# pierluigiferrari/fcn8s_tensorflow

Measured on AMD Instinct MI355X. Metric: training images/sec at 1024x512 bs16, higher is better.
Workload: dtype f32; 1 GPU; FCN-8s (VGG-16, fc6 7x7, 20 classes) train step, 1024x512, 16 images/GPU, SGD+momentum, keep_prob 0.5; global_batch=16, parallelism=dp1

## Files before the change

fcn8s_tensorflow_amd/csrc/fcn8s_internal.h:

```cpp
#pragma once
#include <hip/hip_runtime.h>
#include <stdint.h>
#include "../../include/fcn8s_hip.h"

#if defined(__HIP_DEVICE_COMPILE__) && !defined(__gfx950__)
#error "libfcn8s_hip is written for gfx950 (MI355X) only: build with --offload-arch=gfx950"
#endif
#define FCN8S_LDS_BYTES_NEEDED (160u * 1024u)

#include <string>
namespace fcn8s {

extern thread_local const char* g_last_kernel;
void defer_error(int code, const char* fmt, ...) __attribute__((format(printf, 2, 3)));
int take_deferred_error(std::string* text);

struct IgemmArgs {
    const float* x; const float* w; const float* bias; const float* addend; const float* mask;
    float* y;
    int N, Ma, Mb; long long M;
    int Hi, Wi, Cin, ldx;
    int KW, in_scale, tap_step, tap_off, Ktot;
    int Ho, Wo, Cout, ldy;
    int out_scale, out_offy, out_offx;
    int phases_x; long long w_phase_stride;
    float alpha; int relu; float mask_scale;
    int dropout; float keep_prob; unsigned long long seed; unsigned int stream_id;
    int batched; long long x_batch_stride, y_batch_stride;
    int m_fastest;
    int bt, ldw;
    int fixed_tile;
    int split;
};
void launch_igemm(const IgemmArgs& a, int phases, hipStream_t s);

struct Bf16ConvArgs {
    const float* x; const unsigned short* xh;
    const unsigned short* wt; const float* bias; float* y;
    int N, H, W, Cin, Cout, K;
    int relu, dropout; float keep_prob; unsigned long long seed; unsigned int stream_id;
    long long M; int m_fastest;
};
void launch_w_to_bf16_tiles(const float* w, unsigned short* wt, int K, int Cout, hipStream_t s);
bool launch_conv_bf16(const Bf16ConvArgs& a, hipStream_t s);
void launch_f32_to_bf16(const float* x, unsigned short* y, long long n, hipStream_t s);
struct Bf16Conv256Args {
    const unsigned short* xp; const unsigned short* wt; const float* bias; float* y;
    int N, H, W, Cin, Cout, K;
    int relu, dropout; float keep_prob; unsigned long long seed; unsigned int stream_id;
    long long M; int m_fastest;
    const float* addend;
    const float* mask; float mask_scale;
    int any_shape;
    const unsigned short* mask16;
    float* colpart;
    int ksplit; float* part;
    int rows_bn;
    int guarded;
    unsigned short* yb; int yb_pad;
    long long xp_ps, yb_ps, mask16_ps;
};
bool conv_bf16_256_ok(long long M, int Cin, int Cout, int mode);
void launch_w_to_bf16_t(const float* w, unsigned short* wt, int K, int Cout, hipStream_t s);
void launch_f32_to_bf16_padded(const float* x, unsigned short* xp, int N, int H, int W, int C, int pad, hipStream_t s, long long ps = 0);
int conv_bf16_rows_bm(int Cout, int rows_bn);
bool launch_conv_bf16_256(const Bf16Conv256Args& a, hipStream_t s);
struct Fp8ConvArgs {
    const unsigned char* xp = nullptr; long long xp_ps = 0;
    const unsigned char* wq = nullptr; const int* ew = nullptr;
    const float* bias = nullptr; float* y = nullptr;
    unsigned char* yq = nullptr; long long yq_ps = 0; int yq_pad = 0, yq_exp = 0;
    int ex = 0, relu = 1;
    int N = 0, H = 0, W = 0, Cin = 0, Cout = 0, K = 1;
    long long M = 0;
};
bool launch_conv_fp8(const Fp8ConvArgs& a, hipStream_t s);
void launch_w_to_fp8(const float* w, unsigned char* wq, int* ew, unsigned* amax_scratch, int rows, int Cout, hipStream_t s);
void launch_f32_to_fp8_padded(const float* x, unsigned char* xq, int N, int H, int W, int C, int pad, long long ps, int ex, hipStream_t s);
void launch_zero_border_fp8(unsigned char* xq, int planes, long long ps, int N, int H, int W, int pad, hipStream_t s);
void launch_maxpool_fp8(const unsigned char* xq, long long xps, unsigned char* yq, long long yps, int N, int H, int W, int C, int ypad, hipStream_t s);
void launch_amax(const float* x, long long n, unsigned* amax, hipStream_t s);
bool launch_f32_to_bf16_padded_colsum(const float* x, unsigned short* xp, float* db, int N, int H, int W, int C, int pad, hipStream_t s, long long ps = 0);
void launch_w_to_bf16_flip_t(const float* w, unsigned short* wt, int K, int Cin, int Cout, hipStream_t s);
struct Bf16WgradArgs {
    const unsigned short* A; const unsigned short* B; float* C;
    long long R; int Ci, Cj, K, Wp;
    long long chunk, split_stride; int plain_store;
    long long a_ps, b_ps;
};
bool launch_wgrad_bf16(const Bf16WgradArgs& a, hipStream_t s);

struct WgradArgs {
    const float* A; const float* B; float* C;
    int N, Pa, Pb; long long P;
    int Ha, Wa, Adim, lda, Areal;
    int Bdim, ldb;
    int KW, a_scale, tap_off, ntaps;
    int ldc;
    float alpha;
    float* colsum;
    int batched; long long a_batch_stride, b_batch_stride;
    int c_uninitialized;
    int plain_store;
    int split;
    long long split_stride;
};
void launch_wgrad(const WgradArgs& a, hipStream_t s);

extern thread_local int t_deterministic;
float* det_scratch(hipStream_t s, size_t floats);
float* scratch2(hipStream_t s, size_t floats);
void scratch_release(hipStream_t s);
void launch_det_reduce(float* C, const float* ws, long long rows, int cols, int ldc, long long slab, int nsplit, bool accumulate, hipStream_t s);
bool launch_wgrad_taps(const float* X, const float* dZ, float* dW, float* db, int N, int H, int W, int Cin, int Cout,
// ... 42 lines not shown
                          float rate, float* loss_out, hipStream_t s, const unsigned long long* den = nullptr, float* terms = nullptr);
struct LovaszLayout {
    int nseg = 0, C = 0, tiles = 0; long long L = 0, nsc = 0;
    size_t o_keys[2] = {0, 0}, o_pays[2] = {0, 0}, o_hist = 0, o_tcnt = 0, o_part = 0, o_G = 0, o_V = 0, o_w = 0, o_ncls = 0, o_colpart = 0, o_lov = 0;
    size_t bytes = 0;
};
LovaszLayout lovasz_layout(long long npix, int nseg, int C);
double lovasz_bytes(long long npix, int C, int nmask);
void launch_lovasz_loss(const float* x, int is_logits, const uint8_t* labels, const PixMap* map, int N, long long npix, const LovaszLayout& y,
                        int classes_all, const uint8_t* mask_dev, char* ws, float* class_loss, float* terms, float lce, float llov, float* loss_out,
                        hipStream_t s);
void launch_lovasz_backward(const float* x, int is_logits, const uint8_t* labels, const PixMap* map, int N, long long npix, const LovaszLayout& y,
                            char* ws, float lambda, int accumulate, float* out, float* colsum, hipStream_t s);
void launch_lovasz_total(float* terms, float lce, float* loss_out, hipStream_t s);
void launch_softmax_argmax(const float* logits, float* softmax_out, long long* argmax_out,
                           long long npix, int C, hipStream_t s, const PixMap* map = nullptr, int N = 0);
void launch_tconv_im2col(const float* x, float* A, int N, int Hi, int Wi, int C, int KP, hipStream_t s);
void launch_tconv_col2im(const float* dA, float* dx, int N, int Hi, int Wi, int C, int KP, hipStream_t s);
void launch_tconv_pack_gemm(const float* w, const float* bias, float* b2, float* b2t, float* bias_tiled, int C, int S, int KP, hipStream_t s);
void launch_tconv_unpack_dw(const float* db2, float* dw, int C, int S, hipStream_t s);
void launch_unblock_logits(const float* blocked, float* nhwc, const PixMap& map, int N, int C, hipStream_t s);
void launch_onehot_to_ids(const void* oh, int elem_bytes, long long npix, int C, uint8_t* ids, int* bad, hipStream_t s);
void launch_confusion(const uint8_t* labels, const long long* pred, long long npix,
                      unsigned long long* conf, int C, hipStream_t s);
bool launch_head_fwd(const float* x, const float* w, const float* bias, float* y, long long M, int K, int C, float alpha, hipStream_t s,
                     float* scratch = nullptr, size_t scratch_floats = 0);
bool launch_head_dgrad(const float* dy, const float* wt, const float* mask, float mask_scale, float* dx, long long M, int K, int C, float alpha,
                       hipStream_t s);
bool launch_head_wgrad(const float* x, const float* dy, float* dw, long long M, int K, int C, float alpha, hipStream_t s);
bool launch_maxpool_bwd_bf16(const float* x, const float* dy, unsigned short* dzb, float* db, int N, int H, int W, int C, hipStream_t s, const unsigned char* route = nullptr, long long dzb_ps = 0);
void launch_colsum(const float* x, float* out, long long rows, int C, hipStream_t s);
void launch_sumsq(const float* x, float* out, long long n, hipStream_t s);
void launch_axpy(float* y, const float* x, float a, long long n, hipStream_t s);
void launch_tf_adam(float* theta, const float* g, float* m, float* v, long long n,
                    float lr_t, float b1, float b2, float eps, float gscale, hipStream_t s);
void launch_sgd_momentum(float* theta, const float* g, float* buf, long long n,
                         float lr, float mom, float gscale, hipStream_t s);
void launch_grad_accumulate(float* dst, const float* src, long long n, int mode, hipStream_t s);
constexpr int kGradNormBlocks = 2048;
struct UpdateStats { float norm, clip, scale; int ok; unsigned long long skipped; };
void launch_grad_norm(const float* g, long long n, float grad_scale, float max_norm, double* partials, void* out, bool as_floats, hipStream_t s);
void launch_tf_adam_dev(float* theta, const float* g, float* m, float* v, long long n,
                        float lr_t, float b1, float b2, float eps, const float* s_dev, const int* ok_dev, hipStream_t s);
void launch_sgd_momentum_dev(float* theta, const float* g, float* buf, long long n,
                             float lr, float mom, const float* s_dev, const int* ok_dev, hipStream_t s);
void launch_tf_adam_ema(float* theta, const float* g, float* m, float* v, float* sh, long long n, float lr_t, float b1, float b2, float eps,
                        float gscale, const float* s_dev, const int* ok_dev, float w, hipStream_t s);
void launch_sgd_momentum_ema(float* theta, const float* g, float* buf, float* sh, long long n, float lr, float mom,
                             float gscale, const float* s_dev, const int* ok_dev, float w, hipStream_t s);
void launch_ema_update(float* sh, const float* theta, long long n, float w, const int* ok_dev, hipStream_t s);
void launch_swap(float* a, float* b, long long n, hipStream_t s);
void launch_flip_transpose(const float* w, float* wt, int taps, int Cin, int Cout, hipStream_t s);
void launch_pad_cin(const float* w, float* w4, int taps, int Cin, int Cinp, int Cout, hipStream_t s);
void launch_tconv_phase_pack(const float* w, float* wp, int K, int S, int C, hipStream_t s);
void launch_dropout_mask(float* mask, long long n, float keep_prob, unsigned long long seed,
                         unsigned int stream_id, hipStream_t s);
int wino_r(int KS);
int wino_nsub(int KS);
int wino_alpha(int tile, int KS);
long long wino_slab(long long T, int C);
void launch_wino_filter(int tile, const float* w, float* u, int Cin, int Cout, int KS, hipStream_t s, int transpose_out = 0);
void launch_wino_input(int tile, const float* x, float* v, int N, int H, int W, int C, int KS, hipStream_t s, unsigned* rbits_out = nullptr);
void launch_wino_input_conv1(const float* x0, const float* w4, const float* bias, float* v, int N, int H, int W, hipStream_t s, unsigned* rbits_out = nullptr);
void launch_wino_input_xb(const float* x, float* v, unsigned short* xb, int N, int H, int W, int C, hipStream_t s, unsigned* rbits_out = nullptr);
bool launch_wino_input_dout(int tile, const float* dy, float* v, float* dm, int N, int H, int W, int C, hipStream_t s, const unsigned char* pidx = nullptr);
void launch_wino_output(int tile, const float* m, const float* bias, const float* addend, const float* mask, float mask_scale,
                        int relu, float* y, int N, int H, int W, int C, int dropout, float keep, unsigned long long seed,
                        unsigned int stream_id, hipStream_t s, float* pool = nullptr, unsigned char* pidx = nullptr, int KS = 3,
                        unsigned* rbits_out = nullptr, const unsigned* rbits_in = nullptr);
size_t wino_rbits_words(int tile, int N, int H, int W, int C);
void launch_wino_dout(int tile, const float* dy, float* dm, int N, int H, int W, int C, hipStream_t s, int KS = 3, const unsigned char* pidx = nullptr);
void launch_wino_dgrad_output_dout(const float* dv, const unsigned* rbits_in, float* dm, int N, int H, int W, int C, hipStream_t s);
void launch_wino_dgrad_output_sub44(const float* dv, float* dx, int N, int H, int W, int C, hipStream_t s);
void launch_wino_dgrad_output(const float* dv, const float* addend, const float* mask, float mask_scale, const unsigned* rbits_in, float* y,
                              int N, int H, int W, int C, hipStream_t s);
bool launch_wino_out_in(const float* m, const float* bias, float* v, unsigned* rbits_out, int N, int H, int W, int C, hipStream_t s, bool always = false);
void launch_wino_dfilter(int tile, const float* du, float* dw, int Cin, int Cout, int KS, hipStream_t s);
int fft_fc6_planes();
long long fft_fc6_tiles(int N, int H, int W);
void launch_fft_fc6_filter(const float* w, float* uf, int Cin, int Cout, hipStream_t s);
void launch_fft_fc6_dfilter(const float* duf, float* dw, int Cin, int Cout, hipStream_t s);
void launch_fft_fc6_input(const float* x, float* xf, int N, int H, int W, int C, hipStream_t s);
void launch_fft_fc6_output(const float* yf, const float* bias, float* y, int N, int H, int W, int C, int relu, int dropout, float keep,
                           unsigned long long seed, unsigned int stream_id, hipStream_t s);
void launch_fft_fc6_dout(const float* dz, float* dyf, int N, int H, int W, int C, hipStream_t s);
void launch_fft_fc6_din(const float* dxf, float* patches, float* dx, int N, int H, int W, int C, hipStream_t s);
void launch_augment_u8(const unsigned char* img, const unsigned char* lab, unsigned char* oimg, unsigned char* olab, const int* params,
                       const unsigned char* vlut, int N, int H, int W, int Ho, int Wo, int void_id, hipStream_t s);
void launch_resample_u8(const unsigned char* img, const unsigned char* lab, unsigned char* oimg, unsigned char* olab, const int* params,
                        int N, int H, int W, int Ho, int Wo, int void_id, hipStream_t s);
void launch_tta_input(const void* img, int dtype, int N, int H, int W, int Hs, int Ws, int Hp, int Wp, int flip, float* out4, hipStream_t s);
void launch_tta_accumulate(const float* logits, const PixMap& map, int N, int Hs, int Ws, int flip, int C, int H, int W, float* acc,
                           int first, int last, int npasses, float* softmax_out, long long* argmax_out, hipStream_t s);
bool crf_shape_supported(int C, int radius);
void launch_crf_meanfield(const float* qin, const float* prob, const unsigned char* img, int N, int H, int W, int C, int radius, int dilation,
                          float w_app, float w_smooth, float theta_alpha, float theta_beta, float theta_gamma, float* qout, long long* am, hipStream_t s);
void launch_crf_argmax(const float* p, long long npix, int C, long long* am, hipStream_t s);
size_t cityscapes_work_bytes(int N);
void launch_cityscapes_pair(const uint8_t* gt, const uint16_t* inst, const void* pred, int pred_kind, int N, long long P,
                            unsigned long long* conf, void* work, int* entries, int max_entries, unsigned long long* counts, hipStream_t s);
void launch_boundary_pair(const uint8_t* gt, const void* pred, int pred_kind, int N, int H, int W, int R, unsigned long long* rings,
                          unsigned long long* bprec, unsigned long long* brec, unsigned long long* bad, hipStream_t s);
void launch_fingerprint(const float* x, long long n, unsigned long long* out, hipStream_t s);
void launch_init_normal(float* w, long long n, float stddev, int truncated, unsigned long long seed,
                        unsigned int stream_id, hipStream_t s);

__host__ __device__ inline uint32_t mulhi32(uint32_t a, uint32_t b) { return (uint32_t)(((uint64_t)a * b) >> 32); }
__host__ __device__ inline uint32_t philox_u32(unsigned long long idx, unsigned long long seed, uint32_t stream)
{
    uint32_t c0 = (uint32_t)idx, c1 = (uint32_t)(idx >> 32), c2 = stream, c3 = 0x9E3779B9u;
    uint32_t k0 = (uint32_t)seed, k1 = (uint32_t)(seed >> 32);
#pragma unroll
    for (int r = 0; r < 10; ++r) {
        const uint32_t h0 = mulhi32(0xD2511F53u, c0), l0 = 0xD2511F53u * c0;
        const uint32_t h1 = mulhi32(0xCD9E8D57u, c2), l1 = 0xCD9E8D57u * c2;
        const uint32_t n0 = h1 ^ c1 ^ k0, n2 = h0 ^ c3 ^ k1;
        c0 = n0; c1 = l1; c2 = n2; c3 = l0;
        k0 += 0x9E3779B9u; k1 += 0xBB67AE85u;
    }
    return c0;
}
__host__ __device__ inline float philox_uniform(unsigned long long idx, unsigned long long seed, uint32_t stream)
{
    return (float)(philox_u32(idx, seed, stream) >> 8) * (1.0f / 16777216.0f);
}

}
```

fcn8s_tensorflow_amd/csrc/fft_fc6.hip:

```cpp
#include "fcn8s_internal.h"

namespace fcn8s {

namespace {

__device__ __forceinline__ float c14(int k)
{
    constexpr float t[14] = {1.000000000f, 0.900968868f, 0.623489802f, 0.222520934f, -0.222520934f, -0.623489802f, -0.900968868f,
                             -1.000000000f, -0.900968868f, -0.623489802f, -0.222520934f, 0.222520934f, 0.623489802f, 0.900968868f};
    return t[k % 14];
}
__device__ __forceinline__ float s14(int k)
{
    constexpr float t[14] = {0.000000000f, 0.433883739f, 0.781831482f, 0.974927912f, 0.974927912f, 0.781831482f, 0.433883739f,
                             0.000000000f, -0.433883739f, -0.781831482f, -0.974927912f, -0.974927912f, -0.781831482f, -0.433883739f};
    return t[k % 14];
}
constexpr int nu_of(int v) { return (v == 0 || v == 7) ? 8 : 14; }
constexpr bool is_real(int u, int v) { return (v == 0 || v == 7) && (u == 0 || u == 7); }
constexpr int cplx(int u, int v) { return v == 0 ? u - 1 : (v == 7 ? 90 + u - 1 : 6 + (v - 1) * 14 + u); }
constexpr int realp(int u, int v) { return 288 + (u == 7 ? 1 : 0) + (v == 7 ? 2 : 0); }

#define FFT_FENCE __builtin_amdgcn_sched_barrier(0)

// ... 141 lines not shown
            case 1: input_col<1>(x, xf, slab, tc, oy, ox, H, W, C, c, img); break;
            case 2: input_col<2>(x, xf, slab, tc, oy, ox, H, W, C, c, img); break;
            case 3: input_col<3>(x, xf, slab, tc, oy, ox, H, W, C, c, img); break;
            case 4: input_col<4>(x, xf, slab, tc, oy, ox, H, W, C, c, img); break;
            case 5: input_col<5>(x, xf, slab, tc, oy, ox, H, W, C, c, img); break;
            case 6: input_col<6>(x, xf, slab, tc, oy, ox, H, W, C, c, img); break;
            default: input_col<7>(x, xf, slab, tc, oy, ox, H, W, C, c, img); break;
        }
    }
}

template <int V>
__device__ __forceinline__ void output_col(const float* __restrict__ yf, long long slab, long long tc, float (&acc)[8][8])
{
    constexpr int NU = nu_of(V);
    float R[NU], I[NU];
#pragma unroll
    for (int u = 0; u < NU; ++u) {
        if (is_real(u, V)) { R[u] = yf[realp(u, V) * slab + tc]; I[u] = 0.f; }
        else {
            const float* p = yf + 3LL * cplx(u, V) * slab + tc;
            const float k1 = p[0], k2 = p[slab], k3 = p[2 * slab];
            R[u] = k1 - k3; I[u] = k1 + k2;
        }
    }
#pragma unroll
    for (int j = 0; j < 8; ++j) {
        const int n = 6 + j;
        float P = 0.f, Q = 0.f;
#pragma unroll
        for (int u = 0; u < NU; ++u) {
            const float beta = (is_real(u, V) ? 1.f : 2.f) / 196.f;
            if (is_real(u, V)) { P = fmaf(R[u], beta * c14(u * n), P); Q = fmaf(R[u], beta * s14(u * n), Q); }
            else {
                P = fmaf(R[u], beta * c14(u * n), fmaf(I[u], -beta * s14(u * n), P));
                Q = fmaf(R[u], beta * s14(u * n), fmaf(I[u], beta * c14(u * n), Q));
            }
        }
#pragma unroll
        for (int i = 0; i < 8; ++i) acc[j][i] = fmaf(P, c14(V * (6 + i)), fmaf(Q, -s14(V * (6 + i)), acc[j][i]));
    }
}
__device__ __forceinline__ void output_tile(const float* __restrict__ yf, const float* __restrict__ bias, float* __restrict__ y, int H, int W, int C, long long slab,
                                            long long tc, int n, int ty, int tx, int c, int relu, int dropout, float keep, unsigned long long seed, unsigned int stream_id)
{
    float acc[8][8];
#pragma unroll
    for (int j = 0; j < 8; ++j)
#pragma unroll
        for (int k = 0; k < 8; ++k) acc[j][k] = 0.f;
    output_col<0>(yf, slab, tc, acc); FFT_FENCE; output_col<1>(yf, slab, tc, acc); FFT_FENCE; output_col<2>(yf, slab, tc, acc); FFT_FENCE;
    output_col<3>(yf, slab, tc, acc); FFT_FENCE; output_col<4>(yf, slab, tc, acc); FFT_FENCE; output_col<5>(yf, slab, tc, acc); FFT_FENCE;
    output_col<6>(yf, slab, tc, acc); FFT_FENCE; output_col<7>(yf, slab, tc, acc); FFT_FENCE;
    const float bv = bias ? bias[c] : 0.f;
    const float ik = 1.f / keep;
#pragma unroll
    for (int j = 0; j < 8; ++j)
#pragma unroll
        for (int k = 0; k < 8; ++k) {
            const int py = 8 * ty + j, px = 8 * tx + k;
            if (py >= H || px >= W) continue;
            float v = bv + acc[j][k];
            if (relu) v = fmaxf(v, 0.f);
            const long long off = (((long long)n * H + py) * W + px) * C + c;
            if (dropout) v = philox_uniform((unsigned long long)off, seed, stream_id) < keep ? v * ik : 0.f;
            y[off] = v;
        }
}
__global__ __launch_bounds__(256) void fft_fc6_output_kernel(const float* __restrict__ yf, const float* __restrict__ bias, float* __restrict__ y,
                                                             int N, int H, int W, int C, long long slab, int relu, int dropout, float keep,
                                                             unsigned long long seed, unsigned int stream_id)
{
    const int th = (H + 7) / 8, tw = (W + 7) / 8;
    const long long total = (long long)N * th * tw * C;
    for (long long i = (long long)blockIdx.x * 256 + threadIdx.x; i < total; i += (long long)gridDim.x * 256) {
        const int c = (int)(i % C);
        const long long t = i / C;
        const int tx = (int)(t % tw), ty = (int)((t / tw) % th), n = (int)(t / ((long long)tw * th));
        output_tile(yf, bias, y, H, W, C, slab, i, n, ty, tx, c, relu, dropout, keep, seed, stream_id);
    }
}

template <int V>
__device__ __forceinline__ void dout_col(const float (&d)[8][8], float* __restrict__ dyf, long long slab, long long tc)
{
    float sr[8], si[8];
#pragma unroll
    for (int j = 0; j < 8; ++j) {
        float a = 0.f, b = 0.f;
#pragma unroll
        for (int k = 0; k < 8; ++k) { a = fmaf(d[j][k], c14(V * (6 + k)), a); b = fmaf(d[j][k], -s14(V * (6 + k)), b); }
        sr[j] = a; si[j] = b;
    }
#pragma unroll
    for (int u = 0; u < nu_of(V); ++u) {
        const float beta = (is_real(u, V) ? 1.f : 2.f) / 196.f;
        float gr = 0.f, gi = 0.f;
#pragma unroll
        for (int j = 0; j < 8; ++j) {
            const int n = 6 + j;
            gr = fmaf(sr[j], beta * c14(u * n), fmaf(si[j], beta * s14(u * n), gr));
            gi = fmaf(si[j], beta * c14(u * n), fmaf(sr[j], -beta * s14(u * n), gi));
        }
        if (is_real(u, V)) dyf[realp(u, V) * slab + tc] = gr;
        else {
            const long long p = 3LL * cplx(u, V) * slab + tc;
            dyf[p] = gr + gi; dyf[p + slab] = gi; dyf[p + 2 * slab] = -gr;
        }
    }
}
__global__ __launch_bounds__(256) void fft_fc6_dout_kernel(const float* __restrict__ dz, float* __restrict__ dyf, int N, int H, int W, int C, long long slab)
{
    const int th = (H + 7) / 8, tw = (W + 7) / 8;
    const long long total = (long long)N * th * tw * C;
    for (long long i = (long long)blockIdx.x * 256 + threadIdx.x; i < total; i += (long long)gridDim.x * 256) {
        const int c = (int)(i % C);
        const long long t = i / C;
        const int tx = (int)(t % tw), ty = (int)((t / tw) % th), n = (int)(t / ((long long)tw * th));
        float d[8][8];
#pragma unroll
        for (int j = 0; j < 8; ++j)
#pragma unroll
            for (int k = 0; k < 8; ++k) {
                const int py = 8 * ty + j, px = 8 * tx + k;
                d[j][k] = (py < H && px < W) ? dz[(((long long)n * H + py) * W + px) * C + c] : 0.f;
            }
        dout_col<0>(d, dyf, slab, i); dout_col<1>(d, dyf, slab, i); dout_col<2>(d, dyf, slab, i); dout_col<3>(d, dyf, slab, i);
        dout_col<4>(d, dyf, slab, i); dout_col<5>(d, dyf, slab, i); dout_col<6>(d, dyf, slab, i); dout_col<7>(d, dyf, slab, i);
    }
}

template <int V, int HALF>
__device__ __forceinline__ void din_col(const float* __restrict__ dxf, long long slab, long long tc, float (&acc)[7][14])
{
    constexpr int NU = nu_of(V);
    float A[NU], B[NU];
#pragma unroll
    for (int u = 0; u < NU; ++u) {
        if (is_real(u, V)) { A[u] = dxf[realp(u, V) * slab + tc]; B[u] = 0.f; }
        else {
            const float* p = dxf + 3LL * cplx(u, V) * slab + tc;
            const float ds = p[0], da = p[slab], db = p[2 * slab];
            A[u] = ds + da; B[u] = ds + db;
        }
    }
#pragma unroll
    for (int r = 0; r < 7; ++r) {
        const int n = 7 * HALF + r;
        float P = 0.f, Q = 0.f;
#pragma unroll
        for (int u = 0; u < NU; ++u) {
            if (is_real(u, V)) { P = fmaf(A[u], c14(u * n), P); Q = fmaf(A[u], s14(u * n), Q); }
            else {
                P = fmaf(A[u], c14(u * n), fmaf(B[u], -s14(u * n), P));
                Q = fmaf(A[u], s14(u * n), fmaf(B[u], c14(u * n), Q));
            }
        }
#pragma unroll
        for (int m = 0; m < 14; ++m) acc[r][m] = fmaf(P, c14(V * m), fmaf(Q, -s14(V * m), acc[r][m]));
    }
}
template <int HALF>
__device__ __forceinline__ void din_half(const float* __restrict__ dxf, float* __restrict__ pt, long long slab, long long t, int c, int C)
{
    float acc[7][14];
#pragma unroll
    for (int r = 0; r < 7; ++r)
#pragma unroll
        for (int m = 0; m < 14; ++m) acc[r][m] = 0.f;
    const long long tc = t * C + c;
    din_col<0, HALF>(dxf, slab, tc, acc); FFT_FENCE; din_col<1, HALF>(dxf, slab, tc, acc); FFT_FENCE; din_col<2, HALF>(dxf, slab, tc, acc); FFT_FENCE; din_col<3, HALF>(dxf, slab, tc, acc); FFT_FENCE;
    din_col<4, HALF>(dxf, slab, tc, acc); FFT_FENCE; din_col<5, HALF>(dxf, slab, tc, acc); FFT_FENCE; din_col<6, HALF>(dxf, slab, tc, acc); FFT_FENCE; din_col<7, HALF>(dxf, slab, tc, acc);
    float* o = pt + (t * 196 + 7 * HALF * 14) * C + c;
#pragma unroll
    for (int r = 0; r < 7; ++r)
#pragma unroll
        for (int m = 0; m < 14; ++m) o[(r * 14 + m) * C] = acc[r][m];
}
__global__ __launch_bounds__(256, 2) void fft_fc6_din_kernel(const float* __restrict__ dxf, float* __restrict__ pt, long long T, int C, long long slab)
{
    const long long total = T * 2 * C;
    for (long long i = (long long)blockIdx.x * 256 + threadIdx.x; i < total; i += (long long)gridDim.x * 256) {
        const int c = (int)(i % C);
        const long long r = i / C;
        const int half = (int)(r % 2);
        const long long t = r / 2;
        if (half == 0) din_half<0>(dxf, pt, slab, t, c, C);
        else           din_half<1>(dxf, pt, slab, t, c, C);
    }
}

__global__ __launch_bounds__(256) void fft_fc6_din_gather_kernel(const float* __restrict__ pt, float* __restrict__ dx, int N, int H, int W, int C)
{
    const int th = (H + 7) / 8, tw = (W + 7) / 8;
    const long long total = (long long)N * H * W * C;
    for (long long i = (long long)blockIdx.x * 256 + threadIdx.x; i < total; i += (long long)gridDim.x * 256) {
        const int c = (int)(i % C);
        const long long p = i / C;
        const int px = (int)(p % W), py = (int)((p / W) % H), n = (int)(p / ((long long)W * H));
        const int ty1 = (py + 3) / 8, tx1 = (px + 3) / 8;
        float s = 0.f;
#pragma unroll
        for (int dy = 1; dy >= 0; --dy) {
            const int ty = ty1 - dy, ry = py + 3 - 8 * ty;
            if (ty < 0 || ty >= th || ry > 13) continue;
#pragma unroll
            for (int dxo = 1; dxo >= 0; --dxo) {
                const int tx = tx1 - dxo, rx = px + 3 - 8 * tx;
                if (tx < 0 || tx >= tw || rx > 13) continue;
                s += pt[((((long long)n * th + ty) * tw + tx) * 196 + ry * 14 + rx) * C + c];
            }
        }
        dx[i] = s;
    }
}

}

int fft_fc6_planes() { return 292; }
long long fft_fc6_tiles(int N, int H, int W) { return (long long)N * ((H + 7) / 8) * ((W + 7) / 8); }

void launch_fft_fc6_filter(const float* w, float* uf, int Cin, int Cout, hipStream_t s)
{
    const long long CC = (long long)Cin * Cout;
    hipLaunchKernelGGL(fft_fc6_filter_kernel, dim3(grid_for(CC)), dim3(256), 0, s, w, uf, CC);
}
void launch_fft_fc6_dfilter(const float* duf, float* dw, int Cin, int Cout, hipStream_t s)
{
    const long long CC = (long long)Cin * Cout;
    hipLaunchKernelGGL(fft_fc6_dfilter_kernel, dim3(grid_for(CC)), dim3(256), 0, s, duf, dw, CC);
}
void launch_fft_fc6_input(const float* x, float* xf, int N, int H, int W, int C, hipStream_t s)
{
    const long long T = fft_fc6_tiles(N, H, W);
    hipLaunchKernelGGL(fft_fc6_input_kernel, dim3(grid_for(T * 8 * C)), dim3(256), 0, s, x, xf, N, H, W, C, wino_slab(T, C));
}
void launch_fft_fc6_output(const float* yf, const float* bias, float* y, int N, int H, int W, int C, int relu, int dropout, float keep,
                           unsigned long long seed, unsigned int stream_id, hipStream_t s)
{
    const long long T = fft_fc6_tiles(N, H, W);
    hipLaunchKernelGGL(fft_fc6_output_kernel, dim3(grid_for(T * C)), dim3(256), 0, s, yf, bias, y, N, H, W, C, wino_slab(T, C), relu, dropout, keep, seed, stream_id);
}
void launch_fft_fc6_dout(const float* dz, float* dyf, int N, int H, int W, int C, hipStream_t s)
{
    const long long T = fft_fc6_tiles(N, H, W);
    hipLaunchKernelGGL(fft_fc6_dout_kernel, dim3(grid_for(T * C)), dim3(256), 0, s, dz, dyf, N, H, W, C, wino_slab(T, C));
}
void launch_fft_fc6_din(const float* dxf, float* patches, float* dx, int N, int H, int W, int C, hipStream_t s)
{
    const long long T = fft_fc6_tiles(N, H, W);
    hipLaunchKernelGGL(fft_fc6_din_kernel, dim3(grid_for(T * 2 * C)), dim3(256), 0, s, dxf, patches, T, C, wino_slab(T, C));
    hipLaunchKernelGGL(fft_fc6_din_gather_kernel, dim3(grid_for((long long)N * H * W * C)), dim3(256), 0, s, patches, dx, N, H, W, C);
}

}
```

fcn8s_tensorflow_amd/csrc/igemm.hip:

```cpp
#include "fcn8s_internal.h"
#include <cmath>
#include <cstdlib>
#include <map>
#include <mutex>
#include <string>

namespace fcn8s {

thread_local const char* g_last_kernel = nullptr;
#define FCN8S_STR2(x) #x
#define FCN8S_STR(x) FCN8S_STR2(x)

typedef float f32x16 __attribute__((ext_vector_type(16)));
constexpr int BK_ = 16;

static __device__ __forceinline__ float4 ldg4(const float* p) { return *reinterpret_cast<const float4*>(p); }

static __device__ __forceinline__ unsigned xcd_swizzle(unsigned p, unsigned total)
{
    const unsigned q = total >> 3, r = total & 7u, xcd = p & 7u, i = p >> 3;
    return (xcd < r ? xcd * (q + 1) : r * (q + 1) + (xcd - r) * q) + i;
}

thread_local int t_deterministic = 0;
// ... 349 lines not shown
    }
}

static __device__ __forceinline__ void glds16(const float* sbase, unsigned voff, unsigned lds_byte_off)
{
    asm volatile("s_mov_b32 m0, %2\n\ts_nop 0\n\tglobal_load_lds_dwordx4 %0, %1" ::"v"(voff), "s"(sbase), "s"(lds_byte_off) : "memory", "m0");
}
template <int N> static __device__ __forceinline__ void wait_vmcnt() { asm volatile("s_waitcnt vmcnt(%0)" ::"n"(N) : "memory"); }

typedef __bf16 bf16x8 __attribute__((ext_vector_type(8)));
template <int NS> struct Bf16Pieces { bf16x8 p[NS]; };
template <int NS>
static __device__ __forceinline__ void split_bf16(const float (&x)[8], Bf16Pieces<NS>& o)
{
    typedef __bf16 bf16x2 __attribute__((ext_vector_type(2)));
    typedef float f32x2 __attribute__((ext_vector_type(2)));
    typedef unsigned u32x4 __attribute__((ext_vector_type(4)));
    u32x4 w[NS];
#pragma unroll
    for (int i = 0; i < 4; ++i) {
        f32x2 r = {x[2 * i], x[2 * i + 1]};
#pragma unroll
        for (int k = 0; k < NS; ++k) {
            const unsigned pk = __builtin_bit_cast(unsigned, __builtin_convertvector(r, bf16x2));
            w[k][i] = pk;
            if (k + 1 < NS) {
                const f32x2 back = {__builtin_bit_cast(float, pk << 16), __builtin_bit_cast(float, pk & 0xffff0000u)};
                r = r - back;
            }
        }
    }
#pragma unroll
    for (int k = 0; k < NS; ++k) o.p[k] = __builtin_bit_cast(bf16x8, w[k]);
}
template <int NS>
static __device__ __forceinline__ f32x16 mfma_split(const Bf16Pieces<NS>& a, const Bf16Pieces<NS>& b, f32x16 acc)
{
    if constexpr (NS == 3) {
        acc = __builtin_amdgcn_mfma_f32_32x32x16_bf16(a.p[2], b.p[0], acc, 0, 0, 0);
        acc = __builtin_amdgcn_mfma_f32_32x32x16_bf16(a.p[0], b.p[2], acc, 0, 0, 0);
        acc = __builtin_amdgcn_mfma_f32_32x32x16_bf16(a.p[1], b.p[1], acc, 0, 0, 0);
    }
    acc = __builtin_amdgcn_mfma_f32_32x32x16_bf16(a.p[1], b.p[0], acc, 0, 0, 0);
    acc = __builtin_amdgcn_mfma_f32_32x32x16_bf16(a.p[0], b.p[1], acc, 0, 0, 0);
    return __builtin_amdgcn_mfma_f32_32x32x16_bf16(a.p[0], b.p[0], acc, 0, 0, 0);
}

template <int BM, int BN, int WM, int WN, int S, bool EPI, int NSPLIT, bool BT = false>
static __device__ __forceinline__ void gemm_glds_body(const IgemmArgs& p);
template <int BM, int BN, int WM, int WN, int S, bool EPI>
__global__ __launch_bounds__(256, (S * (BM + BN) * 64 <= 40960) ? 4 : 3) void gemm_glds_kernel(const IgemmArgs p) { gemm_glds_body<BM, BN, WM, WN, S, EPI, 0>(p); }
template <int BM, int BN, int WM, int WN, int S, bool EPI>
__global__ __launch_bounds__(256, (S * (BM + BN) * 64 <= 40960) ? 4 : 3) void gemm_glds_x3_kernel(const IgemmArgs p) { gemm_glds_body<BM, BN, WM, WN, S, EPI, 3>(p); }
template <int BM, int BN, int WM, int WN, int S>
__global__ __launch_bounds__(256, (S * (BM + BN) * 64 <= 40960) ? 4 : 3) void gemm_glds_nt_kernel(const IgemmArgs p) { gemm_glds_body<BM, BN, WM, WN, S, false, 0, true>(p); }
template <int BM, int BN, int WM, int WN, int S>
__global__ __launch_bounds__(256, (S * (BM + BN) * 64 <= 40960) ? 4 : 3) void gemm_glds_nt_x3_kernel(const IgemmArgs p) { gemm_glds_body<BM, BN, WM, WN, S, false, 3, true>(p); }
template <int BM, int BN, int WM, int WN, int S, bool EPI>
__global__ __launch_bounds__(256, (S * (BM + BN) * 64 <= 40960) ? 4 : 3) void gemm_glds_x2_kernel(const IgemmArgs p) { gemm_glds_body<BM, BN, WM, WN, S, EPI, 2>(p); }
template <int BM, int BN, int WM, int WN, int S>
__global__ __launch_bounds__(256, (S * (BM + BN) * 64 <= 40960) ? 4 : 3) void gemm_glds_nt_x2_kernel(const IgemmArgs p) { gemm_glds_body<BM, BN, WM, WN, S, false, 2, true>(p); }
template <int BM, int BN, int WM, int WN, int S, bool EPI, int NSPLIT, bool BT>
static __device__ __forceinline__ void gemm_glds_body(const IgemmArgs& p)
{
    constexpr int BK = 16, CH = 4, RPI = 16;
    constexpr int TM = BM / WM / 32, TN = BN / WN / 32;
    constexpr int A_PW = BM / RPI / 4, B_PW = BT ? BN / RPI / 4 : BK * BN / 256 / 4;
    static_assert(WM * WN == 4 && A_PW >= 1 && B_PW >= 1, "tile / wave split");
    constexpr int L = A_PW + B_PW;
    constexpr int STAGE = BM * BK + BK * BN;
    __shared__ __attribute__((aligned(16))) float smem[S * STAGE];
    static_assert(S * STAGE >= 4 * 32 * 36, "epilogue patches");

    const int tid = threadIdx.x, lane = tid & 63, wave = __builtin_amdgcn_readfirstlane(tid >> 6);
    int cwave = wave;
    bool idle = false;
    if constexpr (BM == 64 && WM == 2 && WN == 2) {
        if (p.M <= 32) {
            const unsigned lin = blockIdx.x + gridDim.x * (blockIdx.y + gridDim.y * blockIdx.z);
            cwave = wave ^ (int)(((lin >> 8) & 1u) << 1); idle = cwave >= 2;
        }
    }
    const int wm = cwave / WN, wn = cwave % WN;
    const int pz = blockIdx.z;
    const float* __restrict__ Wp = p.w + (long long)pz * p.w_phase_stride;
    const float* __restrict__ X = p.batched ? p.x + (long long)pz * p.x_batch_stride : p.x;
    float* __restrict__ Y = p.batched ? p.y + (long long)pz * p.y_batch_stride : p.y;
    const unsigned ntn = (unsigned)(p.Cout / BN);
    const unsigned lid = xcd_swizzle(blockIdx.x, gridDim.x);
    const unsigned ntm = gridDim.x / ntn;
    const long long m0 = (long long)(p.m_fastest ? lid % ntm : lid / ntn) * BM;
    const int n0 = (int)(p.m_fastest ? lid / ntm : lid % ntn) * BN;

    unsigned a_voff[A_PW], b_voff[B_PW];
#pragma unroll
    for (int i = 0; i < A_PW; ++i) {
        const int row = (wave * A_PW + i) * RPI + lane / CH, pc = lane % CH;
        const int c = pc ^ ((row >> 2) & 3);
        long long m = m0 + row; if (m >= p.M) m = p.M - 1;
        a_voff[i] = (unsigned)((m - m0) * p.ldx + c * 4) * 4u;
    }
#pragma unroll
    for (int i = 0; i < B_PW; ++i) {
        if (BT) {
            const int row = (wave * B_PW + i) * RPI + lane / CH, pc = lane % CH;
            const int c = pc ^ ((row >> 2) & 3);
            b_voff[i] = (unsigned)(row * p.ldw + c * 4) * 4u;
        } else {
            const int f = (wave * B_PW + i) * 64 + lane;
            const int k = f / (BN / 4), j = (f % (BN / 4)) * 4;
            b_voff[i] = (unsigned)(k * p.Cout + j) * 4u;
        }
    }
    const int nkt_all = p.Ktot / BK;
    const int kt0 = (int)((long long)nkt_all * blockIdx.y / gridDim.y);
    const int nkt = (int)((long long)nkt_all * (blockIdx.y + 1) / gridDim.y) - kt0;
    const float* a_base = X + m0 * p.ldx + (long long)kt0 * BK;
    const float* b_base = BT ? Wp + (long long)n0 * p.ldw + (long long)kt0 * BK : Wp + n0 + (long long)kt0 * BK * p.Cout;
    const unsigned lds0 = (unsigned)(size_t)(__attribute__((address_space(3))) float*)smem;
    auto issue = [&](int kt, int stage) {
        const float* ga = a_base + (long long)kt * BK;
        const float* gb = BT ? b_base + (long long)kt * BK : b_base + (long long)kt * BK * p.Cout;
        const unsigned la = lds0 + (unsigned)(stage * STAGE + wave * A_PW * 256) * 4u;
        const unsigned lb = lds0 + (unsigned)(stage * STAGE + BM * BK + wave * B_PW * 256) * 4u;
#pragma unroll
        for (int i = 0; i < A_PW; ++i) glds16(ga, a_voff[i], la + i * 1024);
#pragma unroll
        for (int i = 0; i < B_PW; ++i) glds16(gb, b_voff[i], lb + i * 1024);
    };

    f32x16 acc[TM][TN];
#pragma unroll
    for (int i = 0; i < TM; ++i)
#pragma unroll
        for (int j = 0; j < TN; ++j)
#pragma unroll
            for (int r = 0; r < 16; ++r) acc[i][j][r] = 0.f;

    int a_off[TM], a_sw[TM];
#pragma unroll
    for (int tm = 0; tm < TM; ++tm) {
        const int row = wm * TM * 32 + tm * 32 + (lane & 31);
        a_off[tm] = row * BK;
        a_sw[tm] = (row >> 2) & 3;
    }
    const int b_off = ((lane >> 5) * 4) * BN + wn * TN * 32 + (lane & 31);
    int bt_off[TN], bt_sw[TN];
#pragma unroll
    for (int tn = 0; tn < TN; ++tn) {
        const int row = wn * TN * 32 + tn * 32 + (lane & 31);
        bt_off[tn] = row * BK;
        bt_sw[tn] = (row >> 2) & 3;
    }
    auto compute = [&](int stage) {
        if (idle) return;
        const float* sa = smem + stage * STAGE;
        const float* sb = sa + BM * BK;
        if constexpr (NSPLIT >= 2) {
            Bf16Pieces<NSPLIT> ap[TM], bp[TN];
#pragma unroll
            for (int tm = 0; tm < TM; ++tm) {
                const float4 u = *reinterpret_cast<const float4*>(sa + a_off[tm] + (((2 * (lane >> 5)) ^ a_sw[tm]) * 4));
                const float4 v = *reinterpret_cast<const float4*>(sa + a_off[tm] + (((2 * (lane >> 5) + 1) ^ a_sw[tm]) * 4));
                const float x[8] = {u.x, u.y, u.z, u.w, v.x, v.y, v.z, v.w};
                split_bf16<NSPLIT>(x, ap[tm]);
            }
#pragma unroll
            for (int tn = 0; tn < TN; ++tn) {
                float x[8];
                if (BT) {
                    const float4 u = *reinterpret_cast<const float4*>(sb + bt_off[tn] + (((2 * (lane >> 5)) ^ bt_sw[tn]) * 4));
                    const float4 v = *reinterpret_cast<const float4*>(sb + bt_off[tn] + (((2 * (lane >> 5) + 1) ^ bt_sw[tn]) * 4));
                    x[0] = u.x; x[1] = u.y; x[2] = u.z; x[3] = u.w; x[4] = v.x; x[5] = v.y; x[6] = v.z; x[7] = v.w;
// ... 282 lines not shown
            const long long pix = ((long long)n * p.H + y0 + 2 * g + (row >> 4)) * p.W + x0 + (row & 15);
            if (p.y) *reinterpret_cast<float4*>(p.y + pix * BN + wn * 32 + (lane & 7) * 4) = v;
        }
        if (p.yb16) {
            const float4 b0 = ldg4(p.bias + wn * 32 + (lane & 3) * 8), b1 = ldg4(p.bias + wn * 32 + (lane & 3) * 8 + 4);
#pragma unroll
            for (int j = 0; j < 2; ++j) {
                const int row = j * 16 + (lane >> 2);
                const float4 u = *reinterpret_cast<const float4*>(&patch[row * LDT + (lane & 3) * 8]);
                const float4 w_ = *reinterpret_cast<const float4*>(&patch[row * LDT + (lane & 3) * 8 + 4]);
                __attribute__((ext_vector_type(8))) __bf16 o;
                o[0] = (__bf16)fmaxf(u.x + b0.x, 0.f); o[1] = (__bf16)fmaxf(u.y + b0.y, 0.f); o[2] = (__bf16)fmaxf(u.z + b0.z, 0.f); o[3] = (__bf16)fmaxf(u.w + b0.w, 0.f);
                o[4] = (__bf16)fmaxf(w_.x + b1.x, 0.f); o[5] = (__bf16)fmaxf(w_.y + b1.y, 0.f); o[6] = (__bf16)fmaxf(w_.z + b1.z, 0.f); o[7] = (__bf16)fmaxf(w_.w + b1.w, 0.f);
                const long long q = ((long long)n * (p.H + 2) + y0 + 2 * g + (row >> 4) + 1) * (p.W + 2) + x0 + (row & 15) + 1;
                *reinterpret_cast<__attribute__((ext_vector_type(8))) __bf16*>(p.yb16 + (p.yb16_ps ? (long long)wn * p.yb16_ps + q * 32 + (lane & 3) * 8 : q * BN + wn * 32 + (lane & 3) * 8)) = o;
            }
        }
        __builtin_amdgcn_wave_barrier();
    }
  }
}

bool launch_conv1_fwd(const float* x4, const float* w48, const float* bias, float* y, const float* zero16, int N, int H, int W, int Cout, int tiled, hipStream_t s, unsigned short* yb16, long long yb16_ps)
{
    if (Cout != 64 || !bias || !zero16) return false;
    if ((yb16 || !y) && !(tiled && H % 8 == 0 && W % 16 == 0)) return false;
    Conv1Args a{x4, w48, bias, y, zero16, N, H, W, (long long)N * H * W, yb16, yb16_ps};
    if (tiled && H % 8 == 0 && W % 16 == 0) {
        g_last_kernel = "conv1_tile_kernel";
        const long long tiles = (long long)N * (H / 8) * (W / 16);
        if (W % 64 == 0 && tiles >= 4 * 4096) hipLaunchKernelGGL(conv1_tile_kernel<4>, dim3((unsigned)(tiles / 4)), dim3(256), 0, s, a);
        else                                  hipLaunchKernelGGL(conv1_tile_kernel<1>, dim3((unsigned)tiles), dim3(256), 0, s, a);
        return true;
    }
    g_last_kernel = "conv1_glds_kernel";
    hipLaunchKernelGGL(conv1_glds_kernel, dim3((unsigned)((a.M + 127) / 128)), dim3(256), 0, s, a);
    return true;
}

template <int BM, int BN, int WM, int WN, int BKF = 16>
static void launch_igemm_cfg(const IgemmArgs& a0, int phases, hipStream_t s)
{
    IgemmArgs a = a0;
    a.m_fastest = (double)a.Ktot * a.Cout > (double)a.M * a.Cin;
    dim3 grid((unsigned)(((a.M + BM - 1) / BM) * ((a.Cout + BN - 1) / BN)), 1, (unsigned)phases);
    const bool fast = (phases == 1 || a.batched) && a.Cin % BKF == 0 && a.Cout % BN == 0 && a.Ktot % a.Cin == 0;
    const bool tap_inner = fast && (double)a.Ktot * a.Cout * 4.0 <= 64e6 && a.Ktot / a.Cin <= 32;
    const bool plain = fast && a.batched && a.Ktot == a.Cin && !a.bias && !a.addend && !a.mask && !a.relu && !a.dropout && a.alpha == 1.f &&
                       a.out_scale == 1 && a.ldy >= a.Cout && a.ldy % 4 == 0 && a.in_scale == 1 && a.tap_off == 0;
    const int mode = !fast ? 0 : (plain ? 3 : (tap_inner ? 2 : 1));
    static const std::string base = "igemm_fwd_kernel<" + std::to_string(BM) + ", " + std::to_string(BN) + ", " + std::to_string(WM) + ", " + std::to_string(WN) + ", ";
    static const std::string tags[4] = {base + "0, 16>", base + "1, " + std::to_string(BKF) + ">", base + "2, " + std::to_string(BKF) + ">",
                                        base + "3, " + std::to_string(BKF) + ">"};
    g_last_kernel = tags[mode].c_str();
    const bool linear = (mode == 1 || mode == 3) && !a.relu && !a.mask && !a.dropout && !a.addend && a.out_scale == 1 && a.ldy == a.Cout;
    constexpr int splitk_min_kt = 64;
    const unsigned nblocks = grid.x * (unsigned)phases, nkt_all = (unsigned)(a.Ktot / BKF);
    if (linear && !t_deterministic && !a.fixed_tile && ((grid.x < 512 && nkt_all >= 512) || (nblocks < 2048 && nkt_all >= (unsigned)splitk_min_kt))) {
        unsigned ks = nkt_all >= 512 && grid.x < 512 ? 1024 / grid.x : 4096 / nblocks;
        if (ks > 8) ks = 8;
        if (ks > nkt_all / 16) ks = nkt_all / 16;
        if (ks >= 2) {
            grid.y = ks;
            const size_t nfl = a.batched ? (size_t)(phases - 1) * a.y_batch_stride + (size_t)a.M * a.Cout : (size_t)a.M * a.Cout;
            hipMemsetAsync(a.y, 0, nfl * sizeof(float), s);
        }
    }
    const bool rows1x1 = fast && a.Ktot == a.Cin && a.in_scale == 1 && a.tap_off == 0 && a.out_scale == 1 && a.out_offy == 0 && a.out_offx == 0 &&
                         (a.batched || (phases == 1 && a.Hi == a.Ma && a.Wi == a.Mb && a.Ho == a.Ma && a.Wo == a.Mb)) && a.ldy >= a.Cout;
    const bool bias_only = fast && a.bias && !a.addend && !a.mask && !a.relu && !a.dropout && a.alpha == 1.f && a.ldy % 4 == 0 && a.Cout % 4 == 0 && grid.y == 1;
    if constexpr (BN >= 64 && BKF == 16) {
        if (rows1x1 && (mode == 3 || grid.y == 1) && (long long)(BM - 1) * a.ldx < (1LL << 29) && (long long)16 * a.Cout < (1LL << 29)) {
            static const std::string gbase = "gemm_glds_kernel<" + std::to_string(BM) + ", " + std::to_string(BN) + ", " + std::to_string(WM) + ", " + std::to_string(WN) + ", 3, ";
            static const std::string xbase = "gemm_glds_x3_kernel<" + std::to_string(BM) + ", " + std::to_string(BN) + ", " + std::to_string(WM) + ", " + std::to_string(WN) + ", 3, ";
            static const std::string gt[4] = {gbase + "false>", gbase + "true>", xbase + "false>", xbase + "true>"};
            const bool mask_only = fast && a.mask && !a.bias && !a.addend && !a.relu && !a.dropout && a.alpha == 1.f && a.ldy % 4 == 0 && a.Cout % 4 == 0 && grid.y == 1;
            const bool epi = mode != 3 && !bias_only && !mask_only;
            if (a.bt) {
                static const std::string nb = "gemm_glds_nt_kernel<" + std::to_string(BM) + ", " + std::to_string(BN) + ", " + std::to_string(WM) + ", " + std::to_string(WN) + ", 3>";
                static const std::string nbx = "gemm_glds_nt_x3_kernel<" + std::to_string(BM) + ", " + std::to_string(BN) + ", " + std::to_string(WM) + ", " + std::to_string(WN) + ", 3>";
                if (mode != 3 || (long long)(BN - 1) * a.ldw >= (1LL << 29)) { defer_error(FCN8S_ERR_STATE, "transposed-B GEMM needs the plain batched form"); return; }
                static const std::string nbx2 = "gemm_glds_nt_x2_kernel<" + std::to_string(BM) + ", " + std::to_string(BN) + ", " + std::to_string(WM) + ", " + std::to_string(WN) + ", 3>";
                g_last_kernel = (a.split == 3 ? nbx : a.split == 2 ? nbx2 : nb).c_str();
                if (a.split == 3) hipLaunchKernelGGL((gemm_glds_nt_x3_kernel<BM, BN, WM, WN, 3>), grid, dim3(256), 0, s, a);
                else if (a.split == 2) hipLaunchKernelGGL((gemm_glds_nt_x2_kernel<BM, BN, WM, WN, 3>), grid, dim3(256), 0, s, a);
                else                   hipLaunchKernelGGL((gemm_glds_nt_kernel<BM, BN, WM, WN, 3>), grid, dim3(256), 0, s, a);
                return;
            }
            g_last_kernel = gt[(epi ? 1 : 0) + (a.split == 3 ? 2 : 0)].c_str();
            if (a.split == 3) {
                if (epi) hipLaunchKernelGGL((gemm_glds_x3_kernel<BM, BN, WM, WN, 3, true>), grid, dim3(256), 0, s, a);
                else     hipLaunchKernelGGL((gemm_glds_x3_kernel<BM, BN, WM, WN, 3, false>), grid, dim3(256), 0, s, a);
                return;
            }
            if (a.split == 2) {
                static const std::string x2base = "gemm_glds_x2_kernel<" + std::to_string(BM) + ", " + std::to_string(BN) + ", " + std::to_string(WM) + ", " + std::to_string(WN) + ", 3, ";
                static const std::string x2t[2] = {x2base + "false>", x2base + "true>"};
                g_last_kernel = x2t[epi ? 1 : 0].c_str();
                if (epi) hipLaunchKernelGGL((gemm_glds_x2_kernel<BM, BN, WM, WN, 3, true>), grid, dim3(256), 0, s, a);
                else     hipLaunchKernelGGL((gemm_glds_x2_kernel<BM, BN, WM, WN, 3, false>), grid, dim3(256), 0, s, a);
                return;
            }
            if (epi) hipLaunchKernelGGL((gemm_glds_kernel<BM, BN, WM, WN, 3, true>), grid, dim3(256), 0, s, a);
            else     hipLaunchKernelGGL((gemm_glds_kernel<BM, BN, WM, WN, 3, false>), grid, dim3(256), 0, s, a);
            return;
        }
    }
    if (a.bt) {
        defer_error(FCN8S_ERR_STATE, "transposed-B GEMM (M %lld, K %d, N %d, tile %dx%d) does not fit the LDS-DMA kernel", a.M, a.Ktot, a.Cout, BM, BN);
        return;
    }
    if (mode == 3)      hipLaunchKernelGGL((igemm_fwd_kernel<BM, BN, WM, WN, 3, BKF>), grid, dim3(256), 0, s, a);
    else if (mode == 2) hipLaunchKernelGGL((igemm_fwd_kernel<BM, BN, WM, WN, 2, BKF>), grid, dim3(256), 0, s, a);
    else if (mode == 1) hipLaunchKernelGGL((igemm_fwd_kernel<BM, BN, WM, WN, 1, BKF>), grid, dim3(256), 0, s, a);
    else                hipLaunchKernelGGL((igemm_fwd_kernel<BM, BN, WM, WN, 0, 16>), grid, dim3(256), 0, s, a);
}

void launch_igemm(const IgemmArgs& a, int phases, hipStream_t s)
{
    auto cost = [&](int bm, int bn, int bpc, double eff) {
        const long long blocks = ((a.M + bm - 1) / bm) * ((a.Cout + bn - 1) / bn) * phases;
        const long long n = (blocks + 255) / 256, rem = n % bpc;
        const double tail = rem == 0 ? 0.0 : (rem == 1 ? 2.0 : (rem == 2 ? 2.4 : 3.0));
        return ((double)(n / bpc) * bpc + tail) * bm * bn / eff;
    };
    if (a.fixed_tile && a.Cout % 128 == 0) { launch_igemm_cfg<128, 128, 2, 2>(a, phases, s); return; }
    if (a.fixed_tile && a.Cout % 64 == 0)  { launch_igemm_cfg<128, 64, 2, 2>(a, phases, s); return; }
    if (a.Cout <= 32)      launch_igemm_cfg<128, 32, 4, 1>(a, phases, s);
    else if (a.Cout <= 64) {
        if (cost(128, 64, 4, 1.0) <= cost(64, 64, 4, 0.9)) launch_igemm_cfg<128, 64, 2, 2>(a, phases, s);
        else                                               launch_igemm_cfg<64, 64, 2, 2>(a, phases, s);
    } else {
        const double c128 = cost(128, 128, 3, 1.0), c64x128 = cost(64, 128, 4, 0.9), c64 = cost(64, 64, 4, 0.85);
        if (a.M > 64 && c128 <= c64x128 && c128 <= c64) launch_igemm_cfg<128, 128, 2, 2>(a, phases, s);
        else if (c64x128 <= c64)                        launch_igemm_cfg<64, 128, 2, 2>(a, phases, s);
        else                                            launch_igemm_cfg<64, 64, 2, 2>(a, phases, s);
    }
}

template <int BM, int BN, int WM, int WN, int WK, bool FAST, bool COLSUM>
__global__ __launch_bounds__(256, FAST ? 4 : 1) void wgrad_kernel(const WgradArgs p, const int chunk)
{
    constexpr int BK = 16, LDA = BM, LDB = BN;
    constexpr int TM = BM / WM / 32, TN = BN / WN / 32;
    constexpr int A_F4 = BK * BM / 4, B_F4 = BK * BN / 4;
    constexpr int A_LD = (A_F4 + 255) / 256, B_LD = (B_F4 + 255) / 256;
    static_assert(WM * WN * WK == 4, "4 waves");
    __shared__ __attribute__((aligned(16))) float smem[2 * BK * LDA + 2 * BK * LDB];
    float* As = smem;
    float* Bs = smem + 2 * BK * LDA;

    const int tid = threadIdx.x, lane = tid & 63, wave = tid >> 6;
    const int wk = wave / (WM * WN), wmn = wave % (WM * WN);
    const int wm = wmn / WN, wn = wmn % WN;
    const int ntj = (p.Bdim + BN - 1) / BN;
    const int ti = blockIdx.x / ntj, tj = blockIdx.x - ti * ntj;
    const int i0 = ti * BM, j0 = tj * BN;
    const int tap = blockIdx.z;
    const int ty = tap / p.KW, tx = tap - ty * p.KW;
    const int dy = p.batched ? 0 : ty + p.tap_off, dx = p.batched ? 0 : tx + p.tap_off;
    const float* __restrict__ Ap = p.batched ? p.A + (long long)tap * p.a_batch_stride : p.A;
    const float* __restrict__ Bp = p.batched ? p.B + (long long)tap * p.b_batch_stride : p.B;
    const long long pbeg = (long long)blockIdx.y * chunk;
    const long long pend = (pbeg + chunk < p.P) ? pbeg + chunk : p.P;
    const int PaPb = p.Pa * p.Pb;
    const bool do_colsum = COLSUM && p.colsum != nullptr && tap == 0 && ti == 0 && wm == 0;
// ... 834 lines not shown
```

fcn8s_tensorflow_amd/csrc/model.hip:

```cpp
#include "../../include/fcn8s_hip.h"
#include "fcn8s_internal.h"
#include "device_buffer.h"
#include "pass_state.h"
#include <cstdarg>

#include <dlfcn.h>
#include <atomic>
#include <chrono>
#include <thread>
#include <cmath>
#include <cstdio>
#include <cstring>
#include <cstdlib>
#include <algorithm>
#include <mutex>
#include <map>
#include <set>
#include <string>
#include <vector>

using namespace fcn8s;

extern "C" {
typedef struct ncclComm* ncclComm_t;
typedef struct { char internal[128]; } ncclUniqueId;
typedef enum { ncclSuccess = 0, ncclUnhandledCudaError = 1, ncclSystemError = 2, ncclInternalError = 3, ncclInvalidArgument = 4, ncclInvalidUsage = 5,
               ncclRemoteError = 6, ncclInProgress = 7 } ncclResult_t;
typedef enum { ncclSum = 0 } ncclRedOp_t;
typedef enum { ncclFloat = 7, ncclDouble = 8 } ncclDataType_t;
}
static_assert(sizeof(ncclUniqueId) == FCN8S_COMM_ID_BYTES, "fcn8s_comm_unique_id hands out ncclUniqueId bytes");

namespace {

thread_local std::string g_last_error;
thread_local int t_deferred_code = 0;
thread_local std::string t_deferred_text;

struct ParamInfo {
    std::string name;
    int ndim;
    int64_t shape[4];
    size_t offset, numel;
};

struct ProfGroup {
    std::string name;
    std::vector<std::pair<hipEvent_t, hipEvent_t>> ev;
    std::vector<std::pair<hipEvent_t, hipEvent_t>> ev_shared;
    double flops = 0, bytes = 0;
    int64_t launches = 0;
};

struct Act { float* p = nullptr; size_t n = 0; int H = 0, W = 0, C = 0; };

const int kConvsPerBlock[5] = {2, 2, 3, 3, 3};

}

namespace fcn8s {
void defer_error(int code, const char* fmt, ...)
{
    if (t_deferred_code) return;
    char buf[1024];
    va_list ap; va_start(ap, fmt); vsnprintf(buf, sizeof buf, fmt, ap); va_end(ap);
    t_deferred_code = code; t_deferred_text = buf;
}
int take_deferred_error(std::string* text)
{
    const int c = t_deferred_code;
    if (c && text) *text = t_deferred_text;
    t_deferred_code = 0; t_deferred_text.clear();
    return c;
}
}

struct Q8Buf { DeviceBuf<unsigned char> p; int N = 0, H = 0, W = 0, C = 0, pad = -1, ex = 0; long long ps = 0; };
struct W8Bank { DeviceBuf<unsigned char> wq; int* ew = nullptr; unsigned* amax = nullptr; };

struct fcn8s_model {
    int C = 20, fc6k = 7, device = 0;
    int widths[7] = {64, 128, 256, 512, 512, 4096, 4096};
    uint64_t seed = 0;
    std::vector<ParamInfo> params;
    std::map<std::string, int> index;
    size_t total = 0;
    size_t bucket_off[FCN8S_MAX_BUCKETS] = {0}, bucket_n[FCN8S_MAX_BUCKETS] = {0};
    hipEvent_t bucket_ev[FCN8S_MAX_BUCKETS] = {nullptr};
    bool bucket_final[FCN8S_MAX_BUCKETS] = {false};
    ncclComm_t comm = nullptr; int comm_rank = 0, comm_world = 1;
    hipStream_t comm_stream = nullptr;
    static constexpr int kCommSlots = FCN8S_MAX_BUCKETS + 1, kCommMisc = FCN8S_MAX_BUCKETS;
    hipEvent_t comm_done[kCommSlots] = {nullptr}; bool comm_pending[FCN8S_MAX_BUCKETS] = {false};
    std::mutex comm_mu;
    std::thread comm_watch; std::atomic<bool> comm_watch_stop{false}, comm_failed{false};
    std::atomic<bool> comm_inflight[kCommSlots] = {}; int64_t comm_enq_ns[kCommSlots] = {0};
    std::string comm_error; int64_t comm_timeout_ms = 600000;
    float *d_params = nullptr, *d_grads = nullptr;
    DeviceBuf<float> own_params, own_grads;
    DeviceBuf<float> d_m, d_v, d_wt, d_w1pad, d_tph[3];
    DeviceBuf<float> d_wino_u; float *d_wino_v = nullptr, *d_wino_m = nullptr;
    size_t ufl = 0;
    int wino_min_cin = 64;
    int wino_tile = 6;
    int wino_fc6 = 1;
    int fc6_fft = 1;
    int fc6_fft_wgrad = 1;
    int wino_tile_hires = 0, wino_hires_pixels = 0;
    int wino_force_tile = 0;
    int precision = FCN8S_PREC_F32;
    bool frozen = false;
    unsigned long long frozen_fp = 0; DeviceBuf<unsigned long long> d_fp;
    PinnedBuf<unsigned long long> h_fp; hipEvent_t fp_event = nullptr;
    std::map<std::string, DeviceBuf<float>> u_cache;
    std::map<std::string, DeviceBuf<float>> u_train;
    bool fwd_train = false;
    PassState pass;
    int deterministic = 0;
    int fuse_dgrad_dout = 1;
    int fuse_out_in = 1;
    int conv1_tiled = 1, conv1_wgrad_mfma = 1;
    int conv1_in_transform = 1;
    DeviceBuf<unsigned short> d_wbf16;
    std::map<std::string, DeviceBuf<unsigned short>> wbf16_cache;
    std::set<std::string> bank_stale; bool banks_stale = false;
    int bf16_gemm256 = 1;
    DeviceBuf<unsigned short> d_abf16;
    std::map<std::string, DeviceBuf<unsigned short>> xbf16;
    using G16Map = std::map<std::string, DeviceBuf<unsigned short>>;
    G16Map xg16, dyg16;
    std::set<std::string> g16_stale;
    int bf16_fuse_pool = 1;
    int bf16_infer_copies = 1;
    int bf16_rows_bn = 0;
    int bf16_acts = 1;
    bool fp8_calibrated = false, fp8_calibrating = false; float fp8_amax[FCN8S_FP8_LAYERS] = {}; DeviceBuf<unsigned> d_fp8_amax;
    std::map<std::string, Q8Buf> q8;
    std::map<std::string, W8Bank> w8; std::set<std::string> w8_valid;
    int saved_wino_min_cin = -1, saved_wino_fc6 = -1;
    int bf16_copy_by_transform = 1;
    int64_t ws_allocs = 0;
    bool x0_ready = false;
    DeviceBuf<char> crf_buf;
    DeviceBuf<char> tta_buf;
    hipStream_t stream = nullptr;
    int64_t step = 0;
    int N = 0, H = 0, W = 0;
    int plan_N = 0;
    DeviceBuf<char> arena;
    std::map<std::string, Act> acts;
    struct KeptDy { DeviceBuf<float> p; size_t n = 0; };
    int keep_dy = 0; std::map<std::string, KeptDy> kept_dy;
    int tconv_gemm = 1; PixMap pm{0, 0, 0, 0, 0, 0}; int tg_kp = 0;
    float *logits_b = nullptr, *dlogits_b = nullptr, *tg_A = nullptr, *tg_dA = nullptr;
    DeviceBuf<float> tg_b2, tg_b2t, tg_bias, tg_db2;
    bool logits_nhwc_valid = false;
    float *dlogits = nullptr, *da3 = nullptr, *da4 = nullptr, *ds7 = nullptr, *gskip3 = nullptr, *gskip4 = nullptr;
    float *gbuf[2] = {nullptr, nullptr};
    int gcur = 0;
    void* d_images = nullptr; uint8_t* d_labels = nullptr;
    DeviceBuf<float> d_loss; float *d_regsum = nullptr, *d_softmax = nullptr;
    PinnedBuf<float> h_loss; hipEvent_t loss_ev = nullptr; bool loss_copied = false;
    float* d_lastbias = nullptr;
    double* d_partials = nullptr; long long* d_pred = nullptr;
    int loss_mode = 0, last_loss_mode = 0; float ohem_thresh = 0.f; int64_t ohem_min_kept = 0;
    DeviceBuf<float> d_cw; DeviceBuf<char> loss_ws;
    bool lov_on = false, have_terms = false; float lov_ce = 1.f, lov_w = 0.f; int lov_per_image = 0, lov_all = 0;
    DeviceBuf<uint8_t> d_lovmask; int lov_nmask = 0; DeviceBuf<char> lov_ws; float* d_terms = nullptr;
    DeviceBuf<float> d_acc; int acc_k[FCN8S_MAX_BUCKETS] = {0}; bool acc_taken[FCN8S_MAX_BUCKETS] = {false};
    float max_norm = 0.f; DeviceBuf<char> upd_ws; bool last_update_clipped = false;
    DeviceBuf<float> d_ema; double ema_decay = 0.0; int ema_warmup = 1; bool ema_swapped = false;
    DeviceBuf<unsigned long long> d_conf;
    double loss_sum = 0; int64_t loss_cnt = 0;
    float keep_prob = 1.f, l2_rate = 0.f;
    uint32_t drop_stream = 0;
    bool have_forward = false, have_loss = false, train_mode = false;
    int next_bucket = 0;
    const uint8_t* cur_labels = nullptr;
    bool profile = false, profile_detail = false;
    struct StageSlot { PinnedBuf<uint8_t> h_img, h_lab; DeviceBuf<uint8_t> d_img, d_lab;
                       hipEvent_t ready = nullptr, consumed = nullptr; bool used = false; };
    StageSlot slots[FCN8S_NUM_STAGE_SLOTS];
    hipStream_t copy_stream = nullptr;
    std::vector<ProfGroup> groups;
    std::string err;
    fcn8s_model() = default;
    fcn8s_model(const fcn8s_model&) = delete;
    ~fcn8s_model()
    {
// ... 67 lines not shown
    add("fc7_pool4_conv2d_trans/bias", {C});
    add("fc7_pool4_pool3_conv2d_trans/kernel", {16, 16, C, C});
    add("fc7_pool4_pool3_conv2d_trans/bias", {C});
    total = off;
    for (int i = 0; i < FCN8S_MAX_BUCKETS; ++i) { boff[i] = 0; bn[i] = 0; }
    boff[0] = fc7_start;   bn[0] = total - fc7_start;
    boff[1] = fc6_start;   bn[1] = fc7_start - fc6_start;
    boff[2] = conv4_start; bn[2] = fc6_start - conv4_start;
    boff[3] = 0;           bn[3] = conv4_start;
}

void resolve_cfg(const fcn8s_config* cfg, int& C, int widths[7], int& fc6k)
{
    static const int def[7] = {64, 128, 256, 512, 512, 4096, 4096};
    C = cfg->num_classes;
    fc6k = cfg->fc6_ksize > 0 ? cfg->fc6_ksize : 7;
    for (int i = 0; i < 7; ++i) widths[i] = cfg->widths[i] > 0 ? cfg->widths[i] : def[i];
}

const ParamInfo& P(const fcn8s_model* m, const std::string& n) { return m->params[m->index.at(n)]; }
float* Wp(fcn8s_model* m, const std::string& n) { return m->d_params + P(m, n).offset; }
float* Gp(fcn8s_model* m, const std::string& n) { return m->d_grads + P(m, n).offset; }
float* WTp(fcn8s_model* m, const std::string& n) { return m->d_wt + P(m, n).offset; }

int group_id(fcn8s_model* m, const char* name)
{
    for (size_t i = 0; i < m->groups.size(); ++i) if (m->groups[i].name == name) return (int)i;
    ProfGroup g; g.name = name; m->groups.push_back(g);
    return (int)m->groups.size() - 1;
}
struct ProfScope {
    fcn8s_model* m; int gid = -1; hipEvent_t a = nullptr, b = nullptr; double fl = 0, by = 0;
    ProfScope(fcn8s_model* m_, const char* group, double flops, double bytes, const char* layer = nullptr) : m(m_), fl(flops), by(bytes)
    {
        if (!m || !m->profile) return;
        fcn8s::g_last_kernel = nullptr;
        gid = (m->profile_detail && layer) ? group_id(m, (std::string(group) + ":" + layer).c_str()) : group_id(m, group);
        hipEventCreate(&a); hipEventCreate(&b);
        hipEventRecord(a, m->stream);
        m->groups[gid].flops += flops; m->groups[gid].bytes += bytes; m->groups[gid].launches += 1;
    }
    ~ProfScope()
    {
        if (gid < 0) return;
        hipEventRecord(b, m->stream);
        m->groups[gid].ev.emplace_back(a, b);
        if (fcn8s::g_last_kernel) {
            const int k = group_id(m, (std::string("kernel:") + fcn8s::g_last_kernel).c_str());
            m->groups[k].flops += fl; m->groups[k].bytes += by; m->groups[k].launches += 1;
            m->groups[k].ev_shared.emplace_back(a, b);
        }
    }
};

static void prof_derived(fcn8s_model* m, const char* what)
{
    if (m && m->profile && m->profile_detail) m->groups[group_id(m, (std::string("derived:") + what).c_str())].launches += 1;
}

struct ConvEpi { float alpha = 1.f; };
struct FwdEpi : ConvEpi {
    const float* bias = nullptr; int relu = 0;
    int dropout = 0; float keep = 1.f; uint32_t stream_id = 0;
    float* pool_out = nullptr; unsigned char* pool_idx = nullptr;
    int skip_y = 0;
    unsigned* relu_bits_out = nullptr;
    unsigned* in_relu_bits_out = nullptr; const char* in_layer = nullptr;
    float* next_v = nullptr; const char* next_layer = nullptr;
};
struct DgradEpi : ConvEpi {
    const float* addend = nullptr;
    const float* mask = nullptr; float mask_scale = 1.f;
    const unsigned* relu_bits_in = nullptr;
    const float* w_fwd = nullptr;
    int lazy_wt = 0;
    float* dm_out = nullptr; const char* dm_out_layer = nullptr;
    const char* yb_layer = nullptr; int yb_K = 3;
    bool yb_only = false;
};

static bool bt_gemm_ok(int K, int N) { return K % 16 == 0 && (N == 64 || N % 128 == 0); }
thread_local int t_op_split = 0;
thread_local int t_op_rows_bn = 0;
thread_local int t_op_planes = 1;
int split_of(const fcn8s_model* m)
{
    if (!m) return t_op_split;
    if (m->precision == FCN8S_PREC_F32X3 || m->precision == FCN8S_PREC_BF16_FWD) return 3;
    if (m->precision == FCN8S_PREC_F32X2 || m->precision == FCN8S_PREC_BF16_FWD_X2) return 2;
    return 0;
}
static inline bool bf16_fwd_mode(const fcn8s_model* m) { return m->precision == FCN8S_PREC_BF16_FWD || m->precision == FCN8S_PREC_BF16_FWD_X2; }
static inline bool bf16_train_mode(const fcn8s_model* m) { return m && m->precision == FCN8S_PREC_BF16_TRAIN; }
static inline long long bf16_guard_rows(int K, int Wp) { return (long long)((K - 1) / 2) * Wp + (K - 1) / 2 + 640; }
#ifndef A_PLANES
#define A_PLANES 1
#endif
static inline long long g16_ps(int N, int H, int W, int K) { const int pad = (K - 1) / 2, Wp_ = W + 2 * pad; return A_PLANES ? ((long long)N * (H + 2 * pad) * Wp_ + 2 * bf16_guard_rows(K, Wp_)) * 32 : 0; }
static inline long long g16_off(long long G, int C) { return A_PLANES ? G * 32 : G * C; }
unsigned short* g16_for(fcn8s_model* m, fcn8s_model::G16Map& bufs, const char* layer, int N, int H, int W, int C, int K, hipStream_t s);
unsigned short* dyb_for(fcn8s_model* m, const char* layer, const float* dy, int N, int H, int W, int C, int K, hipStream_t s, float* db = nullptr, bool* db_done = nullptr);

int wino_tile_for(const fcn8s_model* m, int H, int W, int K = 3)
{
    if (!m || H % 2 || W % 2) return 0;
    if (m->wino_force_tile && K == 3) return (m->wino_force_tile == 6 || (H % m->wino_force_tile == 0 && W % m->wino_force_tile == 0)) ? m->wino_force_tile : 0;
    int tmax = m->wino_tile;
    if (K == 3 && m->wino_tile_hires && m->wino_hires_pixels > 0 && (long long)H * W >= m->wino_hires_pixels && m->wino_tile_hires < tmax) tmax = m->wino_tile_hires;
    const bool t4 = tmax >= 4 && H % 4 == 0 && W % 4 == 0;
    if (K == 7) return (m->wino_tile >= 4 && H % 4 == 0 && W % 4 == 0) ? 4 : 0;
    if (tmax == 6) {
        auto rows = [&](long long tiles) { return m->plan_N == 1 ? (tiles + 63) / 64 * 64 : tiles; };
        const long long c6 = 64LL * rows((long long)((H + 5) / 6) * ((W + 5) / 6)), c4 = t4 ? 36LL * rows((long long)(H / 4) * (W / 4)) : 16LL * rows((long long)(H / 2) * (W / 2));
        if (c6 < c4) return 6;
    }
    return t4 ? 4 : 2;
}
long long wino_tiles(int tile, int N, int H, int W) { return (long long)N * ((H + tile - 1) / tile) * ((W + tile - 1) / tile); }
struct WinoEpi { const float* bias = nullptr; const float* addend = nullptr; const float* mask = nullptr; float mask_scale = 1.f;
                 int relu = 0; int dropout = 0; float keep = 1.f; unsigned long long seed = 0; unsigned int stream_id = 0; float* pool = nullptr; unsigned char* pidx = nullptr;
                 unsigned* rbits_out = nullptr; const unsigned* rbits_in = nullptr; int skip_y = 0;
                 unsigned* in_rbits_out = nullptr;
                 float* next_v = nullptr; bool* fused_out = nullptr; };
static bool fft6_cheaper(const fcn8s_model* m, int H, int W)
{
    const long long fft = 292LL * ((H + 7) / 8) * ((W + 7) / 8);
    const long long other = wino_tile_for(m, H, W, 7) == 4 ? 196LL * (H / 4) * (W / 4) : 49LL * H * W;
    return fft < other;
}
static bool fft6_shape_ok(const fcn8s_model* m, int ci, int co) { return m->wino_fc6 && m->fc6_fft && m->fc6k == 7 && ci % 16 == 0 && co % 128 == 0; }
static bool fft6_on(const fcn8s_model* m, int N, int H, int W, int ci, int co)
{
    if (!m || !fft6_shape_ok(m, ci, co) || !fft6_cheaper(m, H, W) || m->precision != FCN8S_PREC_F32 || m->frozen || !m->d_wino_v || !m->d_wino_m) return false;
    const long long T = fft_fc6_tiles(N, H, W);
    auto v = m->acts.find("wino_v"), mm = m->acts.find("wino_m");
    return v != m->acts.end() && mm != m->acts.end() && v->second.n >= (size_t)fft_fc6_planes() * (size_t)wino_slab(T, ci) &&
           mm->second.n >= std::max((size_t)fft_fc6_planes() * (size_t)wino_slab(T, co), (size_t)T * 196 * ci);
}
constexpr long long kFft6WgradMinTiles = 32;
static bool fft6_wgrad_wanted(const fcn8s_model* m, long long T) { return m->fc6_fft_wgrad == 2 || (m->fc6_fft_wgrad == 1 && T >= kFft6WgradMinTiles); }
struct Fc6Scratch { size_t v_wino = 0, v_fft = 0, m_fft = 0, wv = 0; };
static Fc6Scratch fc6_scratch_floats(const fcn8s_model* m, int N, int h5, int w5, int ci, int co)
{
    Fc6Scratch r;
    const int hi = std::max(ci, co);
    if (m->wino_fc6 && m->fc6k == 7 && wino_tile_for(m, h5, w5, 7) == 4 && ci % 16 == 0 && co % 64 == 0) {
        const size_t P = (size_t)wino_alpha(4, 7) * wino_alpha(4, 7);
        const int ns2 = wino_nsub(7) * wino_nsub(7);
        const long long T = wino_tiles(4, N, h5, w5);
        r.v_wino = std::max(P * (size_t)wino_slab(T, ns2 * hi), P * (size_t)wino_slab(T, hi));
        r.wv = P * (size_t)wino_slab(T, ns2 * ci);
    }
    if (fft6_shape_ok(m, ci, co) && fft6_cheaper(m, h5, w5)) {
        const size_t P = (size_t)fft_fc6_planes();
        const long long T = fft_fc6_tiles(N, h5, w5);
        r.v_fft = P * (size_t)wino_slab(T, ci);
        r.m_fft = std::max(P * (size_t)wino_slab(T, co), (size_t)T * 196 * ci);
        if (fft6_wgrad_wanted(m, T)) r.wv = std::max(r.wv, P * (size_t)wino_slab(T, ci));
    }
    return r;
}
static size_t fc6_bank_floats(int ci, int co)
{
    size_t n = 49 * 4 * (size_t)ci * co;
    if (ci % 16 == 0 && co % 128 == 0) n = std::max(n, (size_t)fft_fc6_planes() * ci * co);
    return n;
}
static IgemmArgs fft6_gemm(const float* x, const float* w, float* y, long long T, int K, int Nc)
{
    IgemmArgs a{};
    a.x = x; a.w = w; a.y = y;
    a.N = 1; a.Ma = (int)T; a.Mb = 1; a.M = T;
    a.Hi = (int)T; a.Wi = 1; a.Cin = K; a.ldx = K;
    a.KW = 1; a.in_scale = 1; a.tap_step = 1; a.tap_off = 0; a.Ktot = K;
    a.Ho = (int)T; a.Wo = 1; a.Cout = Nc; a.ldy = Nc;
    a.out_scale = 1; a.phases_x = 1; a.w_phase_stride = (long long)K * Nc;
    a.alpha = 1.f; a.mask_scale = 1.f;
    a.batched = 1; a.x_batch_stride = wino_slab(T, K); a.y_batch_stride = wino_slab(T, Nc);
    return a;
}
static bool conv_fft6_fwd(fcn8s_model* m, const char* layer, const float* x, const float* w, float* y, int N, int H, int W, int Cin, int Cout,
                          const float* bias, int relu, int dropout, float keep, unsigned int stream_id, hipStream_t s)
{
    const int P = fft_fc6_planes();
    const long long T = fft_fc6_tiles(N, H, W);
    DeviceBuf<float>& uf = m->u_train[std::string(layer) + "#fft"];
    if (!uf.grow((size_t)P * Cin * Cout * sizeof(float), s)) return false;
    auto wv = m->acts.find(std::string("wv:") + layer);
    const bool dft_wgrad = wv != m->acts.end() && fft6_wgrad_wanted(m, T) && wv->second.n >= (size_t)P * (size_t)wino_slab(T, Cin) &&
                           m->ufl >= (size_t)P * Cin * Cout;
    const bool want_v = !dft_wgrad && wv != m->acts.end() && wino_tile_for(m, H, W, 7) == 4;
    float* xf = dft_wgrad ? wv->second.p : m->d_wino_v;
    { ProfScope ps(m, "fc6_fft_transform", 0, 4.0 * ((49.0 + P) * Cin * Cout + (double)N * H * W * Cin + (double)P * T * Cin));
      launch_fft_fc6_filter(w, uf, Cin, Cout, s); launch_fft_fc6_input(x, xf, N, H, W, Cin, s); }
    if (want_v) { ProfScope ps(m, "wino_transform", 0, 4.0 * ((double)N * H * W * Cin * 4 + 49.0 * wino_tiles(4, N, H, W) * 4 * Cin));
                  launch_wino_input(4, x, wv->second.p, N, H, W, Cin, 7, s); }
    IgemmArgs a = fft6_gemm(xf, uf, m->d_wino_m, T, Cin, Cout); a.fixed_tile = 1;
    { ProfScope ps(m, "fc6_fft_gemm_fwd", 2.0 * P * T * Cin * Cout, 4.0 * P * (T * (double)(Cin + Cout) + (double)Cin * Cout), layer); launch_igemm(a, P, s); }
    { ProfScope ps(m, "fc6_fft_transform", 0, 4.0 * ((double)P * T * Cout + (double)N * H * W * Cout));
      launch_fft_fc6_output(m->d_wino_m, bias, y, N, H, W, Cout, relu, dropout, keep, m->seed, stream_id, s); }
    m->pass.fft6_ready.give(layer);
    if (dft_wgrad) m->pass.fft6_xf.give(layer);
    return true;
}
static void conv_fft6_wgrad(fcn8s_model* m, const char* layer, const float* xf, const float* dz, float* dw, float* db, int N, int H, int W, int Cin, int Cout, hipStream_t s)
{
    const int P = fft_fc6_planes();
    const long long T = fft_fc6_tiles(N, H, W);
    { ProfScope ps(m, "fc6_fft_transform", 0, 4.0 * ((double)N * H * W * Cout + (double)P * T * Cout)); launch_fft_fc6_dout(dz, m->d_wino_m, N, H, W, Cout, s); }
    m->pass.fft6_dyf.give(layer);
    WgradArgs g{}; g.split = 0;
    g.A = xf; g.B = m->d_wino_m; g.C = m->d_wino_u;
    g.N = 1; g.Pa = 1; g.Pb = (int)T; g.P = T;
    g.Ha = 1; g.Wa = (int)T; g.Adim = Cin; g.lda = Cin; g.Areal = Cin;
    g.Bdim = Cout; g.ldb = Cout; g.KW = 1; g.a_scale = 1; g.tap_off = 0; g.ntaps = P; g.ldc = Cout; g.alpha = 1.f; g.colsum = nullptr;
    g.batched = 1; g.a_batch_stride = wino_slab(T, Cin); g.b_batch_stride = wino_slab(T, Cout); g.c_uninitialized = 1;
    { ProfScope ps(m, "fc6_fft_gemm_wgrad", 2.0 * P * T * Cin * Cout, 4.0 * P * (T * (double)(Cin + Cout) + (double)Cin * Cout), layer); launch_wgrad(g, s); }
    { ProfScope ps(m, "fc6_fft_transform", 0, 4.0 * (P + 49.0) * Cin * Cout); launch_fft_fc6_dfilter(m->d_wino_u, dw, Cin, Cout, s); }
    if (db) { ProfScope ps(m, "colsum", 0, 4.0 * N * H * W * Cout); launch_colsum(dz, db, (long long)N * H * W, Cout, s); }
}
static void conv_fft6_dgrad(fcn8s_model* m, const char* layer, const float* dz, const float* uf, float* dx, int N, int H, int W, int Cin, int Cout, hipStream_t s)
{
    const int P = fft_fc6_planes();
    const long long T = fft_fc6_tiles(N, H, W);
    if (!m->pass.fft6_dyf.take(layer)) {
        m->pass.fft6_dyf.drop();
        ProfScope ps(m, "fc6_fft_transform", 0, 4.0 * ((double)N * H * W * Cin + (double)P * T * Cin)); launch_fft_fc6_dout(dz, m->d_wino_m, N, H, W, Cin, s);
    }
    IgemmArgs a = fft6_gemm(m->d_wino_m, uf, m->d_wino_v, T, Cin, Cout);
    a.fixed_tile = 1; a.bt = 1; a.ldw = Cin;
    { ProfScope ps(m, "fc6_fft_gemm_dgrad", 2.0 * P * T * Cin * Cout, 4.0 * P * (T * (double)(Cin + Cout) + (double)Cin * Cout), layer); launch_igemm(a, P, s); }
    { ProfScope ps(m, "fc6_fft_transform", 0, 4.0 * ((double)P * T * Cout + 2.0 * 196.0 * T * Cout + (double)N * H * W * Cout));
      launch_fft_fc6_din(m->d_wino_v, m->d_wino_m, dx, N, H, W, Cout, s); }
}

void conv_winograd(fcn8s_model* m, int tile, int KS, bool fwd, const float* x, const float* wk, float* y, float* u, float* v, float* mm,
                   int N, int H, int W, int Cin, int Cout, const WinoEpi& e, hipStream_t s, const char* layer, bool v_ready = false)
{
    const int P = wino_alpha(tile, KS) * wino_alpha(tile, KS), nsub2 = wino_nsub(KS) * wino_nsub(KS);
    const long long T = wino_tiles(tile, N, H, W);
    const int Kg = nsub2 * Cin;
    IgemmArgs a = fft6_gemm(v, u, mm, T, Kg, Cout); a.split = split_of(m);
    const double tb = 4.0 * ((double)N * H * W * Cin * nsub2 + (double)P * T * Kg), ob = 4.0 * ((double)N * H * W * Cout * ((e.pool ? (e.skip_y ? 0.25 : 1.25) : 1.0) + (e.rbits_in ? 1.0 / 32 : (e.mask ? 1.0 : 0.0)) + (e.addend ? 1.0 : 0.0) + (e.rbits_out ? 1.0 / 32 : 0.0)) + (double)P * T * Cout);
    bool u_cached = false;
    const char* tag = KS == 7 ? (fwd ? "wino_gemm_fc6_fwd" : "wino_gemm_fc6_dgrad") : (fwd ? "wino_gemm_fwd" : "wino_gemm_dgrad");
    if (m && m->frozen && layer && fwd) {
        DeviceBuf<float>& cu = m->u_cache[std::string(layer) + "#" + std::to_string(tile)];
        const std::string key = "u:" + std::string(layer) + "#" + std::to_string(tile);
        if (cu && !m->bank_stale.count(key)) { u = cu; u_cached = true; }
        else if (cu) { u = cu; m->bank_stale.erase(key); }
        else if (cu.grow((size_t)P * Kg * Cout * sizeof(float), s, &m->ws_allocs)) u = cu;
        a.w = u;
    }
    if (m && !u_cached && m->fwd_train && layer && fwd && ((KS == 3 && tile == 6) || (KS == 7 && tile == 4))) {
        DeviceBuf<float>& tu = m->u_train[std::string(layer) + "#" + std::to_string(tile)];
        if (tu.grow((size_t)P * Kg * Cout * sizeof(float), s)) { u = tu; a.w = u; }
    }
    auto pre = [&]() { if (!u_cached) { prof_derived(m, "wino_filter_kernel"); launch_wino_filter(tile, wk, u, Cin, Cout, KS, s); } if (!v_ready) launch_wino_input(tile, x, v, N, H, W, Cin, KS, s, e.in_rbits_out); };
    auto post = [&]() {
        if (e.next_v && tile == 6 && KS == 3 && e.relu && e.bias && !e.addend && !e.mask && !e.dropout && !e.pool && !e.rbits_in &&
            launch_wino_out_in(mm, e.bias, e.next_v, e.rbits_out, N, H, W, Cout, s, m && m->fuse_out_in >= 2)) { if (e.fused_out) *e.fused_out = true; return; }
        launch_wino_output(tile, mm, e.bias, e.addend, e.mask, e.mask_scale, e.relu, (e.skip_y && e.pool) ? nullptr : y, N, H, W, Cout, e.dropout, e.keep, e.seed, e.stream_id, s, e.pool, e.pidx, KS, e.rbits_out, e.rbits_in); };
    const double ob_fused = 4.0 * (2.0 * P * T * Cout + (e.rbits_out ? (double)N * H * W * Cout / 32 : 0.0));
    { ProfScope ps(m, "wino_transform", 0, (v_ready ? 0.0 : tb) + (u_cached ? 0.0 : (double)(KS * KS + P * nsub2) * 4 * Cin * Cout)); pre(); }
    { ProfScope ps(m, tag, 2.0 * P * T * Kg * Cout, 4.0 * P * (T * (double)(Kg + Cout) + (double)Kg * Cout), layer); launch_igemm(a, P, s); }
    { ProfScope ps(m, "wino_transform", 0, ob); post(); if (e.fused_out && *e.fused_out && m && m->profile && !m->groups.empty()) { const int g = group_id(m, "wino_transform"); m->groups[g].bytes += ob_fused - ob; } }
}

static void conv_direct(fcn8s_model* m, const char* group, IgemmArgs a, const float* x, const float* w, float* y,
                        int N, int H, int W, int Cin, int Cout, int K, hipStream_t s, int real_cin, const char* layer)
{
    a.split = split_of(m);
    a.x = x; a.w = w; a.y = y;
    a.N = N; a.Ma = H; a.Mb = W; a.M = (long long)N * H * W;
    a.Hi = H; a.Wi = W; a.Cin = Cin; a.ldx = Cin;
    a.KW = K; a.in_scale = 1; a.tap_step = 1; a.tap_off = -(K - 1) / 2; a.Ktot = K * K * Cin;
    a.Ho = H; a.Wo = W; a.Cout = Cout; a.ldy = Cout;
    a.out_scale = 1; a.out_offy = 0; a.out_offx = 0; a.phases_x = 1; a.w_phase_stride = 0;
    a.seed = m ? m->seed : 0;
    const double rc = real_cin ? real_cin : Cin;
    const double flops = 2.0 * a.M * K * K * rc * Cout;
    const double bytes = 4.0 * (a.M * rc + (double)a.M * Cout + (double)K * K * rc * Cout);
    auto run = [&]() {
        if (K == 1 && !real_cin && !a.addend && !a.relu && !a.dropout) {
            if (Cout <= 32 && !a.mask && launch_head_fwd(x, w, a.bias, y, a.M, Cin, Cout, a.alpha, s, m ? m->d_wino_u : nullptr, m ? m->ufl : 0)) return;
            if (Cin <= 32 && !a.bias && launch_head_dgrad(x, w, a.mask, a.mask_scale, y, a.M, Cout, Cin, a.alpha, s)) return;
        }
        launch_igemm(a, 1, s);
    };
    { ProfScope ps(m, group, flops, bytes, layer); run(); }
}

bool conv_fwd(fcn8s_model* m, const char* group, const float* x, const float* w, float* y,
              int N, int H, int W, int Cin, int Cout, int K, const FwdEpi& e, hipStream_t s, int real_cin = 0,
              const char* layer = nullptr)
{
    if (m && K == 7 && layer && !real_cin && e.alpha == 1.f && !e.pool_out && !e.relu_bits_out && m->fwd_train && fft6_on(m, N, H, W, Cin, Cout) &&
        conv_fft6_fwd(m, layer, x, w, y, N, H, W, Cin, Cout, e.bias, e.relu, e.dropout, e.keep, e.stream_id, s)) return false;
    if (m) m->pass.drop_backward_handoffs();
    const bool wino3 = m && K == 3 && m->wino_min_cin > 0 && Cin >= m->wino_min_cin && m->d_wino_v && wino_tile_for(m, H, W, 3) && !e.dropout;
    const bool wino7 = m && K == 7 && m->wino_fc6 && m->d_wino_v && wino_tile_for(m, H, W, 7) == 4;
    if ((wino3 || wino7) && Cin % 16 == 0 && Cout % 64 == 0 && e.alpha == 1.f && !real_cin) {
        const bool v_ready = m->pass.fwd_v.take(layer);
        m->pass.fwd_v.drop();
        float* vbuf = m->d_wino_v;
        if (layer) { auto it = m->acts.find(std::string("wv:") + layer); if (it != m->acts.end()) vbuf = it->second.p; }
        WinoEpi we; we.bias = e.bias; we.relu = e.relu;
        we.dropout = e.dropout; we.keep = e.keep; we.seed = m->seed; we.stream_id = e.stream_id; we.pool = e.pool_out; we.pidx = e.pool_idx;
        we.rbits_out = e.relu_bits_out; we.skip_y = e.skip_y && e.pool_out;
        if (e.relu_bits_out && layer) m->pass.rbits_ok.insert(layer);
        if (e.in_relu_bits_out && e.in_layer && K == 3) { we.in_rbits_out = e.in_relu_bits_out; m->pass.rbits_ok.insert(e.in_layer); }
        bool fused_out = false;
        if (e.next_v && e.next_layer) { we.next_v = e.next_v; we.fused_out = &fused_out; }
        conv_winograd(m, wino_tile_for(m, H, W, K), K, true, x, w, y, m->d_wino_u, vbuf, m->d_wino_m, N, H, W, Cin, Cout, we, s, layer, v_ready);
        if (fused_out) { m->pass.fwd_v.give(e.next_layer); if (layer) m->pass.y_unwritten.insert(layer); }
        return e.pool_out != nullptr;
    }
    IgemmArgs a{}; a.bias = e.bias; a.alpha = e.alpha; a.relu = e.relu; a.mask_scale = 1.f; a.dropout = e.dropout; a.keep_prob = e.keep; a.stream_id = e.stream_id;
    conv_direct(m, group, a, x, w, y, N, H, W, Cin, Cout, K, s, real_cin, layer);
    return false;
}

void conv_dgrad(fcn8s_model* m, const char* group, const float* x, const float* w, float* y,
                int N, int H, int W, int Cin, int Cout, int K, const DgradEpi& e, hipStream_t s, const char* layer = nullptr)
{
    const bool bf16_step = bf16_train_mode(m) && m->train_mode && layer;
    if (bf16_step && e.w_fwd && e.alpha == 1.f && Cin % 32 == 0 && Cout % 64 == 0) {
        const size_t wneed = (size_t)K * K * Cin * Cout;
        const bool ok = m->d_wbf16.grow(wneed * sizeof(unsigned short), s, &m->ws_allocs);
        unsigned short* dyb = ok ? dyb_for(m, layer, x, N, H, W, Cin, K, s) : nullptr;
        if (dyb) {
            { ProfScope ps(m, "weight_relayout", 0, 6.0 * wneed); launch_w_to_bf16_flip_t(e.w_fwd, m->d_wbf16, K, Cout, Cin, s); }
            Bf16Conv256Args g{};
            g.xp = dyb; g.xp_ps = g16_ps(N, H, W, K); g.wt = m->d_wbf16; g.y = y; g.N = N; g.H = H; g.W = W; g.Cin = Cin; g.Cout = Cout; g.K = K;
            g.addend = e.addend; g.mask = e.mask; g.mask_scale = e.mask_scale; g.any_shape = 1; g.guarded = 1; g.rows_bn = m->bf16_rows_bn;
            if (e.mask && K == 3 && e.mask_scale == 1.f) {
                auto xi = m->xg16.find(layer);
                if (xi != m->xg16.end() && xi->second) { g.mask16 = xi->second + g16_off(bf16_guard_rows(3, W + 2), Cout); g.mask16_ps = g16_ps(N, H, W, 3); }
            }
            const bool only16 = e.yb_layer && e.yb_only && m->bf16_acts && K == 3 && e.yb_K == 3 && Cout % 64 == 0;
            if (only16) { g.yb = g16_for(m, m->dyg16, e.yb_layer, N, H, W, Cout, e.yb_K, s); g.yb_pad = (e.yb_K - 1) / 2; g.yb_ps = g16_ps(N, H, W, e.yb_K); }
            long long prow = 0;
            if (g.yb) {
                prow = ((long long)N * (H + 2) * (W + 2) + conv_bf16_rows_bm(Cout, g.rows_bn) - 1) / conv_bf16_rows_bm(Cout, g.rows_bn);
                g.colpart = det_scratch(s, (size_t)prow * Cout);
                if (g.colpart) g.y = nullptr; else prow = 0;
            }
            const double M = (double)N * H * W;
            bool done;
            { ProfScope ps(m, K == 1 ? "fc7_dgrad_bf16" : (K == 3 ? "conv3x3_dgrad_bf16" : "fc6_dgrad_bf16"), 2.0 * M * K * K * Cin * Cout,
                           (g.y ? 4.0 : 0.0) * M * Cout + (g.yb ? 2.0 : 0.0) * M * Cout + (g.mask16 ? 2.0 : (e.mask ? 4.0 : 0.0)) * M * Cout + 2.0 * M * Cin + 2.0 * wneed, layer);
              done = launch_conv_bf16_256(g, s); }
            if (done) {
                if (g.yb) m->pass.dyg16_filled.insert(e.yb_layer);
                if (g.colpart) {
                    ProfScope ps(m, "colsum", 0, 4.0 * prow * Cout);
                    launch_colsum(g.colpart, Gp(m, std::string(e.yb_layer) + "/biases"), prow, Cout, s);
                    m->pass.db_taken.insert(e.yb_layer); m->pass.dy_bf16_only.insert(e.yb_layer);
                }
                return;
            }
            if (g.colpart) { defer_error(FCN8S_ERR_SHAPE, "bf16_train: %s's data gradient was refused by the flat-position kernel", layer); return; }
        }
    }
    if (bf16_step && m->pass.dy_bf16_only.count(layer)) {
        defer_error(FCN8S_ERR_SHAPE, "bf16_train: %s's data gradient could not run on the bf16 kernel and its fp32 output gradient was not kept (option \"bf16_acts\" = 0 keeps it)", layer); return;
    }
    if (bf16_step && e.mask && m->pass.in_bf16_only.count(layer)) {
        defer_error(FCN8S_ERR_SHAPE, "bf16_train: %s's data gradient could not run on the bf16 kernel and its fp32 mask was not kept (option \"bf16_acts\" = 0 keeps it)", layer); return;
    }
    const bool dm_ready = m && m->pass.dm.take(layer), v_ready = m && m->pass.dgrad_v.take(layer);
    if (m) m->pass.drop_backward_handoffs();
    if (m && K == 7 && layer && e.alpha == 1.f && !e.addend && !e.mask && !e.relu_bits_in) {
        auto kept = m->u_train.find(std::string(layer) + "#fft");
        if (m->pass.fft6_ready.holds(layer) && kept != m->u_train.end() && kept->second && fft6_on(m, N, H, W, Cout, Cin) && bt_gemm_ok(Cin, Cout)) {
            conv_fft6_dgrad(m, layer, x, kept->second, y, N, H, W, Cin, Cout, s);
            return;
        }
    }
    const bool wino3 = m && K == 3 && m->wino_min_cin > 0 && Cin >= m->wino_min_cin && m->d_wino_v && wino_tile_for(m, H, W, 3);
    const bool wino7 = m && K == 7 && m->wino_fc6 && m->d_wino_v && wino_tile_for(m, H, W, 7) == 4;
    if (wino3 && dm_ready && e.w_fwd && wino_tile_for(m, H, W, 3) == 6 && Cin % 64 == 0 && Cout % 64 == 0 && e.alpha == 1.f) {
        const int P = 64;
        const long long T = wino_tiles(6, N, H, W);
        IgemmArgs a = fft6_gemm(m->d_wino_m, m->d_wino_u, m->d_wino_v, T, Cin, Cout); a.split = split_of(m);
        auto kept = m->u_train.find(std::string(layer) + "#6");
        if (kept != m->u_train.end() && kept->second && bt_gemm_ok(Cin, Cout)) {
            a.w = kept->second; a.bt = 1; a.ldw = Cin;
        } else {
            ProfScope ps(m, "wino_transform", 0, (double)(9 + P) * 4 * Cin * Cout); launch_wino_filter(6, e.w_fwd, m->d_wino_u, Cout, Cin, 3, s, 1);
        }
        { ProfScope ps(m, "wino_gemm_dgrad", 2.0 * P * T * Cin * Cout, 4.0 * P * (T * (double)(Cin + Cout) + (double)Cin * Cout), layer); launch_igemm(a, P, s); }
        if (e.dm_out && e.dm_out_layer && e.relu_bits_in && !e.addend && e.mask_scale == 1.f) {
            ProfScope ps(m, "wino_transform", 0, 4.0 * ((double)N * H * W * Cout / 32 + 2.0 * P * T * Cout));
            launch_wino_dgrad_output_dout(m->d_wino_v, e.relu_bits_in, e.dm_out, N, H, W, Cout, s);
            m->pass.dm_prefilled.give(e.dm_out_layer);
            return;
        }
        { ProfScope ps(m, "wino_transform", 0, 4.0 * ((double)N * H * W * Cout * (1.0 + (e.relu_bits_in ? 1.0 / 32 : (e.mask ? 1.0 : 0.0)) + (e.addend ? 1.0 : 0.0)) + (double)P * T * Cout));
          launch_wino_dgrad_output(m->d_wino_v, e.addend, e.mask, e.mask_scale, e.relu_bits_in, y, N, H, W, Cout, s); }
        return;
    }
    if (wino7 && dm_ready && e.alpha == 1.f && !e.mask && !e.addend && bt_gemm_ok(Cin, 4 * Cout)) {
        auto kept = m->u_train.find(std::string(layer) + "#4");
        if (kept != m->u_train.end() && kept->second) {
            const int P = 49, Ng = 4 * Cout;
            const long long T = wino_tiles(4, N, H, W);
            IgemmArgs a = fft6_gemm(m->d_wino_m, kept->second, m->d_wino_v, T, Cin, Ng); a.split = split_of(m);
            a.bt = 1; a.ldw = Cin;
            { ProfScope ps(m, "wino_gemm_fc6_dgrad", 2.0 * P * T * Cin * Ng, 4.0 * P * (T * (double)(Cin + Ng) + (double)Cin * Ng), layer); launch_igemm(a, P, s); }
            { ProfScope ps(m, "wino_transform", 0, 4.0 * ((double)N * H * W * Cout + (double)P * T * Ng)); launch_wino_dgrad_output_sub44(m->d_wino_v, y, N, H, W, Cout, s); }
            return;
        }
    }
    if (e.lazy_wt && e.w_fwd) {
        ProfScope ps(m, "weight_relayout", 0, 8.0 * K * K * Cin * Cout); launch_flip_transpose(e.w_fwd, const_cast<float*>(w), K * K, Cout, Cin, s);
    }
    if ((wino3 || wino7) && Cin % 16 == 0 && Cout % 64 == 0 && e.alpha == 1.f) {
        WinoEpi we; we.addend = e.addend; we.mask = e.mask; we.mask_scale = e.mask_scale; we.seed = m->seed; we.rbits_in = e.relu_bits_in;
        conv_winograd(m, wino_tile_for(m, H, W, K), K, false, x, w, y, m->d_wino_u, m->d_wino_v, m->d_wino_m, N, H, W, Cin, Cout, we, s, layer, v_ready);
        return;
    }
    IgemmArgs a{}; a.addend = e.addend; a.mask = e.mask; a.alpha = e.alpha; a.mask_scale = e.mask_scale; a.keep_prob = 1.f;
    conv_direct(m, group, a, x, w, y, N, H, W, Cin, Cout, K, s, 0, layer);
}

void tconv_fwd(fcn8s_model* m, const float* x, const float* wp, const float* bias, const float* addend,
               float* y, int N, int Hi, int Wi, int C, int K, int S, hipStream_t s)
{
    IgemmArgs a{}; a.split = split_of(m);
    a.x = x; a.w = wp; a.bias = bias; a.addend = addend; a.mask = nullptr; a.y = y;
    a.N = N; a.Ma = Hi + 1; a.Mb = Wi + 1; a.M = (long long)N * a.Ma * a.Mb;
    a.Hi = Hi; a.Wi = Wi; a.Cin = C; a.ldx = C;
    a.KW = 2; a.in_scale = 1; a.tap_step = -1; a.tap_off = 0; a.Ktot = 4 * C;
    a.Ho = Hi * S; a.Wo = Wi * S; a.Cout = C; a.ldy = C;
    a.out_scale = S; a.out_offy = -(K - S) / 2; a.out_offx = -(K - S) / 2;
    a.phases_x = S; a.w_phase_stride = 4LL * C * C;
    a.alpha = 1.f; a.relu = 0; a.mask_scale = 1.f; a.dropout = 0;
    const double opix = (double)N * Hi * S * Wi * S;
    ProfScope ps(m, "tconv_fwd", 2.0 * opix * 4 * C * C, 4.0 * (opix * C * (addend ? 2 : 1) + (double)N * Hi * Wi * C)); launch_igemm(a, S * S, s);
}

void tconv_dgrad(fcn8s_model* m, const float* dy, const float* w, float* dx, int N, int Hi, int Wi, int C,
                 int K, int S, hipStream_t s)
{
    IgemmArgs a{}; a.split = split_of(m);
    a.x = dy; a.w = w; a.y = dx;
    a.N = N; a.Ma = Hi; a.Mb = Wi; a.M = (long long)N * Hi * Wi;
    a.Hi = Hi * S; a.Wi = Wi * S; a.Cin = C; a.ldx = C;
    a.KW = K; a.in_scale = S; a.tap_step = 1; a.tap_off = -(K - S) / 2; a.Ktot = K * K * C;
    a.Ho = Hi; a.Wo = Wi; a.Cout = C; a.ldy = C;
    a.out_scale = 1; a.phases_x = 1; a.alpha = 1.f; a.mask_scale = 1.f;
    const double flops = 2.0 * a.M * K * K * C * C;
    ProfScope ps(m, "tconv_dgrad", flops, 4.0 * ((double)N * Hi * S * Wi * S * C + (double)a.M * C)); launch_igemm(a, 1, s);
}

void conv_wgrad(fcn8s_model* m, const char* group, const float* x, const float* dz, float* dw, float* db,
                int N, int H, int W, int Cin, int Cout, int K, float alpha, hipStream_t s, int real_cin = 0,
                const char* layer = nullptr, bool fuse_dgrad_input = false, const unsigned char* pool_idx = nullptr)
{
    const bool promised = m && m->pass.dm_prefilled.take(layer);
    if (m) m->pass.dm_prefilled.drop();
    if (m && m->keep_dy && layer) {
        fcn8s_model::KeptDy& k = m->kept_dy[layer];
        const size_t n = (size_t)N * H * W * Cout;
        k.n = 0;
        if (!(promised || pool_idx || m->pass.dy_bf16_only.count(layer) || m->pass.dz_unwritten.count(layer))) {
            if (k.p.grow(n * sizeof(float), s)) { k.n = n; hipMemcpyAsync(k.p, dz, n * sizeof(float), hipMemcpyDeviceToDevice, s); }
            else defer_error(FCN8S_ERR_OOM, "keep_output_gradients: %s's copy cannot be allocated", layer);
        }
    }
    auto broken_promise = [&]() { defer_error(FCN8S_ERR_STATE, "%s was handed dM instead of dZ but does not take the Winograd-domain path", layer); };
    WgradArgs a{}; a.split = split_of(m);
    a.A = x; a.B = dz; a.C = dw;
    a.N = N; a.Pa = H; a.Pb = W; a.P = (long long)N * H * W;
    a.Ha = H; a.Wa = W; a.Adim = Cin; a.lda = Cin; a.Areal = real_cin ? real_cin : Cin;
    a.Bdim = Cout; a.ldb = Cout;
    a.KW = K; a.a_scale = 1; a.tap_off = -(K - 1) / 2; a.ntaps = K * K;
    a.ldc = Cout; a.alpha = alpha; a.colsum = db;
    const double rc = a.Areal;
    const double flops = 2.0 * a.P * K * K * rc * Cout;
    const double bytes = 4.0 * (a.P * rc + (double)a.P * Cout + (double)K * K * rc * Cout);
    if (bf16_train_mode(m) && m->train_mode && layer && !real_cin && alpha == 1.f && Cin % 64 == 0 && Cout % 64 == 0) {
        auto it = m->xg16.find(layer);
        if (it != m->xg16.end() && it->second) {
            const int pad = (K - 1) / 2, Wp_ = W + 2 * pad;
            const long long G = bf16_guard_rows(K, Wp_), R = (long long)N * (H + 2 * pad) * Wp_;
            bool db_done = false;
            unsigned short* dyb = dyb_for(m, layer, dz, N, H, W, Cout, K, s, db, &db_done);
            if (m->pass.db_taken.count(layer)) db_done = true;
            if (dyb) {
                Bf16WgradArgs g{};
                g.A = it->second + g16_off(G, Cin); g.B = dyb; g.C = dw; g.R = R; g.Ci = Cin; g.Cj = Cout; g.K = K; g.Wp = Wp_; g.a_ps = g.b_ps = g16_ps(N, H, W, K);
                bool done;
                { ProfScope ps(m, K == 1 ? "fc7_wgrad_bf16" : (K == 3 ? "conv3x3_wgrad_bf16" : "fc6_wgrad_bf16"), flops, 2.0 * K * K * R * (Cin + Cout) + 4.0 * K * K * Cin * Cout, layer);
                  done = launch_wgrad_bf16(g, s); }
                if (done) {
                    if (db && !db_done) { ProfScope ps(m, "colsum", 0, 4.0 * a.P * Cout); launch_colsum(dz, db, a.P, Cout, s); }
                    return;
                }
                if (db_done) { defer_error(FCN8S_ERR_SHAPE, "bf16_train: %s's weight-gradient launch refused its shape after the bias gradient was taken", layer); return; }
            }
        }
    }
    if (bf16_train_mode(m) && m->train_mode && layer && (m->pass.in_bf16_only.count(layer) || m->pass.dy_bf16_only.count(layer))) {
        defer_error(FCN8S_ERR_SHAPE, "bf16_train: %s's weight gradient could not run on the bf16 kernel and its fp32 input was not kept (option \"bf16_acts\" = 0 keeps it)", layer); return;
    }
    if (m && K == 7 && alpha == 1.f && !real_cin && m->train_mode && m->pass.fft6_xf.take(layer)) {
        if (promised) broken_promise();
        m->pass.drop_backward_handoffs();
        conv_fft6_wgrad(m, layer, m->acts[std::string("wv:") + layer].p, dz, dw, db, N, H, W, Cin, Cout, s);
        return;
    }
    if (m && (K == 3 || K == 7) && layer && alpha == 1.f && !real_cin && m->train_mode) {
        auto it = m->acts.find(std::string("wv:") + layer);
        if (it != m->acts.end() && m->d_wino_m && (K == 3 || wino_tile_for(m, H, W, 7) == 4)) {
            const int tile = wino_tile_for(m, H, W, K), NP = wino_alpha(tile, K) * wino_alpha(tile, K);
            const long long T = wino_tiles(tile, N, H, W);
            const int Kg = wino_nsub(K) * wino_nsub(K) * Cin;
            WgradArgs g{}; g.split = split_of(m);
            g.A = it->second.p; g.B = m->d_wino_m; g.C = m->d_wino_u;
            g.N = 1; g.Pa = 1; g.Pb = (int)T; g.P = T;
            g.Ha = 1; g.Wa = (int)T; g.Adim = Kg; g.lda = Kg; g.Areal = Kg;
            g.Bdim = Cout; g.ldb = Cout; g.KW = 1; g.a_scale = 1; g.tap_off = 0; g.ntaps = NP; g.ldc = Cout; g.alpha = 1.f; g.colsum = nullptr;
            g.batched = 1; g.a_batch_stride = wino_slab(T, Kg); g.b_batch_stride = wino_slab(T, Cout); g.c_uninitialized = 1;
            bool fused = false, dm_ready = false;
            const bool adj_bytes = fuse_dgrad_input && tile == 6 && K == 3 && Cin % 64 == 0 && Cout % 64 == 0;
            const bool prefilled = promised && adj_bytes && !pool_idx;
            if (promised && !prefilled) broken_promise();
            if (prefilled) dm_ready = true;
            else {
                { ProfScope ps(m, "wino_transform", 0, 4.0 * ((double)N * H * W * Cout * (pool_idx ? 0.3125 : 1.0) + ((fuse_dgrad_input && !adj_bytes) ? 2.0 : 1.0) * NP * T * Cout));
                  if (adj_bytes) { launch_wino_dout(6, dz, m->d_wino_m, N, H, W, Cout, s, 3, pool_idx); dm_ready = true; }
                  else {
                      if (fuse_dgrad_input && tile >= 4 && K == 3) fused = launch_wino_input_dout(tile, dz, m->d_wino_v, m->d_wino_m, N, H, W, Cout, s, pool_idx);
                      if (!fused) launch_wino_dout(tile, dz, m->d_wino_m, N, H, W, Cout, s, K);
                  } }
                if (K == 7 && tile == 4 && !fused && Cin % 2 == 0 && bt_gemm_ok(Cout, 4 * Cin) && m->u_train.count(std::string(layer) + "#4") && !m->pass.fft6_ready.holds(layer)) dm_ready = true;
            }
            m->pass.drop_backward_handoffs();
            if (fused) m->pass.dgrad_v.give(layer);
            if (dm_ready) m->pass.dm.give(layer);
            { ProfScope ps(m, K == 7 ? "wino_gemm_fc6_wgrad" : "wino_gemm_wgrad", 2.0 * NP * T * Kg * Cout, 4.0 * NP * (T * (double)(Kg + Cout) + (double)Kg * Cout), layer); launch_wgrad(g, s); }
            { ProfScope ps(m, "wino_transform", 0, 4.0 * (9.0 + NP) * Cin * Cout + 4.0 * N * H * W * Cout * (tile >= 4 ? 1.0 / (tile * tile) : 1.0));
              launch_wino_dfilter(tile, m->d_wino_u, dw, Cin, Cout, K, s);
              if (db) {
                  if (tile >= 4) launch_colsum(m->d_wino_m + (wino_alpha(tile, K) + 1) * wino_slab(T, Cout), db, T, Cout, s);
                  else launch_colsum(dz, db, (long long)N * H * W, Cout, s);
              } }
            return;
        }
    }
    if (promised) broken_promise();
    const bool taps = (K == 3 || K == 7) && alpha == 1.f && !real_cin;
    const bool first = K == 3 && alpha == 1.f && real_cin == 3 && Cin == 4;
    auto run = [&]() {
        if (K == 1 && !real_cin && Cout <= 32 && launch_head_wgrad(x, dz, dw, a.P, Cin, Cout, alpha, s)) {
            if (db) launch_colsum(dz, db, a.P, Cout, s);
            return;
        }
        if (taps && launch_wgrad_taps(x, dz, dw, db, N, H, W, Cin, Cout, K, s)) return;
        if (first && launch_conv1_wgrad(x, dz, dw, db, N, H, W, Cout, m->conv1_wgrad_mfma, s)) return;
        launch_wgrad(a, s);
    };
    { ProfScope ps(m, group, flops, bytes, layer); run(); }
}

void tconv_wgrad(fcn8s_model* m, const float* x, const float* dy, float* dw, int N, int Hi, int Wi, int C,
                 int K, int S, hipStream_t s)
{
    WgradArgs a{}; a.split = split_of(m);
    a.A = dy; a.B = x; a.C = dw;
    a.N = N; a.Pa = Hi; a.Pb = Wi; a.P = (long long)N * Hi * Wi;
    a.Ha = Hi * S; a.Wa = Wi * S; a.Adim = C; a.lda = C; a.Areal = C;
    a.Bdim = C; a.ldb = C;
    a.KW = K; a.a_scale = S; a.tap_off = -(K - S) / 2; a.ntaps = K * K;
    a.ldc = C; a.alpha = 1.f; a.colsum = nullptr;
    auto run = [&]() { if (!launch_tconv_wgrad(x, dy, dw, N, Hi, Wi, C, K, S, s)) launch_wgrad(a, s); };
    ProfScope ps(m, "tconv_wgrad", 2.0 * a.P * K * K * C * C, 4.0 * ((double)N * Hi * S * Wi * S * C + (double)a.P * C)); run();
}

struct WsItem { std::string name; size_t n; int h, w, c; float** extra; };
struct WsPlan { std::vector<WsItem> items; std::vector<size_t> offs; size_t o_img = 0, o_lab = 0, o_pred = 0, o_part = 0, bytes = 0; };
int check_shape(fcn8s_model* m, int N, int H, int W)
{
    if (N <= 0) return fail(m, FCN8S_ERR_SHAPE, "batch size must be positive");
    if (H <= 0 || W <= 0 || H % 32 || W % 32)
        return fail(m, FCN8S_ERR_SHAPE, "image height and width must be positive multiples of 32 (five 2x2 pools, then x2, x2, x8 upsampling must line up with the skip connections)");
    return FCN8S_OK;
}
void plan_workspace(fcn8s_model* m, int N, int H, int W, WsPlan& pl)
{
    m->plan_N = N;
    const int C = m->C;
    using Item = WsItem;
    std::vector<Item>& items = pl.items;
    items.clear(); pl.offs.clear();
    auto add = [&](const std::string& nm, int h, int w, int c, float** extra = nullptr) {
        items.push_back({nm, (size_t)N * h * w * c, h, w, c, extra});
    };
    add("x0", H, W, 4);
    int h = H, w = W;
    for (int b = 0; b < 5; ++b) {
        for (int i = 1; i <= kConvsPerBlock[b]; ++i) {
            char nm[32]; snprintf(nm, sizeof nm, "conv%d_%d", b + 1, i);
            add(nm, h, w, m->widths[b]);
        }
        h /= 2; w /= 2;
        char nm[32]; snprintf(nm, sizeof nm, "pool%d", b + 1);
        add(nm, h, w, m->widths[b]);
    }
    const int h5 = H / 32, w5 = W / 32, h4 = H / 16, w4 = W / 16, h3 = H / 8, w3 = W / 8;
    {
        int cin = 3;
        for (int b = 0, hh = H, ww = W; b < 5; ++b, hh /= 2, ww /= 2)
// ... 785 lines not shown
    if (with_grad) m->have_terms = true;
    if (lov_sort) {
        ProfScope ps(m, "lovasz", 0, lovasz_bytes(npix, m->C, m->lov_nmask));
        const bool blk = m->tconv_gemm && m->logits_b;
        const float* lg = blk ? m->logits_b : A(m, "logits");
        launch_lovasz_loss(lg, 1, lab_dev, blk ? &m->pm : nullptr, m->N, npix, ly, m->lov_all, m->d_lovmask, m->lov_ws, nullptr, m->d_terms,
                           m->lov_ce, m->lov_w, m->d_loss, s);
        launch_lovasz_backward(lg, 1, lab_dev, blk ? &m->pm : nullptr, m->N, npix, ly, m->lov_ws, m->lov_w, 1, blk ? m->dlogits_b : m->dlogits,
                               m->d_lastbias, s);
    } else if (lov)
        launch_lovasz_total(m->d_terms, m->lov_ce, m->d_loss, s);
    m->loss_copied = m->h_loss && m->loss_ev && hipMemcpyAsync(m->h_loss, m->d_loss, sizeof(float), hipMemcpyDeviceToHost, s) == hipSuccess &&
                     hipEventRecord(m->loss_ev, s) == hipSuccess;
    m->l2_rate = l2_rate; m->have_loss = true;
    return FCN8S_OK;
}

void prepare_backward_weights(fcn8s_model* m)
{
    hipStream_t s = m->stream;
    ProfScope ps(m, "weight_relayout", 0, 8.0 * ((double)m->widths[5] * m->widths[6] +
                                                 (double)m->C * (m->widths[2] + m->widths[3] + m->widths[6])));
    launch_flip_transpose(Wp(m, "fc7/weights"), WTp(m, "fc7/weights"), 1, m->widths[5], m->widths[6], s);
    launch_flip_transpose(Wp(m, "pool3_1x1/kernel"), WTp(m, "pool3_1x1/kernel"), 1, m->widths[2], m->C, s);
    launch_flip_transpose(Wp(m, "pool4_1x1/kernel"), WTp(m, "pool4_1x1/kernel"), 1, m->widths[3], m->C, s);
    launch_flip_transpose(Wp(m, "fc7_1x1/kernel"), WTp(m, "fc7_1x1/kernel"), 1, m->widths[6], m->C, s);
}

void l2_grad(fcn8s_model* m, const char* kernel)
{
    if (m->l2_rate != 0.f) launch_axpy(Gp(m, kernel), Wp(m, kernel), m->l2_rate, (long long)P(m, kernel).numel, m->stream);
}

void mark_bucket_final(fcn8s_model* m, int b, hipStream_t s)
{
    if (!m->bucket_ev[b]) hipEventCreateWithFlags(&m->bucket_ev[b], hipEventDisableTiming);
    hipEventRecord(m->bucket_ev[b], s);
    m->bucket_final[b] = true;
}

void backward_head(fcn8s_model* m)
{
    hipStream_t s = m->stream;
    const int N = m->N, H = m->H, W = m->W, C = m->C;
    const int h5 = H / 32, w5 = W / 32, h4 = H / 16, w4 = W / 16, h3 = H / 8, w3 = W / 8;
    const float inv_keep = (m->train_mode && m->keep_prob < 1.f) ? 1.f / m->keep_prob : 1.f;
    hipMemsetAsync(m->d_grads, 0, m->total * sizeof(float), s);
    prepare_backward_weights(m);
    const bool blk = m->tconv_gemm && m->logits_b;
    if (blk) tconv_gemm_wgrad(m); else tconv_wgrad(m, A(m, "a3"), m->dlogits, Gp(m, "fc7_pool4_pool3_conv2d_trans/kernel"), N, h3, w3, C, 16, 8, s);
    launch_axpy(Gp(m, "fc7_pool4_pool3_conv2d_trans/bias"), m->d_lastbias, 1.f, C, s);
    if (blk) tconv_gemm_dgrad(m); else tconv_dgrad(m, m->dlogits, Wp(m, "fc7_pool4_pool3_conv2d_trans/kernel"), m->da3, N, h3, w3, C, 16, 8, s);
    l2_grad(m, "fc7_pool4_pool3_conv2d_trans/kernel");
    conv_wgrad(m, "score1x1_wgrad", A(m, "pool3"), m->da3, Gp(m, "pool3_1x1/kernel"), Gp(m, "pool3_1x1/bias"), N, h3, w3, m->widths[2], C, 1, 0.0001f, s);
    l2_grad(m, "pool3_1x1/kernel");
    { DgradEpi e; e.alpha = 0.0001f; conv_dgrad(m, "score1x1_dgrad", m->da3, WTp(m, "pool3_1x1/kernel"), m->gskip3, N, h3, w3, C, m->widths[2], 1, e, s); }
    tconv_wgrad(m, A(m, "a4"), m->da3, Gp(m, "fc7_pool4_conv2d_trans/kernel"), N, h4, w4, C, 4, 2, s);
    launch_colsum(m->da3, Gp(m, "fc7_pool4_conv2d_trans/bias"), (long long)N * h3 * w3, C, s);
    tconv_dgrad(m, m->da3, Wp(m, "fc7_pool4_conv2d_trans/kernel"), m->da4, N, h4, w4, C, 4, 2, s);
    l2_grad(m, "fc7_pool4_conv2d_trans/kernel");
    conv_wgrad(m, "score1x1_wgrad", A(m, "pool4"), m->da4, Gp(m, "pool4_1x1/kernel"), Gp(m, "pool4_1x1/bias"), N, h4, w4, m->widths[3], C, 1, 0.01f, s);
    l2_grad(m, "pool4_1x1/kernel");
    { DgradEpi e; e.alpha = 0.01f; conv_dgrad(m, "score1x1_dgrad", m->da4, WTp(m, "pool4_1x1/kernel"), m->gskip4, N, h4, w4, C, m->widths[3], 1, e, s); }
    tconv_wgrad(m, A(m, "s7"), m->da4, Gp(m, "fc7_conv2d_trans/kernel"), N, h5, w5, C, 4, 2, s);
    launch_colsum(m->da4, Gp(m, "fc7_conv2d_trans/bias"), (long long)N * h4 * w4, C, s);
    tconv_dgrad(m, m->da4, Wp(m, "fc7_conv2d_trans/kernel"), m->ds7, N, h5, w5, C, 4, 2, s);
    l2_grad(m, "fc7_conv2d_trans/kernel");
    conv_wgrad(m, "score1x1_wgrad", A(m, "fc7"), m->ds7, Gp(m, "fc7_1x1/kernel"), Gp(m, "fc7_1x1/bias"), N, h5, w5, m->widths[6], C, 1, 1.f, s);
    l2_grad(m, "fc7_1x1/kernel");
    { DgradEpi e; e.mask = A(m, "fc7"); e.mask_scale = inv_keep;
      conv_dgrad(m, "score1x1_dgrad", m->ds7, WTp(m, "fc7_1x1/kernel"), m->gbuf[0], N, h5, w5, C, m->widths[6], 1, e, s); }
    conv_wgrad(m, "fc7_wgrad", A(m, "fc6"), m->gbuf[0], Gp(m, "fc7/weights"), Gp(m, "fc7/biases"), N, h5, w5, m->widths[5], m->widths[6], 1, 1.f, s, 0, "fc7");
    mark_bucket_final(m, 0, s);
}

void backward_fc6(fcn8s_model* m)
{
    hipStream_t s = m->stream;
    const int N = m->N, H = m->H, W = m->W;
    const int h5 = H / 32, w5 = W / 32;
    const float inv_keep = (m->train_mode && m->keep_prob < 1.f) ? 1.f / m->keep_prob : 1.f;
    { DgradEpi e; e.mask = A(m, "fc6"); e.mask_scale = inv_keep; e.w_fwd = Wp(m, "fc7/weights"); e.yb_layer = "fc6"; e.yb_K = m->fc6k;
      conv_dgrad(m, "fc7_dgrad", m->gbuf[0], WTp(m, "fc7/weights"), m->gbuf[1], N, h5, w5, m->widths[6], m->widths[5], 1, e, s, "fc7"); }
    conv_wgrad(m, "fc6_wgrad", A(m, "pool5"), m->gbuf[1], Gp(m, "fc6/weights"), Gp(m, "fc6/biases"), N, h5, w5, m->widths[4], m->widths[5], m->fc6k, 1.f, s, 0, "fc6");
    mark_bucket_final(m, 1, s);
    { DgradEpi e; e.w_fwd = Wp(m, "fc6/weights"); e.lazy_wt = 1;
      conv_dgrad(m, "fc6_dgrad", m->gbuf[1], WTp(m, "fc6/weights"), m->gbuf[0], N, h5, w5, m->widths[5], m->widths[4], m->fc6k, e, s, "fc6"); }
    m->gcur = 0;
}

void backward_blocks(fcn8s_model* m, int b_hi, int b_lo)
{
    hipStream_t s = m->stream;
    const int N = m->N;
    for (int b = b_hi; b >= b_lo; --b) {
        const int h = m->H >> (b - 1), w = m->W >> (b - 1);
        const int cw = m->widths[b - 1];
        const int nconv = kConvsPerBlock[b - 1];
        char last[32]; snprintf(last, sizeof last, "conv%d_%d", b, nconv);
        const unsigned char* pidx = nullptr;
        {
            char ix[16]; snprintf(ix, sizeof ix, "pidx%d", b);
            const bool wino_both = pool_backward_fused(m, b, m->pass.pool_fused[b - 1]);
            if (wino_both) pidx = (const unsigned char*)A(m, ix);
        }
        bool pool_done = false;
        if (!pidx && bf16_train_mode(m) && m->bf16_fuse_pool && m->train_mode && cw % 64 == 0) {
            unsigned short* dzb = g16_for(m, m->dyg16, last, N, h, w, cw, 3, s);
            if (dzb) {
                ProfScope ps(m, "maxpool_bwd", 0, 4.0 * N * h * w * cw * (m->pass.pool_routed[b - 1] ? 0.3125 : 1.25) + 2.0 * N * h * w * cw);
                char ix[16]; snprintf(ix, sizeof ix, "pidx%d", b);
                pool_done = launch_maxpool_bwd_bf16(A(m, last), m->gbuf[m->gcur], dzb, Gp(m, std::string(last) + "/biases"), N, h, w, cw, s,
                                                    m->pass.pool_routed[b - 1] ? (const unsigned char*)A(m, ix) : nullptr, g16_ps(N, h, w, 3));
            }
            if (pool_done) { m->pass.dyg16_filled.insert(last); m->pass.db_taken.insert(last); m->pass.dz_unwritten.insert(last); m->gcur ^= 1; }
        }
        if (!pidx && !pool_done) {
            ProfScope ps(m, "maxpool_bwd", 0, 4.0 * N * h * w * cw * 2.25);
            launch_maxpool_bwd(A(m, last), m->gbuf[m->gcur], m->gbuf[m->gcur ^ 1], N, h, w, cw, 1, s);
            m->gcur ^= 1;
        }
        for (int i = nconv; i >= 1; --i) {
            char nm[32]; snprintf(nm, sizeof nm, "conv%d_%d", b, i);
            const float* dz = m->gbuf[m->gcur];
            const float* xin; int cin; int real_cin = 0;
            char inname[32];
            if (i > 1) { snprintf(inname, sizeof inname, "conv%d_%d", b, i - 1); xin = A(m, inname); cin = cw; }
            else if (b > 1) { snprintf(inname, sizeof inname, "pool%d", b - 1); xin = A(m, inname); cin = m->widths[b - 2]; }
            else { xin = A(m, "x0"); cin = 4; real_cin = 3; }
            const bool first = (b == 1 && i == 1);
            const bool dgrad_wino = !first && m->wino_min_cin > 0 && cw >= m->wino_min_cin && m->d_wino_v && wino_tile_for(m, h, w) >= 4 &&
                                    cw % 16 == 0 && cin % 64 == 0;
            const unsigned char* pix = i == nconv ? pidx : nullptr;
            conv_wgrad(m, first ? "conv1_1_wgrad" : "conv3x3_wgrad", xin, dz, Gp(m, std::string(nm) + "/filter"), Gp(m, std::string(nm) + "/biases"),
                       N, h, w, cin, cw, 3, 1.f, s, real_cin, nm, dgrad_wino, pix);
            if (first) break;
            DgradEpi e; e.w_fwd = Wp(m, std::string(nm) + "/filter"); e.lazy_wt = 1;
            if (i > 1) {
                e.mask = xin; e.mask_scale = 1.f; e.yb_layer = inname; e.yb_K = 3;
                if (m->pass.rbits_ok.count(inname)) e.relu_bits_in = (const unsigned*)A(m, (std::string("rb:") + inname).c_str());
                const int cin_prev = i > 2 ? cw : (b > 1 ? m->widths[b - 2] : 4);
                const bool prev_first = (b == 1 && i == 2);
                e.yb_only = !prev_first && cin_prev % 64 == 0 && cw % 64 == 0;
                if (m->fuse_dgrad_dout && e.relu_bits_in && !prev_first && m->train_mode && m->d_wino_m &&
                    wino_tile_for(m, h, w) == 6 && cw % 64 == 0 && cin_prev % 64 == 0 && m->acts.count(std::string("wv:") + inname)) {
                    e.dm_out = m->d_wino_m; e.dm_out_layer = inname;
                }
            }
            else if (b == 5) e.addend = m->gskip4;
            else if (b == 4) e.addend = m->gskip3;
            conv_dgrad(m, "conv3x3_dgrad", dz, WTp(m, std::string(nm) + "/filter"), m->gbuf[m->gcur ^ 1], N, h, w, cw, cin, 3, e, s, nm);
            m->gcur ^= 1;
        }
    }
}

int do_backward_bucket(fcn8s_model* m, int bucket)
{
    t_deterministic = m->deterministic;
    if (!m->have_loss || !m->train_mode) return fail(m, FCN8S_ERR_STATE, "fcn8s_backward_bucket: call fcn8s_forward_loss first");
    if (bucket != m->next_bucket) return fail(m, FCN8S_ERR_STATE, "fcn8s_backward_bucket: buckets must be run in order 0, 1, ... fcn8s_num_buckets() - 1");
    if (bucket == 0) {
        m->pass.begin_backward();
        for (int b = 0; b < kNumBuckets; ++b) m->bucket_final[b] = false;
        for (int b = 0; b < kNumBuckets; ++b)
            if (m->comm_pending[b]) { hipStreamWaitEvent(m->stream, m->comm_done[b], 0); m->comm_pending[b] = false; }
        backward_head(m);
// ... 156 lines not shown
    }
    if (precision == FCN8S_PREC_BF16_FC || precision == FCN8S_PREC_BF16_FWD || precision == FCN8S_PREC_BF16_FWD_X2) {
        if (m->widths[4] % 32 || m->widths[5] % 128 || m->widths[6] % 128)
            return fail(m, FCN8S_ERR_BAD_ARG, "fcn8s_set_precision: the bf16 modes need conv5 width % 32 == 0 and fc6 / fc7 widths % 128 == 0");
    }
    if (precision != m->precision) {
        HIPCHK(m, hipStreamSynchronize(m->stream));
        drop_precision_state(m);
        const bool was = direct_mode(m->precision), now = direct_mode(precision);
        if (was != now) {
            if (now) { m->saved_wino_min_cin = m->wino_min_cin; m->saved_wino_fc6 = m->wino_fc6; m->wino_min_cin = 0; m->wino_fc6 = 0; }
            else { if (m->saved_wino_min_cin >= 0) m->wino_min_cin = m->saved_wino_min_cin; if (m->saved_wino_fc6 >= 0) m->wino_fc6 = m->saved_wino_fc6; }
            drop_arena(m);
        }
    }
    m->precision = precision;
    return FCN8S_OK;
}
int fcn8s_get_precision(const fcn8s_model* m) { return m ? m->precision : -1; }

int fcn8s_fp8_calibrate(fcn8s_model* m, const void* images, int dtype, int N, int H, int W, int where, int reset)
{
    if (!m || !images) return fail(m, FCN8S_ERR_BAD_ARG, "fcn8s_fp8_calibrate: null argument");
    if (!fp8_mode(m)) return fail(m, FCN8S_ERR_STATE, "fcn8s_fp8_calibrate: set the fp8_infer precision first (fcn8s_set_precision(m, FCN8S_PREC_FP8_INFER))");
    int rc = ensure_workspace(m, N, H, W); if (rc) return rc;
    const void* img; const uint8_t* lab;
    rc = stage_inputs(m, images, dtype, nullptr, where, &img, &lab); if (rc) return rc;
    if (!m->d_fp8_amax.grow(FCN8S_FP8_LAYERS * sizeof(unsigned), m->stream)) return fail(m, FCN8S_ERR_OOM, "fcn8s_fp8_calibrate: out of device memory");
    float start[FCN8S_FP8_LAYERS] = {};
    if (!reset && m->fp8_calibrated) memcpy(start, m->fp8_amax, sizeof start);
    HIPCHK(m, hipStreamSynchronize(m->stream));
    HIPCHK(m, hipMemcpy(m->d_fp8_amax, start, sizeof start, hipMemcpyHostToDevice));
    take_deferred_error(nullptr);
    m->fp8_calibrating = true;
    rc = forward(m, img, dtype, 1.0f, false);
    m->fp8_calibrating = false;
    if (rc) { take_deferred_error(nullptr); return rc; }
    rc = deferred_rc(m); if (rc) return rc;
    {
        double by = 0;
        for (int L = 0; L < FCN8S_FP8_LAYERS; ++L) by += 4.0 * N * (H / kFp8InDiv[L]) * (W / kFp8InDiv[L]) * m->widths[kFp8InWidth[L]];
        ProfScope ps(m, "fp8_calibrate", 0, by);
        for (int L = 0; L < FCN8S_FP8_LAYERS; ++L) {
            const char* in = kFp8Inputs[L];
            auto it = m->acts.find(in);
            if (it == m->acts.end() || !it->second.p || m->pass.y_unwritten.count(in))
                return fail(m, FCN8S_ERR_STATE, std::string("fcn8s_fp8_calibrate: the fp32 pass did not materialise ") + in);
            const long long n = (long long)N * (H / kFp8InDiv[L]) * (W / kFp8InDiv[L]) * m->widths[kFp8InWidth[L]];
            launch_amax(it->second.p, n, m->d_fp8_amax + L, m->stream);
        }
    }
    unsigned bits[FCN8S_FP8_LAYERS];
    HIPCHK(m, hipMemcpyAsync(bits, m->d_fp8_amax, sizeof bits, hipMemcpyDeviceToHost, m->stream));
    HIPCHK(m, hipStreamSynchronize(m->stream));
    memcpy(m->fp8_amax, bits, sizeof bits);
    m->fp8_calibrated = true;
    return FCN8S_OK;
}
int fcn8s_fp8_get_calibration(const fcn8s_model* m, float* amax, int n)
{
    if (!m || !amax || n != FCN8S_FP8_LAYERS) return FCN8S_ERR_BAD_ARG;
    if (!m->fp8_calibrated) return FCN8S_ERR_STATE;
    memcpy(amax, m->fp8_amax, sizeof m->fp8_amax);
    return FCN8S_OK;
}
int fcn8s_fp8_set_calibration(fcn8s_model* m, const float* amax, int n)
{
    if (!m || !amax) return fail(m, FCN8S_ERR_BAD_ARG, "fcn8s_fp8_set_calibration: null argument");
    if (n != FCN8S_FP8_LAYERS) return fail(m, FCN8S_ERR_BAD_ARG, "fcn8s_fp8_set_calibration: needs FCN8S_FP8_LAYERS (14) maxima");
    for (int i = 0; i < n; ++i)
        if (!std::isfinite(amax[i]) || amax[i] < 0.f) return fail(m, FCN8S_ERR_BAD_ARG, "fcn8s_fp8_set_calibration: maxima must be finite and >= 0");
    memcpy(m->fp8_amax, amax, sizeof m->fp8_amax);
    m->fp8_calibrated = true;
    return FCN8S_OK;
}

static int* model_option(fcn8s_model* m, const std::string& key)
{
    if (key == "winograd_min_cin") return &m->wino_min_cin;
    if (key == "winograd_tile") return &m->wino_tile;
    if (key == "winograd_fc6") return &m->wino_fc6;
    if (key == "fc6_fft") return &m->fc6_fft;
    if (key == "fc6_fft_wgrad") return &m->fc6_fft_wgrad;
    if (key == "tconv_gemm") return &m->tconv_gemm;
    if (key == "fuse_dgrad_dout") return &m->fuse_dgrad_dout;
    if (key == "fuse_out_in") return &m->fuse_out_in;
    if (key == "bf16_gemm256") return &m->bf16_gemm256;
    if (key == "winograd_tile_hires") return &m->wino_tile_hires;
    if (key == "winograd_hires_pixels") return &m->wino_hires_pixels;
    if (key == "conv1_tiled") return &m->conv1_tiled;
    if (key == "conv1_wgrad_mfma") return &m->conv1_wgrad_mfma;
    if (key == "bf16_copy_by_transform") return &m->bf16_copy_by_transform;
    if (key == "conv1_in_transform") return &m->conv1_in_transform;
    if (key == "deterministic") return &m->deterministic;
    if (key == "bf16_acts") return &m->bf16_acts;
    if (key == "bf16_rows_bn") return &m->bf16_rows_bn;
    if (key == "keep_output_gradients") return &m->keep_dy;
    if (key == "bf16_infer_copies") return &m->bf16_infer_copies;
    if (key == "bf16_fuse_pool") return &m->bf16_fuse_pool;
    return nullptr;
}
int fcn8s_set_option(fcn8s_model* m, const char* key, int64_t value)
{
    if (!key) return fail(m, FCN8S_ERR_BAD_ARG, "fcn8s_set_option: null key");
    const std::string k = key;
    if (k == "device_bytes_live") return fail(m, FCN8S_ERR_BAD_ARG, "fcn8s_set_option: 'device_bytes_live' is read-only");
    if (!m) {
        if (k == "op_f32x3") { t_op_split = value ? 3 : 0; return FCN8S_OK; }
        if (k == "op_deterministic") { t_deterministic = value ? 1 : 0; return FCN8S_OK; }
        if (k == "op_bf16_planes") { t_op_planes = value ? 1 : 0; return FCN8S_OK; }
        if (k == "op_bf16_rows_bn") { if (value != 0 && value != 64 && value != 128) return fail(nullptr, FCN8S_ERR_BAD_ARG, "op_bf16_rows_bn must be 0, 64 or 128"); t_op_rows_bn = (int)value; return FCN8S_OK; }
        if (k == "op_split_pieces") {
            if (value != 0 && value != 2 && value != 3) return fail(nullptr, FCN8S_ERR_BAD_ARG, "fcn8s_set_option: op_split_pieces is 0, 2 or 3");
            t_op_split = (int)value; return FCN8S_OK;
        }
        return fail(nullptr, FCN8S_ERR_NOT_FOUND, "fcn8s_set_option: unknown op-context option '" + k + "' (model options need a model)");
    }
    if (k == "workspace_allocations" || k == "frozen") return fail(m, FCN8S_ERR_BAD_ARG, "fcn8s_set_option: '" + k + "' is read-only (the frozen state is set with fcn8s_freeze_params)");
    if (k == "comm_timeout_ms") {
        if (value < 1) return fail(m, FCN8S_ERR_BAD_ARG, "comm_timeout_ms must be >= 1");
        std::lock_guard<std::mutex> lk(m->comm_mu); m->comm_timeout_ms = value; return FCN8S_OK;
    }
    if (k == "conv1_tiled" || k == "conv1_wgrad_mfma" || k == "bf16_copy_by_transform" || k == "conv1_in_transform" || k == "deterministic" || k == "bf16_acts" || k == "bf16_rows_bn" || k == "bf16_fuse_pool" || k == "keep_output_gradients" || k == "bf16_infer_copies") {
        *model_option(m, k) = k == "bf16_rows_bn" ? (int)value : (value ? 1 : 0);
        return FCN8S_OK;
    }
    int* slot = model_option(m, k);
    if (!slot) return fail(m, FCN8S_ERR_NOT_FOUND, "fcn8s_set_option: unknown option '" + k + "'");
    if (direct_mode(m->precision) && (k == "winograd_min_cin" || k == "winograd_fc6")) {
        if (value < 0) return fail(m, FCN8S_ERR_BAD_ARG, "fcn8s_set_option: negative value");
        (k == "winograd_min_cin" ? m->saved_wino_min_cin : m->saved_wino_fc6) = (int)value;
        return FCN8S_OK;
    }
    if (k == "winograd_tile" && value != 2 && value != 4 && value != 6) return fail(m, FCN8S_ERR_BAD_ARG, "winograd_tile must be 2, 4 or 6");
    if (k == "winograd_tile_hires" && value != 0 && value != 2 && value != 4 && value != 6) return fail(m, FCN8S_ERR_BAD_ARG, "winograd_tile_hires must be 0, 2, 4 or 6");
    if (k == "winograd_min_cin" && value < 0) return fail(m, FCN8S_ERR_BAD_ARG, "winograd_min_cin must be >= 0 (0 = direct convolution everywhere)");
    if (k == "fuse_out_in" && (value < 0 || value > 2)) return fail(m, FCN8S_ERR_BAD_ARG, "fuse_out_in must be 0, 1 or 2");
    if (k == "fc6_fft_wgrad" && (value < 0 || value > 2)) return fail(m, FCN8S_ERR_BAD_ARG, "fc6_fft_wgrad must be 0, 1 or 2");
    if (*slot == (int)value) return FCN8S_OK;
    HIPCHK(m, hipStreamSynchronize(m->stream));
    *slot = (k == "winograd_fc6" || k == "fc6_fft" || k == "tconv_gemm") ? (value != 0) : (int)value;
    drop_arena(m);
    drop_banks(m, true); m->u_train.clear();
    return FCN8S_OK;
}
int fcn8s_get_option(const fcn8s_model* m, const char* key, int64_t* value)
{
    if (!key || !value) return FCN8S_ERR_BAD_ARG;
    const std::string k = key;
    if (k == "device_bytes_live") { *value = g_device_bytes_live.load(); return FCN8S_OK; }
    if (!m) {
        if (k == "op_f32x3") { *value = t_op_split == 3; return FCN8S_OK; }
        if (k == "op_deterministic") { *value = t_deterministic; return FCN8S_OK; }
        if (k == "op_bf16_planes") { *value = t_op_planes; return FCN8S_OK; }
        if (k == "op_bf16_rows_bn") { *value = t_op_rows_bn; return FCN8S_OK; }
        if (k == "op_split_pieces") { *value = t_op_split; return FCN8S_OK; }
        return FCN8S_ERR_NOT_FOUND;
    }
    if (k == "comm_timeout_ms") { *value = m->comm_timeout_ms; return FCN8S_OK; }
    if (k == "workspace_allocations") { *value = m->ws_allocs; return FCN8S_OK; }
    if (k == "frozen") { *value = m->frozen ? 1 : 0; return FCN8S_OK; }
    const int* slot = model_option(const_cast<fcn8s_model*>(m), k);
    if (!slot) return FCN8S_ERR_NOT_FOUND;
    *value = *slot;
    if (direct_mode(m->precision) && k == "winograd_min_cin" && m->saved_wino_min_cin >= 0) *value = m->saved_wino_min_cin;
    if (direct_mode(m->precision) && k == "winograd_fc6" && m->saved_wino_fc6 >= 0) *value = m->saved_wino_fc6;
    return FCN8S_OK;
}

int fcn8s_set_stream(fcn8s_model* m, void* s) { if (!m) return FCN8S_ERR_BAD_ARG; m->stream = (hipStream_t)s; return FCN8S_OK; }
int fcn8s_synchronize(fcn8s_model* m) { if (!m) return FCN8S_ERR_BAD_ARG; HIPCHK(m, hipStreamSynchronize(m->stream)); return FCN8S_OK; }

int fcn8s_num_params(const fcn8s_model* m) { return m ? (int)m->params.size() : 0; }
int fcn8s_param_info(const fcn8s_model* m, int i, const char** name, int32_t* ndim, int64_t shape[4], int64_t* off)
{
    if (!m || i < 0 || i >= (int)m->params.size()) return FCN8S_ERR_BAD_ARG;
    const ParamInfo& p = m->params[i];
    if (name) *name = p.name.c_str();
    if (ndim) *ndim = p.ndim;
    if (shape) for (int k = 0; k < 4; ++k) shape[k] = p.shape[k];
    if (off) *off = (int64_t)p.offset;
    return FCN8S_OK;
}
int fcn8s_param_index(const fcn8s_model* m, const char* name)
{
    if (!m || !name) return -1;
    auto it = m->index.find(name);
    return it == m->index.end() ? -1 : it->second;
}
static int xfer_named(fcn8s_model* m, float* base, const char* name, void* host, size_t n, bool to_dev)
{
    if (!m || !name || !host) return fail(m, FCN8S_ERR_BAD_ARG, "null argument");
    const int i = fcn8s_param_index(m, name);
    if (i < 0) return fail(m, FCN8S_ERR_NOT_FOUND, std::string("unknown variable '") + name + "'");
    const ParamInfo& p = m->params[i];
    if (n != p.numel) return fail(m, FCN8S_ERR_SHAPE, std::string("variable '") + name + "' has " + std::to_string(p.numel) + " elements, got " + std::to_string(n));
    if (base == m->d_grads) { int rcw = fcn8s_comm_wait(m); if (rcw) return rcw; }
    HIPCHK(m, hipStreamSynchronize(m->stream));
    if (to_dev) HIPCHK(m, hipMemcpy(base + p.offset, host, n * sizeof(float), hipMemcpyHostToDevice));
    else HIPCHK(m, hipMemcpy(host, base + p.offset, n * sizeof(float), hipMemcpyDeviceToHost));
    return FCN8S_OK;
}
int fcn8s_set_param(fcn8s_model* m, const char* name, const float* host, size_t n)
{
    if (m && m->frozen) fcn8s_freeze_params(m, 0);
    fp8_clear_calibration(m);
    return xfer_named(m, m ? m->d_params : nullptr, name, (void*)host, n, true);
}
int fcn8s_get_param(fcn8s_model* m, const char* name, float* host, size_t n) { return xfer_named(m, m ? m->d_params : nullptr, name, host, n, false); }
int fcn8s_get_grad(fcn8s_model* m, const char* name, float* host, size_t n) { return xfer_named(m, m ? m->d_grads : nullptr, name, host, n, false); }
void* fcn8s_param_buffer(fcn8s_model* m, size_t* n) { if (!m) return nullptr; if (n) *n = m->total; return m->d_params; }
void* fcn8s_grad_buffer(fcn8s_model* m, size_t* n) { if (!m) return nullptr; if (n) *n = m->total; return m->d_grads; }
int fcn8s_num_buckets(const fcn8s_model* m) { return m ? kNumBuckets : 0; }
int fcn8s_bucket_range(const fcn8s_model* m, int b, size_t* off, size_t* n)
{
    if (!m || b < 0 || b >= kNumBuckets) return FCN8S_ERR_BAD_ARG;
    if (off) *off = m->bucket_off[b];
    if (n) *n = m->bucket_n[b];
    return FCN8S_OK;
}

int fcn8s_init_params(fcn8s_model* m, uint64_t seed)
{
    if (m && m->frozen) fcn8s_freeze_params(m, 0);
    fp8_clear_calibration(m);
    if (!m) return FCN8S_ERR_BAD_ARG;
    HIPCHK(m, hipMemsetAsync(m->d_params, 0, m->total * sizeof(float), m->stream));
    uint32_t sid = 1000;
    for (auto& p : m->params) {
        ++sid;
        if (p.ndim == 1) continue;
        float std; int trunc = 0;
        const bool vgg = p.name.find("/filter") != std::string::npos || p.name.find("/weights") != std::string::npos;
        if (vgg) std = sqrtf(2.0f / (float)(p.shape[0] * p.shape[1] * p.shape[2]));
        else if (p.name.find("trans") != std::string::npos) { std = 0.01f; trunc = 1; }
        else { std = 0.001f; trunc = 1; }
        launch_init_normal(m->d_params + p.offset, (long long)p.numel, std, trunc, seed, sid, m->stream);
// ... 1184 lines not shown
    if ((!images && !labels) || (images && !out_images) || (labels && !out_labels) || !params || N <= 0 || H <= 0 || W <= 0 || Ho <= 0 || Wo <= 0)
        return fail(nullptr, FCN8S_ERR_BAD_ARG, "resample_u8: bad argument");
    launch_resample_u8(images, labels, images ? out_images : nullptr, labels ? out_labels : nullptr, params, N, H, W, Ho, Wo, void_id, (hipStream_t)stream);
    OPCHK(); return FCN8S_OK;
}

int fcn8s_op_conv2d(void* stream, const float* x, const float* w, const float* bias, float* y,
                    int N, int H, int W, int Cin, int Cout, int K, int relu)
{
    if (Cin % 4 || Cout % 4 || K % 2 == 0) return fail(nullptr, FCN8S_ERR_BAD_ARG, "conv2d: Cin, Cout must be multiples of 4 and K odd");
    FwdEpi e; e.bias = bias; e.relu = relu;
    conv_fwd(nullptr, "", x, w, y, N, H, W, Cin, Cout, K, e, (hipStream_t)stream);
    OPCHK(); return FCN8S_OK;
}

int fcn8s_op_conv2d_winograd(void* stream, const float* x, const float* w, const float* bias, float* y,
                             int N, int H, int W, int Cin, int Cout, int K, int relu, int tile)
{
    if ((tile != 2 && tile != 4 && tile != 6) || (K != 3 && K != 7) || (K == 7 && tile != 4) || Cin % 16 || Cout % 32 || (tile != 6 && (H % tile || W % tile)) || H % 2 || W % 2)
        return fail(nullptr, FCN8S_ERR_BAD_ARG, "conv2d_winograd: needs tile in {2,4,6} (4 for K = 7), K in {3,7}, Cin % 16, Cout % 32, even H and W (multiples of tile for tile 2 and 4)");
    hipStream_t s = (hipStream_t)stream;
    const size_t T = (size_t)wino_tiles(tile, N, H, W), P = (size_t)wino_alpha(tile, K) * wino_alpha(tile, K), Kg = (size_t)wino_nsub(K) * wino_nsub(K) * Cin;
    DeviceBuf<float> u, v, mm;
    if (!u.grow(P * Kg * Cout * 4, s) || !v.grow(P * (size_t)wino_slab(T, (int)Kg) * 4, s) || !mm.grow(P * (size_t)wino_slab(T, Cout) * 4, s)) return fail(nullptr, FCN8S_ERR_OOM, "hipMalloc");
    WinoEpi we; we.bias = bias; we.relu = relu;
    conv_winograd(nullptr, tile, K, true, x, w, y, u, v, mm, N, H, W, Cin, Cout, we, s, nullptr);
    hipStreamSynchronize(s);
    OPCHK(); return FCN8S_OK;
}

int fcn8s_op_conv3x3_winograd_fwd_bwd(void* stream, const float* x, const float* w, const float* bias, const float* dy, const float* dx_addend,
                                      float* y, float* pool, float* dx, float* dw, float* db,
                                      int N, int H, int W, int Cin, int Cout, int tile, int pooled, int mask_mode)
{
    if ((tile != 2 && tile != 4 && tile != 6) || Cin % 64 || Cout % 64 || H % 2 || W % 2 || (tile != 6 && (H % tile || W % tile)) || !x || !w || !dy || !dx || !dw ||
        (pooled && (!pool || tile < 4)) || (!pooled && !y) || mask_mode < 0 || mask_mode > 2)
        return fail(nullptr, FCN8S_ERR_BAD_ARG, "conv3x3_winograd_fwd_bwd: needs tile in {2,4,6}, Cin % 64 == 0, Cout % 64 == 0, even H and W (multiples of tile for tiles 2, 4), "
                                                "pooled only with tiles 4 and 6, mask_mode in {0,1,2}");
    hipStream_t s = (hipStream_t)stream;
    fcn8s_model mm; fcn8s_model* m = &mm;
    m->stream = s; m->wino_min_cin = 16; m->wino_tile = 6; m->wino_force_tile = tile; m->N = N; m->H = H; m->W = W;
    m->precision = t_op_split == 3 ? FCN8S_PREC_F32X3 : t_op_split == 2 ? FCN8S_PREC_F32X2 : FCN8S_PREC_F32;
    const int al = tile + 2, P = al * al, cmax = std::max(Cin, Cout);
    const size_t T = (size_t)wino_tiles(tile, N, H, W);
    const size_t slab_max = (size_t)P * (size_t)wino_slab((long long)T, cmax), slab_in = (size_t)P * (size_t)wino_slab((long long)T, Cin);
    DeviceBuf<float> wino_v, wino_m, wv, wt, pidx, rbits;
    bool ok = true;
    auto dalloc = [&](DeviceBuf<float>& b, size_t nfloats) { ok = ok && b.grow(nfloats * sizeof(float), s); };
    dalloc(m->d_wino_u, (size_t)P * cmax * cmax); dalloc(wino_v, slab_max); dalloc(wino_m, slab_max);
    dalloc(wv, slab_in); dalloc(wt, (size_t)9 * Cin * Cout);
    if (pooled) dalloc(pidx, ((size_t)N * (H / 2) * (W / 2) * Cout + 3) / 4);
    if (mask_mode == 2) dalloc(rbits, wino_rbits_words(tile, N, H, W, Cin));
    if (!ok) return fail(nullptr, FCN8S_ERR_OOM, "hipMalloc");
    m->d_wino_v = wino_v; m->d_wino_m = wino_m;
    Act a; a.p = wv; a.n = slab_in; m->acts["wv:op"] = a;
    m->fwd_train = true; m->train_mode = true;
    { FwdEpi e; e.bias = bias; e.relu = 1;
      if (pooled) { e.pool_out = pool; e.pool_idx = (unsigned char*)pidx.get(); e.skip_y = y == nullptr; }
      if (mask_mode == 2) { e.in_relu_bits_out = (unsigned*)rbits.get(); e.in_layer = "prev"; }
      conv_fwd(m, "op", x, w, y, N, H, W, Cin, Cout, 3, e, s, 0, "op"); }
    hipMemsetAsync(dw, 0, (size_t)9 * Cin * Cout * sizeof(float), s);
    if (db) hipMemsetAsync(db, 0, (size_t)Cout * sizeof(float), s);
    conv_wgrad(m, "op", x, dy, dw, db, N, H, W, Cin, Cout, 3, 1.f, s, 0, "op", tile >= 4, pooled ? (const unsigned char*)pidx.get() : nullptr);
    { DgradEpi e; e.w_fwd = w; e.lazy_wt = 1; e.addend = dx_addend;
      if (mask_mode) { e.mask = x; e.mask_scale = 1.f; }
      if (mask_mode == 2 && m->pass.rbits_ok.count("prev")) e.relu_bits_in = (const unsigned*)rbits.get();
      conv_dgrad(m, "op", dy, wt, dx, N, H, W, Cout, Cin, 3, e, s, "op"); }
    hipStreamSynchronize(s);
    OPCHK(); return FCN8S_OK;
}

int fcn8s_op_conv7x7_fc6_fwd_bwd(void* stream, const float* x, const float* w, const float* bias, const float* dy,
                                 float* y, float* dx, float* dw, float* db,
                                 int N, int H, int W, int Cin, int Cout, int path, float keep_prob, uint64_t seed, int* dft_products)
{
    if (dft_products) *dft_products = 0;
    if (N <= 0 || H <= 0 || W <= 0 || Cin <= 0 || Cout <= 0 || Cin % 16 || Cout % 128 || path < 0 || path > 2 || !(keep_prob > 0.f && keep_prob <= 1.f) ||
        !x || !w || !dy || !y || !dx || !dw)
        return fail(nullptr, FCN8S_ERR_BAD_ARG, "conv7x7_fc6_fwd_bwd: needs Cin % 16 == 0, Cout % 128 == 0, path in {0,1,2}, keep_prob in (0, 1], non-null x, w, dy, y, dx, dw");
    hipStream_t s = (hipStream_t)stream;
    fcn8s_model mm; fcn8s_model* m = &mm;
    m->stream = s; m->N = N; m->H = H; m->W = W; m->plan_N = N; m->seed = seed; m->keep_prob = keep_prob;
    m->precision = t_op_split == 3 ? FCN8S_PREC_F32X3 : t_op_split == 2 ? FCN8S_PREC_F32X2 : FCN8S_PREC_F32;
    m->fc6_fft = path != 0; m->fc6_fft_wgrad = path == 2 ? 2 : 0;
    m->profile = true;
    const Fc6Scratch f6 = fc6_scratch_floats(m, N, H, W, Cin, Cout);
    const size_t vmax = std::max(f6.v_wino, f6.v_fft), mmax = std::max(f6.v_wino, f6.m_fft);
    DeviceBuf<float> wino_v, wino_m, wv, wt;
    bool ok = true;
    auto dalloc = [&](DeviceBuf<float>& b, size_t nfloats, bool poison, const char* slot = nullptr) {
        ok = ok && b.grow(nfloats * sizeof(float), s);
        if (ok && poison) hipMemsetAsync(b, 0xFF, nfloats * sizeof(float), s);
        if (ok && slot) { Act a; a.p = b; a.n = nfloats; m->acts[slot] = a; }
    };
    if (vmax) { dalloc(wino_v, vmax, true, "wino_v"); dalloc(wino_m, mmax, true, "wino_m"); m->d_wino_v = wino_v; m->d_wino_m = wino_m; }
    if (f6.wv) dalloc(wv, f6.wv, true, "wv:op");
    m->ufl = fc6_bank_floats(Cin, Cout);
    dalloc(m->d_wino_u, m->ufl, true);
    dalloc(wt, (size_t)49 * Cin * Cout, false);
    if (!ok) { hipStreamSynchronize(s); return fail(nullptr, FCN8S_ERR_OOM, "hipMalloc"); }
    m->fwd_train = true; m->train_mode = true; m->drop_stream = 0;
    { FwdEpi e; e.bias = bias; e.relu = 1; e.dropout = keep_prob < 1.f; e.keep = keep_prob; e.stream_id = m->drop_stream;
      conv_fwd(m, "fc6_fwd", x, w, y, N, H, W, Cin, Cout, 7, e, s, 0, "op"); }
    hipMemsetAsync(dw, 0, (size_t)49 * Cin * Cout * sizeof(float), s);
    if (db) hipMemsetAsync(db, 0, (size_t)Cout * sizeof(float), s);
    conv_wgrad(m, "fc6_wgrad", x, dy, dw, db, N, H, W, Cin, Cout, 7, 1.f, s, 0, "op");
    { DgradEpi e; e.w_fwd = w; e.lazy_wt = 1;
      conv_dgrad(m, "fc6_dgrad", dy, wt, dx, N, H, W, Cout, Cin, 7, e, s, "op"); }
    if (dft_products)
        for (const auto& g : m->groups) {
            if (g.launches <= 0) continue;
            if (g.name == "fc6_fft_gemm_fwd") *dft_products |= 1;
            if (g.name == "fc6_fft_gemm_wgrad") *dft_products |= 2;
            if (g.name == "fc6_fft_gemm_dgrad") *dft_products |= 4;
        }
    hipStreamSynchronize(s);
    OPCHK(); return FCN8S_OK;
}

int fcn8s_op_conv2d_bf16(void* stream, const float* x, const float* w, const float* bias, float* y,
                         int N, int H, int W, int Cin, int Cout, int K, int relu)
{
    if (Cin % 32 || Cout % 128 || K % 2 == 0) return fail(nullptr, FCN8S_ERR_BAD_ARG, "conv2d_bf16: needs Cin % 32 == 0, Cout % 128 == 0, K odd");
    hipStream_t s = (hipStream_t)stream;
    DeviceBuf<unsigned short> wt;
    if (!wt.grow((size_t)K * K * Cin * Cout * 2, s)) return fail(nullptr, FCN8S_ERR_OOM, "hipMalloc");
    launch_w_to_bf16_tiles(w, wt, K * K * Cin, Cout, s);
    Bf16ConvArgs a{};
    a.x = x; a.wt = wt; a.bias = bias; a.y = y; a.N = N; a.H = H; a.W = W; a.Cin = Cin; a.Cout = Cout; a.K = K; a.relu = relu;
    launch_conv_bf16(a, s);
    hipStreamSynchronize(s);
    OPCHK(); return FCN8S_OK;
}

int fcn8s_op_conv2d_bf16_train(void* stream, const float* x, const float* w, const float* bias, float* y, int relu,
                               const float* dy, const float* mask, float* dx, float* dw, float* db,
                               int N, int H, int W, int Cin, int Cout, int K)
{
    if (Cin % 64 || Cout % 64 || K % 2 == 0) return fail(nullptr, FCN8S_ERR_BAD_ARG, "conv2d_bf16_train: needs Cin % 64 == 0, Cout % 64 == 0, K odd");
    hipStream_t s = (hipStream_t)stream;
    const int pad = (K - 1) / 2, Wp_ = W + 2 * pad;
    const long long G = bf16_guard_rows(K, Wp_), R = (long long)N * (H + 2 * pad) * Wp_;
    const long long PS = t_op_planes ? (R + 2 * G) * 32 : 0;
    const long long OX = t_op_planes ? G * 32 : G * Cin, OY = t_op_planes ? G * 32 : G * Cout;
    DeviceBuf<unsigned short> xb, dyb, wt;
    const size_t nx = (size_t)(R + 2 * G) * Cin, ny = (size_t)(R + 2 * G) * Cout, nw = (size_t)K * K * Cin * Cout;
    if (!wt.grow(nw * 2, s) || (x && !xb.grow(nx * 2, s, nullptr, true)) || (dy && !dyb.grow(ny * 2, s, nullptr, true))) { hipStreamSynchronize(s); return fail(nullptr, FCN8S_ERR_OOM, "hipMalloc"); }
    if (x) {
        launch_f32_to_bf16_padded(x, xb + OX, N, H, W, Cin, pad, s, PS);
    }
    if (dy) {
        launch_f32_to_bf16_padded(dy, dyb + OY, N, H, W, Cout, pad, s, PS);
    }
    bool ok = true;
    if (y && x && w) {
        launch_w_to_bf16_t(w, wt, K * K * Cin, Cout, s);
        Bf16Conv256Args g{};
        g.xp = xb + OX; g.xp_ps = PS; g.wt = wt; g.bias = bias; g.y = y; g.N = N; g.H = H; g.W = W; g.Cin = Cin; g.Cout = Cout; g.K = K; g.relu = relu; g.any_shape = 1; g.mask_scale = 1.f; g.guarded = 1; g.rows_bn = t_op_rows_bn;
        ok = ok && launch_conv_bf16_256(g, s);
    }
    if (dx && dy && w) {
        launch_w_to_bf16_flip_t(w, wt, K, Cin, Cout, s);
        Bf16Conv256Args g{};
        g.xp = dyb + OY; g.xp_ps = PS; g.wt = wt; g.y = dx; g.N = N; g.H = H; g.W = W; g.Cin = Cout; g.Cout = Cin; g.K = K; g.mask = mask; g.mask_scale = 1.f; g.any_shape = 1; g.guarded = 1; g.rows_bn = t_op_rows_bn;
        ok = ok && launch_conv_bf16_256(g, s);
    }
    if (dw && x && dy) {
        Bf16WgradArgs g{};
        g.A = xb + OX; g.B = dyb + OY; g.a_ps = g.b_ps = PS; g.C = dw; g.R = R; g.Ci = Cin; g.Cj = Cout; g.K = K; g.Wp = Wp_;
        ok = ok && launch_wgrad_bf16(g, s);
    }
    if (db && dy) { hipMemsetAsync(db, 0, (size_t)Cout * sizeof(float), s); launch_colsum(dy, db, (long long)N * H * W, Cout, s); }
    hipStreamSynchronize(s);
    if (!ok) return fail(nullptr, FCN8S_ERR_SHAPE, "conv2d_bf16_train: a launch refused the shape");
    OPCHK(); return FCN8S_OK;
}

int fcn8s_op_conv2d_fp8(void* stream, const float* x, const float* w, const float* bias, float* y, int relu, int x_exp,
                        int N, int H, int W, int Cin, int Cout, int K)
{
    if (!x || !w || !y) return fail(nullptr, FCN8S_ERR_BAD_ARG, "conv2d_fp8: null argument");
    if (Cin % 64 || Cout % 64 || K % 2 == 0 || N <= 0 || H <= 0 || W <= 0 || Cin <= 0 || Cout <= 0)
        return fail(nullptr, FCN8S_ERR_BAD_ARG, "conv2d_fp8: needs Cin % 64 == 0, Cout % 64 == 0, K odd, positive sizes");
    hipStream_t s = (hipStream_t)stream;
    const int pad = (K - 1) / 2;
    const long long R = (long long)N * (H + 2 * pad) * (W + 2 * pad);
    const size_t xb = (size_t)R * Cin, wb = (size_t)K * K * Cin * Cout;
    DeviceBuf<unsigned char> xq, wq;
    if (!xq.grow(xb, s, nullptr, true) || !wq.grow(wb + 8 * (size_t)Cout, s)) { hipStreamSynchronize(s); return fail(nullptr, FCN8S_ERR_OOM, "hipMalloc"); }
    launch_f32_to_fp8_padded(x, xq, N, H, W, Cin, pad, R * 64, x_exp, s);
    int* ew = reinterpret_cast<int*>(wq + wb);
// ... 209 lines not shown
```

fcn8s_tensorflow_amd/csrc/pass_state.h:

```cpp
#pragma once
#include <set>
#include <string>

namespace fcn8s {

struct Handoff {
    void give(const char* layer) { who = layer ? layer : ""; }
    bool holds(const char* layer) const { return layer && !who.empty() && who == layer; }
    bool take(const char* layer) { const bool mine = holds(layer); if (mine) who.clear(); return mine; }
    void drop() { who.clear(); }
private:
    std::string who;
};

struct PassState {
    using Layers = std::set<std::string>;

    Layers rbits_ok;
    Layers y_unwritten;
    Layers in_bf16_only;
    Layers xg16_filled;
    Layers q8_filled;
    bool pool_fused[5] = {};
    bool pool_routed[5] = {};
    Handoff fft6_ready;
    Handoff fft6_xf;

    Layers dyg16_filled;
    Layers db_taken;
    Layers dy_bf16_only;
    Layers dz_unwritten;

    Handoff fwd_v;
    Handoff dgrad_v;
    Handoff dm;
    Handoff dm_prefilled;
    Handoff fft6_dyf;

    void begin_forward(bool fp8_pass)
    {
        rbits_ok.clear(); y_unwritten.clear(); in_bf16_only.clear(); xg16_filled.clear();
        if (fp8_pass) q8_filled.clear();
        for (int b = 0; b < 5; ++b) pool_fused[b] = pool_routed[b] = false;
        fft6_ready.drop(); fft6_xf.drop(); fft6_dyf.drop(); fwd_v.drop();
    }
    void begin_backward() { dyg16_filled.clear(); db_taken.clear(); dy_bf16_only.clear(); dz_unwritten.clear(); dm_prefilled.drop(); }
    void forget_shape_copies(bool keep_regrowable)
    {
        xg16_filled.clear(); dyg16_filled.clear();
        if (!keep_regrowable) q8_filled.clear();
    }
    void drop_backward_handoffs() { dm.drop(); dgrad_v.drop(); }
};

}
```

Baseline: 294.0 images/sec.

## Tune fc6 DFT path: software-pipelined output transform, flattened plane grid, earlier dgrad GEMM

Adds a software-pipelined fc6 FFT output kernel that double-buffers the per-column plane loads so memory latency overlaps the inverse-DFT arithmetic. The transposed-B batched GEMM can now fold its frequency planes into grid.x, so tiles from all planes are spread by the XCD swizzle instead of being split across grid.z. The fc6 data-gradient plane GEMM is moved into the weight-gradient step, right after the dy transform, while those planes are still resident. The new op-level harness options add warm-up and partial-call controls. All of this sits behind a new fc6_fft_tune option that defaults to on, and it adds handoff state that must stay consistent between wgrad and dgrad.

After: 293.5 images/sec. Within noise of the previous version (-0.2%).

```diff
diff --git a/fcn8s_tensorflow_amd/csrc/fcn8s_internal.h b/fcn8s_tensorflow_amd/csrc/fcn8s_internal.h
--- a/fcn8s_tensorflow_amd/csrc/fcn8s_internal.h
+++ b/fcn8s_tensorflow_amd/csrc/fcn8s_internal.h
@@ -30,6 +30,8 @@
     int m_fastest;
     int bt, ldw;
     int fixed_tile;
+    int plane_runs;
+    int planes_x;
     int split;
 };
 void launch_igemm(const IgemmArgs& a, int phases, hipStream_t s);
@@ -238,7 +240,7 @@
 void launch_fft_fc6_dfilter(const float* duf, float* dw, int Cin, int Cout, hipStream_t s);
 void launch_fft_fc6_input(const float* x, float* xf, int N, int H, int W, int C, hipStream_t s);
 void launch_fft_fc6_output(const float* yf, const float* bias, float* y, int N, int H, int W, int C, int relu, int dropout, float keep,
-                           unsigned long long seed, unsigned int stream_id, hipStream_t s);
+                           unsigned long long seed, unsigned int stream_id, hipStream_t s, int pipelined = 0);
 void launch_fft_fc6_dout(const float* dz, float* dyf, int N, int H, int W, int C, hipStream_t s);
 void launch_fft_fc6_din(const float* dxf, float* patches, float* dx, int N, int H, int W, int C, hipStream_t s);
 void launch_augment_u8(const unsigned char* img, const unsigned char* lab, unsigned char* oimg, unsigned char* olab, const int* params,
diff --git a/fcn8s_tensorflow_amd/csrc/fft_fc6.hip b/fcn8s_tensorflow_amd/csrc/fft_fc6.hip
--- a/fcn8s_tensorflow_amd/csrc/fft_fc6.hip
+++ b/fcn8s_tensorflow_amd/csrc/fft_fc6.hip
@@ -247,6 +247,98 @@
 }
 
 template <int V>
+__device__ __forceinline__ void output_col_load(const float* __restrict__ yf, long long slab, unsigned off, float (&raw)[42])
+{
+    constexpr int NU = nu_of(V);
+    asm volatile("" : "+s"(slab));
+#pragma unroll
+    for (int u = 0; u < NU; ++u) {
+        if (is_real(u, V)) raw[3 * u] = (yf + realp(u, V) * slab)[off];
+        else {
+            const float* p = yf + 3LL * cplx(u, V) * slab;
+            raw[3 * u] = p[off]; raw[3 * u + 1] = (p + slab)[off]; raw[3 * u + 2] = (p + 2 * slab)[off];
+        }
+    }
+}
+template <int V>
+__device__ __forceinline__ void output_col_eval(const float (&raw)[42], float (&acc)[8][8])
+{
+    constexpr int NU = nu_of(V);
+    float R[NU], I[NU];
+#pragma unroll
+    for (int u = 0; u < NU; ++u) {
+        if (is_real(u, V)) { R[u] = raw[3 * u]; I[u] = 0.f; }
+        else { R[u] = raw[3 * u] - raw[3 * u + 2]; I[u] = raw[3 * u] + raw[3 * u + 1]; }
+    }
+#pragma unroll
+    for (int j = 0; j < 8; ++j) {
+        const int n = 6 + j;
+        float P = 0.f, Q = 0.f;
+#pragma unroll
+        for (int u = 0; u < NU; ++u) {
+            const float beta = (is_real(u, V) ? 1.f : 2.f) / 196.f;
+            if (is_real(u, V)) { P = fmaf(R[u], beta * c14(u * n), P); Q = fmaf(R[u], beta * s14(u * n), Q); }
+            else {
+                P = fmaf(R[u], beta * c14(u * n), fmaf(I[u], -beta * s14(u * n), P));
+                Q = fmaf(R[u], beta * s14(u * n), fmaf(I[u], beta * c14(u * n), Q));
+            }
+        }
+#pragma unroll
+        for (int i = 0; i < 8; ++i) acc[j][i] = fmaf(P, c14(V * (6 + i)), fmaf(Q, -s14(V * (6 + i)), acc[j][i]));
+    }
+}
+__device__ __forceinline__ unsigned offset_after(unsigned off, const float (&a)[8][8])
+{
+#pragma unroll
+    for (int j = 0; j < 8; ++j)
+        asm volatile("" : "+v"(off) : "v"(a[j][0]), "v"(a[j][1]), "v"(a[j][2]), "v"(a[j][3]), "v"(a[j][4]), "v"(a[j][5]), "v"(a[j][6]), "v"(a[j][7]));
+    return off;
+}
+
+__global__ __launch_bounds__(256) void fft_fc6_output_pipe_kernel(const float* __restrict__ yf, const float* __restrict__ bias, float* __restrict__ y,
+                                                                  int N, int H, int W, int C, long long slab, int relu, int dropout, float keep,
+                                                                  unsigned long long seed, unsigned int stream_id)
+{
+    const int th = (H + 7) / 8, tw = (W + 7) / 8;
+    const long long total = (long long)N * th * tw * C;
+    for (long long i = (long long)blockIdx.x * 256 + threadIdx.x; i < total; i += (long long)gridDim.x * 256) {
+        const int c = (int)(i % C);
+        const long long t = i / C;
+        const int tx = (int)(t % tw), ty = (int)((t / tw) % th), n = (int)(t / ((long long)tw * th));
+        float acc[8][8];
+#pragma unroll
+        for (int j = 0; j < 8; ++j)
+#pragma unroll
+            for (int k = 0; k < 8; ++k) acc[j][k] = 0.f;
+        unsigned off = (unsigned)i;
+        float ra[42], rb[42];
+        output_col_load<0>(yf, slab, off, ra); output_col_load<1>(yf, slab, off, rb);
+        output_col_eval<0>(ra, acc); off = offset_after(off, acc); output_col_load<2>(yf, slab, off, ra);
+        output_col_eval<1>(rb, acc); off = offset_after(off, acc); output_col_load<3>(yf, slab, off, rb);
+        output_col_eval<2>(ra, acc); off = offset_after(off, acc); output_col_load<4>(yf, slab, off, ra);
+        output_col_eval<3>(rb, acc); off = offset_after(off, acc); output_col_load<5>(yf, slab, off, rb);
+        output_col_eval<4>(ra, acc); off = offset_after(off, acc); output_col_load<6>(yf, slab, off, ra);
+        output_col_eval<5>(rb, acc); off = offset_after(off, acc); output_col_load<7>(yf, slab, off, rb);
+        output_col_eval<6>(ra, acc);
+        output_col_eval<7>(rb, acc);
+        const float bv = bias ? bias[c] : 0.f;
+        const float ik = 1.f / keep;
+#pragma unroll
+        for (int j = 0; j < 8; ++j)
+#pragma unroll
+            for (int k = 0; k < 8; ++k) {
+                const int py = 8 * ty + j, px = 8 * tx + k;
+                if (py >= H || px >= W) continue;
+                float v = bv + acc[j][k];
+                if (relu) v = fmaxf(v, 0.f);
+                const long long o = (((long long)n * H + py) * W + px) * C + c;
+                if (dropout) v = philox_uniform((unsigned long long)o, seed, stream_id) < keep ? v * ik : 0.f;
+                y[o] = v;
+            }
+    }
+}
+
+template <int V>
 __device__ __forceinline__ void dout_col(const float (&d)[8][8], float* __restrict__ dyf, long long slab, long long tc)
 {
     float sr[8], si[8];
@@ -401,9 +493,13 @@
     hipLaunchKernelGGL(fft_fc6_input_kernel, dim3(grid_for(T * 8 * C)), dim3(256), 0, s, x, xf, N, H, W, C, wino_slab(T, C));
 }
 void launch_fft_fc6_output(const float* yf, const float* bias, float* y, int N, int H, int W, int C, int relu, int dropout, float keep,
-                           unsigned long long seed, unsigned int stream_id, hipStream_t s)
+                           unsigned long long seed, unsigned int stream_id, hipStream_t s, int pipelined)
 {
     const long long T = fft_fc6_tiles(N, H, W);
+    if (pipelined && T * C < (1LL << 30)) {
+        hipLaunchKernelGGL(fft_fc6_output_pipe_kernel, dim3(grid_for(T * C)), dim3(256), 0, s, yf, bias, y, N, H, W, C, wino_slab(T, C), relu, dropout, keep, seed, stream_id);
+        return;
+    }
     hipLaunchKernelGGL(fft_fc6_output_kernel, dim3(grid_for(T * C)), dim3(256), 0, s, yf, bias, y, N, H, W, C, wino_slab(T, C), relu, dropout, keep, seed, stream_id);
 }
 void launch_fft_fc6_dout(const float* dz, float* dyf, int N, int H, int W, int C, hipStream_t s)
diff --git a/fcn8s_tensorflow_amd/csrc/igemm.hip b/fcn8s_tensorflow_amd/csrc/igemm.hip
--- a/fcn8s_tensorflow_amd/csrc/igemm.hip
+++ b/fcn8s_tensorflow_amd/csrc/igemm.hip
@@ -455,13 +455,16 @@
         }
     }
     const int wm = cwave / WN, wn = cwave % WN;
-    const int pz = blockIdx.z;
+    int pz = blockIdx.z;
+    unsigned lid = xcd_swizzle(blockIdx.x, gridDim.x), ntiles = gridDim.x;
+    if constexpr (BT) {
+        if (p.planes_x > 0) { ntiles = gridDim.x / (unsigned)p.planes_x; pz = (int)(lid / ntiles); lid -= (unsigned)pz * ntiles; }
+    }
     const float* __restrict__ Wp = p.w + (long long)pz * p.w_phase_stride;
     const float* __restrict__ X = p.batched ? p.x + (long long)pz * p.x_batch_stride : p.x;
     float* __restrict__ Y = p.batched ? p.y + (long long)pz * p.y_batch_stride : p.y;
     const unsigned ntn = (unsigned)(p.Cout / BN);
-    const unsigned lid = xcd_swizzle(blockIdx.x, gridDim.x);
-    const unsigned ntm = gridDim.x / ntn;
+    const unsigned ntm = ntiles / ntn;
     const long long m0 = (long long)(p.m_fastest ? lid % ntm : lid / ntn) * BM;
     const int n0 = (int)(p.m_fastest ? lid / ntm : lid % ntn) * BN;
 
@@ -910,6 +913,10 @@
                 if (mode != 3 || (long long)(BN - 1) * a.ldw >= (1LL << 29)) { defer_error(FCN8S_ERR_STATE, "transposed-B GEMM needs the plain batched form"); return; }
                 static const std::string nbx2 = "gemm_glds_nt_x2_kernel<" + std::to_string(BM) + ", " + std::to_string(BN) + ", " + std::to_string(WM) + ", " + std::to_string(WN) + ", 3>";
                 g_last_kernel = (a.split == 3 ? nbx : a.split == 2 ? nbx2 : nb).c_str();
+                a.planes_x = 0;
+                if (a.plane_runs && a.batched && grid.y == 1 && phases > 1 && (unsigned long long)grid.x * (unsigned)phases < (1ull << 31)) {
+                    a.planes_x = phases; grid.x *= (unsigned)phases; grid.z = 1;
+                }
                 if (a.split == 3) hipLaunchKernelGGL((gemm_glds_nt_x3_kernel<BM, BN, WM, WN, 3>), grid, dim3(256), 0, s, a);
                 else if (a.split == 2) hipLaunchKernelGGL((gemm_glds_nt_x2_kernel<BM, BN, WM, WN, 3>), grid, dim3(256), 0, s, a);
                 else                   hipLaunchKernelGGL((gemm_glds_nt_kernel<BM, BN, WM, WN, 3>), grid, dim3(256), 0, s, a);
diff --git a/fcn8s_tensorflow_amd/csrc/model.hip b/fcn8s_tensorflow_amd/csrc/model.hip
--- a/fcn8s_tensorflow_amd/csrc/model.hip
+++ b/fcn8s_tensorflow_amd/csrc/model.hip
@@ -105,6 +105,7 @@
     int wino_tile = 6;
     int wino_fc6 = 1;
     int fc6_fft = 1;
+    int fc6_fft_tune = 1;
     int fc6_fft_wgrad = 1;
     int wino_tile_hires = 0, wino_hires_pixels = 0;
     int wino_force_tile = 0;
@@ -338,6 +339,9 @@
 static bool bt_gemm_ok(int K, int N) { return K % 16 == 0 && (N == 64 || N % 128 == 0); }
 thread_local int t_op_split = 0;
 thread_local int t_op_rows_bn = 0;
+thread_local int t_op_fc6_tune = 1;
+thread_local int t_op_fc6_calls = 3;
+thread_local int t_op_fc6_warm = 0;
 thread_local int t_op_planes = 1;
 int split_of(const fcn8s_model* m)
 {
@@ -394,6 +398,8 @@
            mm->second.n >= std::max((size_t)fft_fc6_planes() * (size_t)wino_slab(T, co), (size_t)T * 196 * ci);
 }
 constexpr long long kFft6WgradMinTiles = 32;
+constexpr int kFft6TuneOrder = 2, kFft6TunePlaneRuns = 4, kFft6TuneOutput = 8;
+static bool fft6_tuned(const fcn8s_model* m, int item) { return m->fc6_fft_tune == 1 || (m->fc6_fft_tune & item) != 0; }
 static bool fft6_wgrad_wanted(const fcn8s_model* m, long long T) { return m->fc6_fft_wgrad == 2 || (m->fc6_fft_wgrad == 1 && T >= kFft6WgradMinTiles); }
 struct Fc6Scratch { size_t v_wino = 0, v_fft = 0, m_fft = 0, wv = 0; };
 static Fc6Scratch fc6_scratch_floats(const fcn8s_model* m, int N, int h5, int w5, int ci, int co)
@@ -454,17 +460,26 @@
     IgemmArgs a = fft6_gemm(xf, uf, m->d_wino_m, T, Cin, Cout); a.fixed_tile = 1;
     { ProfScope ps(m, "fc6_fft_gemm_fwd", 2.0 * P * T * Cin * Cout, 4.0 * P * (T * (double)(Cin + Cout) + (double)Cin * Cout), layer); launch_igemm(a, P, s); }
     { ProfScope ps(m, "fc6_fft_transform", 0, 4.0 * ((double)P * T * Cout + (double)N * H * W * Cout));
-      launch_fft_fc6_output(m->d_wino_m, bias, y, N, H, W, Cout, relu, dropout, keep, m->seed, stream_id, s); }
+      launch_fft_fc6_output(m->d_wino_m, bias, y, N, H, W, Cout, relu, dropout, keep, m->seed, stream_id, s, fft6_tuned(m, kFft6TuneOutput)); }
     m->pass.fft6_ready.give(layer);
     if (dft_wgrad) m->pass.fft6_xf.give(layer);
     return true;
 }
-static void conv_fft6_wgrad(fcn8s_model* m, const char* layer, const float* xf, const float* dz, float* dw, float* db, int N, int H, int W, int Cin, int Cout, hipStream_t s)
+static void fft6_dgrad_planes(fcn8s_model* m, const char* layer, const float* uf, long long T, int Cin, int Cout, hipStream_t s)
+{
+    const int P = fft_fc6_planes();
+    IgemmArgs a = fft6_gemm(m->d_wino_m, uf, m->d_wino_v, T, Cin, Cout);
+    a.fixed_tile = 1; a.bt = 1; a.ldw = Cin; a.plane_runs = fft6_tuned(m, kFft6TunePlaneRuns);
+    ProfScope ps(m, "fc6_fft_gemm_dgrad", 2.0 * P * T * Cin * Cout, 4.0 * P * (T * (double)(Cin + Cout) + (double)Cin * Cout), layer); launch_igemm(a, P, s);
+}
+static void conv_fft6_wgrad(fcn8s_model* m, const char* layer, const float* xf, const float* dz, float* dw, float* db, int N, int H, int W, int Cin, int Cout,
+                            const float* dgrad_uf, hipStream_t s)
 {
     const int P = fft_fc6_planes();
     const long long T = fft_fc6_tiles(N, H, W);
     { ProfScope ps(m, "fc6_fft_transform", 0, 4.0 * ((double)N * H * W * Cout + (double)P * T * Cout)); launch_fft_fc6_dout(dz, m->d_wino_m, N, H, W, Cout, s); }
     m->pass.fft6_dyf.give(layer);
+    if (dgrad_uf) { fft6_dgrad_planes(m, layer, dgrad_uf, T, Cout, Cin, s); m->pass.fft6_dxf.give(layer); }
     WgradArgs g{}; g.split = 0;
     g.A = xf; g.B = m->d_wino_m; g.C = m->d_wino_u;
     g.N = 1; g.Pa = 1; g.Pb = (int)T; g.P = T;
@@ -475,17 +490,16 @@
     { ProfScope ps(m, "fc6_fft_transform", 0, 4.0 * (P + 49.0) * Cin * Cout); launch_fft_fc6_dfilter(m->d_wino_u, dw, Cin, Cout, s); }
     if (db) { ProfScope ps(m, "colsum", 0, 4.0 * N * H * W * Cout); launch_colsum(dz, db, (long long)N * H * W, Cout, s); }
 }
-static void conv_fft6_dgrad(fcn8s_model* m, const char* layer, const float* dz, const float* uf, float* dx, int N, int H, int W, int Cin, int Cout, hipStream_t s)
+static void conv_fft6_dgrad(fcn8s_model* m, const char* layer, const float* dz, const float* uf, float* dx, int N, int H, int W, int Cin, int Cout, bool dxf_ready, hipStream_t s)
 {
     const int P = fft_fc6_planes();
     const long long T = fft_fc6_tiles(N, H, W);
-    if (!m->pass.fft6_dyf.take(layer)) {
-        m->pass.fft6_dyf.drop();
-        ProfScope ps(m, "fc6_fft_transform", 0, 4.0 * ((double)N * H * W * Cin + (double)P * T * Cin)); launch_fft_fc6_dout(dz, m->d_wino_m, N, H, W, Cin, s);
-    }
-    IgemmArgs a = fft6_gemm(m->d_wino_m, uf, m->d_wino_v, T, Cin, Cout);
-    a.fixed_tile = 1; a.bt = 1; a.ldw = Cin;
-    { ProfScope ps(m, "fc6_fft_gemm_dgrad", 2.0 * P * T * Cin * Cout, 4.0 * P * (T * (double)(Cin + Cout) + (double)Cin * Cout), layer); launch_igemm(a, P, s); }
+    const bool dyf_ready = m->pass.fft6_dyf.take(layer);
+    m->pass.fft6_dyf.drop();
+    if (!dxf_ready) {
+        if (!dyf_ready) { ProfScope ps(m, "fc6_fft_transform", 0, 4.0 * ((double)N * H * W * Cin + (double)P * T * Cin)); launch_fft_fc6_dout(dz, m->d_wino_m, N, H, W, Cin, s); }
+        fft6_dgrad_planes(m, layer, uf, T, Cin, Cout, s);
+    }
     { ProfScope ps(m, "fc6_fft_transform", 0, 4.0 * ((double)P * T * Cout + 2.0 * 196.0 * T * Cout + (double)N * H * W * Cout));
       launch_fft_fc6_din(m->d_wino_v, m->d_wino_m, dx, N, H, W, Cout, s); }
 }
@@ -625,15 +639,16 @@
     if (bf16_step && e.mask && m->pass.in_bf16_only.count(layer)) {
         defer_error(FCN8S_ERR_SHAPE, "bf16_train: %s's data gradient could not run on the bf16 kernel and its fp32 mask was not kept (option \"bf16_acts\" = 0 keeps it)", layer); return;
     }
-    const bool dm_ready = m && m->pass.dm.take(layer), v_ready = m && m->pass.dgrad_v.take(layer);
+    const bool dm_ready = m && m->pass.dm.take(layer), v_ready = m && m->pass.dgrad_v.take(layer), dxf_ready = m && m->pass.fft6_dxf.take(layer);
     if (m) m->pass.drop_backward_handoffs();
     if (m && K == 7 && layer && e.alpha == 1.f && !e.addend && !e.mask && !e.relu_bits_in) {
         auto kept = m->u_train.find(std::string(layer) + "#fft");
         if (m->pass.fft6_ready.holds(layer) && kept != m->u_train.end() && kept->second && fft6_on(m, N, H, W, Cout, Cin) && bt_gemm_ok(Cin, Cout)) {
-            conv_fft6_dgrad(m, layer, x, kept->second, y, N, H, W, Cin, Cout, s);
+            conv_fft6_dgrad(m, layer, x, kept->second, y, N, H, W, Cin, Cout, dxf_ready, s);
             return;
         }
     }
+    if (dxf_ready) { defer_error(FCN8S_ERR_STATE, "%s: the data-gradient planes ran with the weight gradient, but the data gradient is not the DFT one", layer); return; }
     const bool wino3 = m && K == 3 && m->wino_min_cin > 0 && Cin >= m->wino_min_cin && m->d_wino_v && wino_tile_for(m, H, W, 3);
     const bool wino7 = m && K == 7 && m->wino_fc6 && m->d_wino_v && wino_tile_for(m, H, W, 7) == 4;
     if (wino3 && dm_ready && e.w_fwd && wino_tile_for(m, H, W, 3) == 6 && Cin % 64 == 0 && Cout % 64 == 0 && e.alpha == 1.f) {
@@ -765,7 +780,12 @@
     if (m && K == 7 && alpha == 1.f && !real_cin && m->train_mode && m->pass.fft6_xf.take(layer)) {
         if (promised) broken_promise();
         m->pass.drop_backward_handoffs();
-        conv_fft6_wgrad(m, layer, m->acts[std::string("wv:") + layer].p, dz, dw, db, N, H, W, Cin, Cout, s);
+        const float* dgrad_uf = nullptr;
+        if (fuse_dgrad_input && fft6_tuned(m, kFft6TuneOrder) && m->pass.fft6_ready.holds(layer) && fft6_on(m, N, H, W, Cin, Cout) && bt_gemm_ok(Cout, Cin)) {
+            auto kept = m->u_train.find(std::string(layer) + "#fft");
+            if (kept != m->u_train.end() && kept->second) dgrad_uf = kept->second;
+        }
+        conv_fft6_wgrad(m, layer, m->acts[std::string("wv:") + layer].p, dz, dw, db, N, H, W, Cin, Cout, dgrad_uf, s);
         return;
     }
     if (m && (K == 3 || K == 7) && layer && alpha == 1.f && !real_cin && m->train_mode) {
@@ -786,7 +806,7 @@
             if (promised && !prefilled) broken_promise();
             if (prefilled) dm_ready = true;
             else {
-                { ProfScope ps(m, "wino_transform", 0, 4.0 * ((double)N * H * W * Cout * (pool_idx ? 0.3125 : 1.0) + ((fuse_dgrad_input && !adj_bytes) ? 2.0 : 1.0) * NP * T * Cout));
+                { ProfScope ps(m, "wino_transform", 0, 4.0 * ((double)N * H * W * Cout * (pool_idx ? 0.3125 : 1.0) + ((fuse_dgrad_input && K == 3 && !adj_bytes) ? 2.0 : 1.0) * NP * T * Cout));
                   if (adj_bytes) { launch_wino_dout(6, dz, m->d_wino_m, N, H, W, Cout, s, 3, pool_idx); dm_ready = true; }
                   else {
                       if (fuse_dgrad_input && tile >= 4 && K == 3) fused = launch_wino_input_dout(tile, dz, m->d_wino_v, m->d_wino_m, N, H, W, Cout, s, pool_idx);
@@ -1738,7 +1758,8 @@
     const float inv_keep = (m->train_mode && m->keep_prob < 1.f) ? 1.f / m->keep_prob : 1.f;
     { DgradEpi e; e.mask = A(m, "fc6"); e.mask_scale = inv_keep; e.w_fwd = Wp(m, "fc7/weights"); e.yb_layer = "fc6"; e.yb_K = m->fc6k;
       conv_dgrad(m, "fc7_dgrad", m->gbuf[0], WTp(m, "fc7/weights"), m->gbuf[1], N, h5, w5, m->widths[6], m->widths[5], 1, e, s, "fc7"); }
-    conv_wgrad(m, "fc6_wgrad", A(m, "pool5"), m->gbuf[1], Gp(m, "fc6/weights"), Gp(m, "fc6/biases"), N, h5, w5, m->widths[4], m->widths[5], m->fc6k, 1.f, s, 0, "fc6");
+    conv_wgrad(m, "fc6_wgrad", A(m, "pool5"), m->gbuf[1], Gp(m, "fc6/weights"), Gp(m, "fc6/biases"), N, h5, w5, m->widths[4], m->widths[5], m->fc6k, 1.f, s, 0, "fc6",
+               true);
     mark_bucket_final(m, 1, s);
     { DgradEpi e; e.w_fwd = Wp(m, "fc6/weights"); e.lazy_wt = 1;
       conv_dgrad(m, "fc6_dgrad", m->gbuf[1], WTp(m, "fc6/weights"), m->gbuf[0], N, h5, w5, m->widths[5], m->widths[4], m->fc6k, e, s, "fc6"); }
@@ -2061,6 +2082,7 @@
     if (key == "winograd_fc6") return &m->wino_fc6;
     if (key == "fc6_fft") return &m->fc6_fft;
     if (key == "fc6_fft_wgrad") return &m->fc6_fft_wgrad;
+    if (key == "fc6_fft_tune") return &m->fc6_fft_tune;
     if (key == "tconv_gemm") return &m->tconv_gemm;
     if (key == "fuse_dgrad_dout") return &m->fuse_dgrad_dout;
     if (key == "fuse_out_in") return &m->fuse_out_in;
@@ -2088,6 +2110,9 @@
         if (k == "op_f32x3") { t_op_split = value ? 3 : 0; return FCN8S_OK; }
         if (k == "op_deterministic") { t_deterministic = value ? 1 : 0; return FCN8S_OK; }
         if (k == "op_bf16_planes") { t_op_planes = value ? 1 : 0; return FCN8S_OK; }
+        if (k == "op_fc6_fft_tune") { if (value < 0 || value > 15) return fail(nullptr, FCN8S_ERR_BAD_ARG, "op_fc6_fft_tune must be 0 .. 15"); t_op_fc6_tune = (int)value; return FCN8S_OK; }
+        if (k == "op_fc6_calls") { if (value < 1 || value > 3) return fail(nullptr, FCN8S_ERR_BAD_ARG, "op_fc6_calls must be 1, 2 or 3"); t_op_fc6_calls = (int)value; return FCN8S_OK; }
+        if (k == "op_fc6_warm_images") { if (value < 0 || value > (1 << 20)) return fail(nullptr, FCN8S_ERR_BAD_ARG, "op_fc6_warm_images must be >= 0"); t_op_fc6_warm = (int)value; return FCN8S_OK; }
         if (k == "op_bf16_rows_bn") { if (value != 0 && value != 64 && value != 128) return fail(nullptr, FCN8S_ERR_BAD_ARG, "op_bf16_rows_bn must be 0, 64 or 128"); t_op_rows_bn = (int)value; return FCN8S_OK; }
         if (k == "op_split_pieces") {
             if (value != 0 && value != 2 && value != 3) return fail(nullptr, FCN8S_ERR_BAD_ARG, "fcn8s_set_option: op_split_pieces is 0, 2 or 3");
@@ -2100,8 +2125,9 @@
         if (value < 1) return fail(m, FCN8S_ERR_BAD_ARG, "comm_timeout_ms must be >= 1");
         std::lock_guard<std::mutex> lk(m->comm_mu); m->comm_timeout_ms = value; return FCN8S_OK;
     }
-    if (k == "conv1_tiled" || k == "conv1_wgrad_mfma" || k == "bf16_copy_by_transform" || k == "conv1_in_transform" || k == "deterministic" || k == "bf16_acts" || k == "bf16_rows_bn" || k == "bf16_fuse_pool" || k == "keep_output_gradients" || k == "bf16_infer_copies") {
-        *model_option(m, k) = k == "bf16_rows_bn" ? (int)value : (value ? 1 : 0);
+    if (k == "conv1_tiled" || k == "conv1_wgrad_mfma" || k == "bf16_copy_by_transform" || k == "conv1_in_transform" || k == "deterministic" || k == "fc6_fft_tune" || k == "bf16_acts" || k == "bf16_rows_bn" || k == "bf16_fuse_pool" || k == "keep_output_gradients" || k == "bf16_infer_copies") {
+        if (k == "fc6_fft_tune" && (value < 0 || value > 15)) return fail(m, FCN8S_ERR_BAD_ARG, "fc6_fft_tune must be 0 .. 15");
+        *model_option(m, k) = (k == "bf16_rows_bn" || k == "fc6_fft_tune") ? (int)value : (value ? 1 : 0);
         return FCN8S_OK;
     }
     int* slot = model_option(m, k);
@@ -2132,6 +2158,9 @@
         if (k == "op_f32x3") { *value = t_op_split == 3; return FCN8S_OK; }
         if (k == "op_deterministic") { *value = t_deterministic; return FCN8S_OK; }
         if (k == "op_bf16_planes") { *value = t_op_planes; return FCN8S_OK; }
+        if (k == "op_fc6_fft_tune") { *value = t_op_fc6_tune; return FCN8S_OK; }
+        if (k == "op_fc6_calls") { *value = t_op_fc6_calls; return FCN8S_OK; }
+        if (k == "op_fc6_warm_images") { *value = t_op_fc6_warm; return FCN8S_OK; }
         if (k == "op_bf16_rows_bn") { *value = t_op_rows_bn; return FCN8S_OK; }
         if (k == "op_split_pieces") { *value = t_op_split; return FCN8S_OK; }
         return FCN8S_ERR_NOT_FOUND;
@@ -3482,7 +3511,7 @@
     fcn8s_model mm; fcn8s_model* m = &mm;
     m->stream = s; m->N = N; m->H = H; m->W = W; m->plan_N = N; m->seed = seed; m->keep_prob = keep_prob;
     m->precision = t_op_split == 3 ? FCN8S_PREC_F32X3 : t_op_split == 2 ? FCN8S_PREC_F32X2 : FCN8S_PREC_F32;
-    m->fc6_fft = path != 0; m->fc6_fft_wgrad = path == 2 ? 2 : 0;
+    m->fc6_fft = path != 0; m->fc6_fft_wgrad = path == 2 ? 2 : 0; m->fc6_fft_tune = t_op_fc6_tune;
     m->profile = true;
     const Fc6Scratch f6 = fc6_scratch_floats(m, N, H, W, Cin, Cout);
     const size_t vmax = std::max(f6.v_wino, f6.v_fft), mmax = std::max(f6.v_wino, f6.m_fft);
@@ -3499,14 +3528,20 @@
     dalloc(m->d_wino_u, m->ufl, true);
     dalloc(wt, (size_t)49 * Cin * Cout, false);
     if (!ok) { hipStreamSynchronize(s); return fail(nullptr, FCN8S_ERR_OOM, "hipMalloc"); }
-    m->fwd_train = true; m->train_mode = true; m->drop_stream = 0;
-    { FwdEpi e; e.bias = bias; e.relu = 1; e.dropout = keep_prob < 1.f; e.keep = keep_prob; e.stream_id = m->drop_stream;
-      conv_fwd(m, "fc6_fwd", x, w, y, N, H, W, Cin, Cout, 7, e, s, 0, "op"); }
-    hipMemsetAsync(dw, 0, (size_t)49 * Cin * Cout * sizeof(float), s);
-    if (db) hipMemsetAsync(db, 0, (size_t)Cout * sizeof(float), s);
-    conv_wgrad(m, "fc6_wgrad", x, dy, dw, db, N, H, W, Cin, Cout, 7, 1.f, s, 0, "op");
-    { DgradEpi e; e.w_fwd = w; e.lazy_wt = 1;
-      conv_dgrad(m, "fc6_dgrad", dy, wt, dx, N, H, W, Cout, Cin, 7, e, s, "op"); }
+    auto pass = [&](int n, int calls, bool follows) {
+        m->N = n; m->pass.begin_forward(false);
+        m->fwd_train = true; m->train_mode = true; m->drop_stream = 0;
+        { FwdEpi e; e.bias = bias; e.relu = 1; e.dropout = keep_prob < 1.f; e.keep = keep_prob; e.stream_id = m->drop_stream;
+          conv_fwd(m, "fc6_fwd", x, w, y, n, H, W, Cin, Cout, 7, e, s, 0, "op"); }
+        m->pass.begin_backward();
+        hipMemsetAsync(dw, 0, (size_t)49 * Cin * Cout * sizeof(float), s);
+        if (db) hipMemsetAsync(db, 0, (size_t)Cout * sizeof(float), s);
+        if (calls & 1) conv_wgrad(m, "fc6_wgrad", x, dy, dw, db, n, H, W, Cin, Cout, 7, 1.f, s, 0, "op", follows);
+        if (calls & 2) { DgradEpi e; e.w_fwd = w; e.lazy_wt = 1;
+                         conv_dgrad(m, "fc6_dgrad", dy, wt, dx, n, H, W, Cout, Cin, 7, e, s, "op"); }
+    };
+    if (t_op_fc6_warm > 0) pass(std::min(t_op_fc6_warm, N), 1, true);
+    pass(N, t_op_fc6_calls, t_op_fc6_calls == 3);
     if (dft_products)
         for (const auto& g : m->groups) {
             if (g.launches <= 0) continue;
diff --git a/fcn8s_tensorflow_amd/csrc/pass_state.h b/fcn8s_tensorflow_amd/csrc/pass_state.h
--- a/fcn8s_tensorflow_amd/csrc/pass_state.h
+++ b/fcn8s_tensorflow_amd/csrc/pass_state.h
@@ -36,13 +36,14 @@
     Handoff dm;
     Handoff dm_prefilled;
     Handoff fft6_dyf;
+    Handoff fft6_dxf;
 
     void begin_forward(bool fp8_pass)
     {
         rbits_ok.clear(); y_unwritten.clear(); in_bf16_only.clear(); xg16_filled.clear();
         if (fp8_pass) q8_filled.clear();
         for (int b = 0; b < 5; ++b) pool_fused[b] = pool_routed[b] = false;
-        fft6_ready.drop(); fft6_xf.drop(); fft6_dyf.drop(); fwd_v.drop();
+        fft6_ready.drop(); fft6_xf.drop(); fft6_dyf.drop(); fft6_dxf.drop(); fwd_v.drop();
     }
     void begin_backward() { dyg16_filled.clear(); db_taken.clear(); dy_bf16_only.clear(); dz_unwritten.clear(); dm_prefilled.drop(); }
     void forget_shape_copies(bool keep_regrowable)
@@ -50,7 +51,7 @@
         xg16_filled.clear(); dyg16_filled.clear();
         if (!keep_regrowable) q8_filled.clear();
     }
-    void drop_backward_handoffs() { dm.drop(); dgrad_v.drop(); }
+    void drop_backward_handoffs() { dm.drop(); dgrad_v.drop(); fft6_dxf.drop(); }
 };
 
 }
```
